# shenwei356/wfa

Measured on AMD Instinct MI355X. Metric: aligned pairs/sec (and Gcells/s) on 1e6 synthetic 1 kbp pairs @5% error, higher is better.
Workload: dtype u32; 1 GPU; 1000000 x 1000 bp pairs/GPU @5% error, global gap-affine 4/6/2, wf-adaptive 10/50/1, seed 3; config=c3, pairs_per_gpu=1000000, length=1000, parallelism=pair-sharded x1, ranks_seen_by_collective=1, backend=none (1 GPU), collective_forced=False, status_ok=1000000, setup_steps=0, gather=none (1 GPU), gather_bytes_per_rank_step=0, packed_pairs=1000000, retried_pairs=831

## Files before the change

### include/wfa_hip.h

```cpp
#ifndef WFA_HIP_H
#define WFA_HIP_H

#include <stddef.h>
#include <stdint.h>

#ifdef __cplusplus
extern "C" {
#endif

#define WFAHIP_VERSION 400

enum {
    WFAHIP_OK              = 0,
    WFAHIP_ERR_NO_DEVICE   = -1,
    WFAHIP_ERR_BAD_ARG     = -2,
    WFAHIP_ERR_OOM         = -3,
    WFAHIP_ERR_HIP         = -4,
    WFAHIP_ERR_UNSUPPORTED = -5,
    WFAHIP_ERR_INTERNAL    = -6
};

enum {
    WFAHIP_PAIR_OK        = 0,
    WFAHIP_PAIR_EMPTY     = 1,
// ... 180 lines not shown

int      wfahip_submit(wfahip_ctx *ctx, const uint8_t *q, uint32_t n, const uint8_t *t, uint32_t m, uint64_t *ticket);

int      wfahip_align_pair(wfahip_ctx *ctx, const wfahip_params *p, const uint8_t *q, uint32_t n, const uint8_t *t, uint32_t m,
                           uint32_t *rec, uint64_t *ops, uint64_t ops_cap, uint64_t *n_ops);
uint64_t wfahip_pending(const wfahip_ctx *ctx);
int      wfahip_collect(wfahip_ctx *ctx, const wfahip_params *p, wfahip_results *out);

typedef struct wfahip_multi wfahip_multi;
int         wfahip_create_multi(const int *device_ids, int n_devices, wfahip_multi **out);
void        wfahip_destroy_multi(wfahip_multi *m);
int         wfahip_multi_size(const wfahip_multi *m);
wfahip_ctx *wfahip_multi_ctx(wfahip_multi *m, int i);
int         wfahip_align_batch_multi(wfahip_multi *m, const wfahip_params *p, const uint8_t *seq_blob,
                                     uint64_t blob_bytes, const uint64_t *q_off, const uint32_t *q_len,
                                     const uint64_t *t_off, const uint32_t *t_len, uint64_t n_pairs,
                                     wfahip_results *out);

int  wfahip_last_timing(const wfahip_ctx *ctx, wfahip_timing *out);

int  wfahip_set_option(wfahip_ctx *ctx, const char *key, int64_t value);

typedef struct { uint32_t score; int32_t lo; uint32_t width; uint64_t word_off; } wfahip_row;
int  wfahip_debug_wavefronts(wfahip_ctx *ctx, const wfahip_params *p, const uint8_t *q, uint32_t n,
                             const uint8_t *t, uint32_t m, wfahip_row **rows, uint64_t *n_rows,
                             uint32_t **words, uint64_t *n_words, wfahip_results *res);
void wfahip_free(void *p);

int  wfahip_debug_team_compact(wfahip_ctx *ctx, const wfahip_params *p, const uint8_t *q, uint32_t n, const uint8_t *t, uint32_t m,
                               wfahip_row **rows, uint64_t *n_rows, uint32_t **words, uint64_t *n_words, wfahip_results *res);
int  wfahip_debug_compact_arena(wfahip_ctx *ctx, uint64_t pair, uint32_t **words, uint64_t *n_words, uint32_t *fmt,
                                uint32_t *meta4);

int  wfahip_debug_score_long_list(const uint8_t *seq_blob, const uint64_t *q_off, const uint32_t *q_len, const uint64_t *t_off,
                                  const uint32_t *t_len, uint64_t n_pairs, uint32_t **words, uint64_t *n_words, uint32_t **table,
                                  uint64_t *n_listed);

int  wfahip_debug_score_device_list(wfahip_ctx *ctx, uint32_t **words, uint64_t *n_words, uint32_t **table, uint64_t *n_listed);

int  wfahip_debug_prepack(wfahip_ctx *ctx, const void *d_seq_blob, const void *d_q_off, const void *d_q_len, const void *d_t_off,
                          const void *d_t_len, const void *d_work, uint64_t n, uint32_t seq_words, uint32_t ppw, uint32_t *slots);

int  wfahip_wide_class_bounds(uint32_t *bounds, int cap);

int  wfahip_debug_wide_plan(wfahip_ctx *ctx, const uint32_t *q_len, const uint32_t *t_len, uint64_t n_pairs, uint32_t **ids,
                            uint64_t *counts, uint32_t *longest, uint64_t *n_ladder);

uint64_t wfahip_gen_stride(uint32_t length, double error_rate);
int      wfahip_generate_pairs(uint64_t seed, uint64_t first_index, uint64_t n_pairs, uint32_t length,
                               double error_rate, int n_threads, uint8_t *blob, uint64_t *q_off,
                               uint32_t *q_len, uint64_t *t_off, uint32_t *t_len);

int      wfahip_debug_clock(wfahip_ctx *ctx, double *mhz, double *mhz_min, double *mhz_max);
int      wfahip_generate_pairs_device(wfahip_ctx *ctx, uint64_t seed, uint64_t first_index, uint64_t n_pairs, uint32_t length,
                                      double error_rate, void *d_blob, void *d_q_off, void *d_q_len, void *d_t_off,
                                      void *d_t_len, void *stream);

#ifdef __cplusplus
}
#endif
#endif
```

### wfa_amd/_lib.py

```python
from __future__ import annotations

import ctypes as C
import os

_HERE = os.path.dirname(os.path.abspath(__file__))
LIB_PATH = os.path.join(_HERE, "lib", "libwfahip.so")

OK, ERR_NO_DEVICE, ERR_BAD_ARG, ERR_OOM, ERR_HIP, ERR_UNSUPPORTED, ERR_INTERNAL = 0, -1, -2, -3, -4, -5, -6
PAIR_OK, PAIR_EMPTY, PAIR_TOO_LONG, PAIR_NO_MEMORY = 0, 1, 2, 4
PAIR_OVER_MAX = 8
MAX_SEQ_LEN = (1 << 29) - 1
REC_WORDS = 16
(REC_STATUS, REC_SCORE, REC_TBEGIN, REC_TEND, REC_QBEGIN, REC_QEND, REC_ALIGN_LEN, REC_MATCHES, REC_GAPS,
 REC_GAP_REGIONS, REC_OPS_LEN, REC_OPS_OFF_LO, REC_OPS_OFF_HI, REC_CELLS_LO, REC_CELLS_HI, REC_N_SCORES) = range(16)

EXPORTS = [
    "wfahip_version", "wfahip_strerror", "wfahip_device_count", "wfahip_create", "wfahip_destroy",
    "wfahip_align_batch", "wfahip_results_free", "wfahip_align_batch_device", "wfahip_last_timing",
    "wfahip_set_option", "wfahip_debug_wavefronts", "wfahip_free", "wfahip_gen_stride",
    "wfahip_generate_pairs", "wfahip_packed_words", "wfahip_pack_pairs", "wfahip_align_batch_packed", "wfahip_align_batch_packed_rc", "wfahip_submit",
    "wfahip_pending", "wfahip_collect", "wfahip_create_multi", "wfahip_destroy_multi", "wfahip_multi_size",
    "wfahip_multi_ctx", "wfahip_align_batch_multi", "wfahip_debug_compact_arena",
    "wfahip_generate_pairs_device", "wfahip_align_pair", "wfahip_last_error", "wfahip_debug_clock",
    "wfahip_debug_team_compact", "wfahip_score_batch", "wfahip_scores_free", "wfahip_score_matrix",
    "wfahip_debug_score_long_list", "wfahip_score_batch_device", "wfahip_debug_score_device_list",
    "wfahip_align_batch_bounded", "wfahip_align_batch_bounded_device", "wfahip_score_batch_packed",
    "wfahip_wide_class_bounds", "wfahip_debug_wide_plan", "wfahip_debug_prepack",
    "wfahip_score_batch_packed_rc", "wfahip_score_matrix_rc", "wfahip_revcomp_packed",
    "wfahip_cigar_text_device", "wfahip_cigar_text", "wfahip_cigars_free", "wfahip_align_batch_text",
    "wfahip_alignment_text_device", "wfahip_alignment_text", "wfahip_align_texts_free",
    "wfahip_pack_pairs_device", "wfahip_align_batch_packed_device",
    "wfahip_score_batch_packed_device", "wfahip_select_pairs_device",
    "wfahip_alignment_text_packed_device", "wfahip_alignment_text_packed",
]


class Params(C.Structure):
    _fields_ = [("mismatch", C.c_uint32), ("gap_open", C.c_uint32), ("gap_ext", C.c_uint32),
                ("global_alignment", C.c_uint8), ("adaptive", C.c_uint8), ("reserved", C.c_uint8 * 2),
                ("min_wf_len", C.c_uint32), ("max_dist_diff", C.c_uint32), ("cutoff_step", C.c_uint32)]


class Results(C.Structure):
    _fields_ = [("n", C.c_uint64), ("status", C.POINTER(C.c_int32)), ("score", C.POINTER(C.c_uint32)),
                ("tbegin", C.POINTER(C.c_int32)), ("tend", C.POINTER(C.c_int32)),
                ("qbegin", C.POINTER(C.c_int32)), ("qend", C.POINTER(C.c_int32)),
                ("align_len", C.POINTER(C.c_uint32)), ("matches", C.POINTER(C.c_uint32)),
                ("gaps", C.POINTER(C.c_uint32)), ("gap_regions", C.POINTER(C.c_uint32)),
                ("ops_off", C.POINTER(C.c_uint64)), ("ops_len", C.POINTER(C.c_uint32)),
                ("ops", C.POINTER(C.c_uint64)), ("n_ops", C.c_uint64)]


class Scores(C.Structure):
    _fields_ = [("n", C.c_uint64), ("status", C.POINTER(C.c_int32)), ("score", C.POINTER(C.c_uint32))]


class Cigars(C.Structure):
    _fields_ = [("n", C.c_uint64), ("n_bytes", C.c_uint64), ("text", C.POINTER(C.c_uint8)), ("off", C.POINTER(C.c_uint64))]


class AlignTexts(C.Structure):
    _fields_ = [("n", C.c_uint64), ("n_bytes", C.c_uint64), ("q_row", C.POINTER(C.c_uint8)), ("a_row", C.POINTER(C.c_uint8)),
                ("t_row", C.POINTER(C.c_uint8)), ("off", C.POINTER(C.c_uint64))]


class Timing(C.Structure):
    _fields_ = [("kernel_ms", C.c_double), ("total_ms", C.c_double), ("n_launches", C.c_uint32),
                ("n_retried_pairs", C.c_uint32), ("cells_stored", C.c_uint64), ("ops_written", C.c_uint64),
                ("arena_bytes", C.c_uint64), ("main_kernel_ms", C.c_double), ("n_main_launches", C.c_uint32),
                ("n_packed_pairs", C.c_uint32), ("main_kernel_kind", C.c_uint32), ("ladder_start_level", C.c_uint32)]


class Row(C.Structure):
    _fields_ = [("score", C.c_uint32), ("lo", C.c_int32), ("width", C.c_uint32), ("word_off", C.c_uint64)]


_lib = None


def lib():
    global _lib
    if _lib is None:
        if not os.path.exists(LIB_PATH):
            raise RuntimeError(f"{LIB_PATH} is missing: build the HIP extension first "
                               "(`make` or `python -c 'import __graft_entry__ as g; g.build()'`). "
                               "There is no CPU fallback.")
# ... 51 lines not shown
        L.wfahip_cigar_text.argtypes = [C.POINTER(Results), C.c_int, C.c_int, C.POINTER(Cigars)]
        L.wfahip_cigars_free.argtypes = [C.POINTER(Cigars)]
        L.wfahip_align_batch_text.restype = C.c_int
        L.wfahip_align_batch_text.argtypes = [vp, C.POINTER(Params), vp, u64, vp, vp, vp, vp, u64, C.c_int, C.POINTER(Results),
                                              C.POINTER(Cigars)]
        L.wfahip_alignment_text_device.restype = C.c_int
        L.wfahip_alignment_text_device.argtypes = [vp, vp, vp, u64, vp, u64, vp, vp, vp, vp, u64, C.c_int, vp, vp, vp, u64, vp,
                                                   C.POINTER(u64), vp]
        L.wfahip_alignment_text.restype = C.c_int
        L.wfahip_alignment_text.argtypes = [C.POINTER(Results), vp, u64, vp, vp, vp, vp, C.c_int, C.c_int, C.POINTER(AlignTexts)]
        L.wfahip_align_texts_free.argtypes = [C.POINTER(AlignTexts)]
        L.wfahip_alignment_text_packed_device.restype = C.c_int
        L.wfahip_alignment_text_packed_device.argtypes = [vp, vp, vp, u64, vp, u64, vp, vp, vp, vp, vp, u64, C.c_int, vp, vp, vp, u64, vp,
                                                          C.POINTER(u64), vp]
        L.wfahip_alignment_text_packed.restype = C.c_int
        L.wfahip_alignment_text_packed.argtypes = [C.POINTER(Results), vp, u64, vp, vp, vp, vp, vp, C.c_int, C.c_int, C.POINTER(AlignTexts)]
        L.wfahip_last_timing.restype = C.c_int
        L.wfahip_last_timing.argtypes = [vp, C.POINTER(Timing)]
        L.wfahip_set_option.restype = C.c_int
        L.wfahip_set_option.argtypes = [vp, C.c_char_p, C.c_int64]
        L.wfahip_debug_wavefronts.restype = C.c_int
        L.wfahip_debug_wavefronts.argtypes = [vp, C.POINTER(Params), C.c_char_p, u32, C.c_char_p, u32,
                                              C.POINTER(C.POINTER(Row)), C.POINTER(u64),
                                              C.POINTER(C.POINTER(u32)), C.POINTER(u64), C.POINTER(Results)]
        L.wfahip_debug_team_compact.restype = C.c_int
        L.wfahip_debug_team_compact.argtypes = [vp, C.POINTER(Params), C.c_char_p, u32, C.c_char_p, u32,
                                              C.POINTER(C.POINTER(Row)), C.POINTER(u64),
                                              C.POINTER(C.POINTER(u32)), C.POINTER(u64), C.POINTER(Results)]
        L.wfahip_free.argtypes = [vp]
        L.wfahip_gen_stride.restype = u64
        L.wfahip_gen_stride.argtypes = [u32, C.c_double]
        L.wfahip_generate_pairs.restype = C.c_int
        L.wfahip_generate_pairs.argtypes = [u64, u64, u64, u32, C.c_double, C.c_int, vp, vp, vp, vp, vp]
        L.wfahip_packed_words.restype = u64
        L.wfahip_packed_words.argtypes = [u32]
        L.wfahip_pack_pairs.restype = C.c_int
        L.wfahip_pack_pairs.argtypes = [vp, vp, vp, vp, vp, u64, C.c_int, vp, vp, vp, C.POINTER(u64)]
        L.wfahip_align_batch_packed.restype = C.c_int
        L.wfahip_align_batch_packed.argtypes = [vp, C.POINTER(Params), vp, u64, vp, vp, vp, vp, u64, C.POINTER(Results)]
        L.wfahip_align_batch_packed_rc.restype = C.c_int
        L.wfahip_align_batch_packed_rc.argtypes = [vp, C.POINTER(Params), vp, u64, vp, vp, vp, vp, vp, u64, C.POINTER(Results)]
        L.wfahip_pack_pairs_device.restype = C.c_int
        L.wfahip_pack_pairs_device.argtypes = [vp, vp, u64, vp, vp, vp, vp, u64, vp, u64, vp, vp, C.POINTER(u64), vp]
        L.wfahip_align_batch_packed_device.restype = C.c_int
        L.wfahip_align_batch_packed_device.argtypes = [vp, C.POINTER(Params), vp, u64, vp, vp, vp, vp, vp, u64, u32, u32, vp, vp,
                                                       u64, C.POINTER(u64), vp]
        L.wfahip_score_batch_packed_device.restype = C.c_int
        L.wfahip_score_batch_packed_device.argtypes = [vp, C.POINTER(Params), vp, u64, vp, vp, vp, vp, vp, u64, u32, u32, vp, vp, vp]
        L.wfahip_select_pairs_device.restype = C.c_int
        L.wfahip_select_pairs_device.argtypes = [vp, vp, u64, vp, vp, vp, vp, vp, vp, vp, vp, vp, vp, vp, C.POINTER(u64), vp]
        L.wfahip_submit.restype = C.c_int
        L.wfahip_submit.argtypes = [vp, C.c_char_p, u32, C.c_char_p, u32, C.POINTER(u64)]
        L.wfahip_pending.restype = u64
        L.wfahip_debug_clock.restype = C.c_int
        L.wfahip_debug_clock.argtypes = [vp, C.POINTER(C.c_double), C.POINTER(C.c_double), C.POINTER(C.c_double)]
        L.wfahip_align_pair.restype = C.c_int
        L.wfahip_align_pair.argtypes = [vp, C.POINTER(Params), C.c_char_p, u32, C.c_char_p, u32, vp, vp, u64, C.POINTER(u64)]
        L.wfahip_last_error.restype = C.c_char_p
        L.wfahip_last_error.argtypes = [vp]
        L.wfahip_pending.argtypes = [vp]
        L.wfahip_collect.restype = C.c_int
        L.wfahip_collect.argtypes = [vp, C.POINTER(Params), C.POINTER(Results)]
        L.wfahip_create_multi.restype = C.c_int
        L.wfahip_create_multi.argtypes = [C.POINTER(C.c_int), C.c_int, C.POINTER(vp)]
        L.wfahip_destroy_multi.argtypes = [vp]
        L.wfahip_multi_size.restype = C.c_int
        L.wfahip_multi_size.argtypes = [vp]
        L.wfahip_multi_ctx.restype = vp
        L.wfahip_multi_ctx.argtypes = [vp, C.c_int]
        L.wfahip_align_batch_multi.restype = C.c_int
        L.wfahip_align_batch_multi.argtypes = [vp, C.POINTER(Params), vp, u64, vp, vp, vp, vp, u64, C.POINTER(Results)]
        L.wfahip_debug_compact_arena.restype = C.c_int
        L.wfahip_debug_compact_arena.argtypes = [vp, u64, C.POINTER(C.POINTER(u32)), C.POINTER(u64), C.POINTER(u32),
                                                 C.POINTER(u32 * 4)]
        L.wfahip_generate_pairs_device.restype = C.c_int
        L.wfahip_generate_pairs_device.argtypes = [vp, u64, u64, u64, u32, C.c_double, vp, vp, vp, vp, vp, vp]
        _lib = L
    return _lib


class WfaHipError(RuntimeError):
    def __init__(self, code: int, what: str = ""):
        self.code = code
        msg = lib().wfahip_strerror(code).decode()
        super().__init__(f"{what}: {msg} ({code})" if what else f"{msg} ({code})")


def check(code: int, what: str = ""):
    if code != OK:
        raise WfaHipError(code, what)
```

### wfa_amd/aligner.py

```python
from __future__ import annotations

import ctypes as C
from dataclasses import dataclass, field
from typing import List, Optional, Sequence, Tuple

import numpy as np

from . import _lib as L

MaxSeqLen = L.MAX_SEQ_LEN
MaskLower32 = 4294967295
OpM, OpD, OpI, OpX, OpH = ord("M"), ord("D"), ord("I"), ord("X"), ord("H")


class WfaError(Exception):
    pass


ErrEmptySeq = WfaError("wfa: invalid empty sequence")
ErrSeqTooLong = WfaError(f"wfa: sequences longer than {MaxSeqLen} are not supported")
ErrOverMaxScore = WfaError("wfa: alignment score exceeds max_score")


@dataclass
# ... 842 lines not shown
        L.check(L.lib().wfahip_debug_team_compact(self._ctx, C.byref(prm), q, len(q), t, len(t), C.byref(rows),
                                                  C.byref(n_rows), C.byref(words), C.byref(n_words), C.byref(res)),
                "wfahip_debug_team_compact")
        try:
            out = {}
            for i in range(n_rows.value):
                r = rows[i]
                out[int(r.score)] = {r.lo + j: int(words[r.word_off + j]) for j in range(r.width)}
            br = BatchResult.from_c(res, 1)
        finally:
            L.lib().wfahip_free(rows)
            L.lib().wfahip_free(words)
            L.lib().wfahip_results_free(C.byref(res))
        return out, br.result(0)

    def debug_wavefronts(self, q: bytes, t: bytes):
        rows, words = C.POINTER(L.Row)(), C.POINTER(C.c_uint32)()
        n_rows, n_words = C.c_uint64(), C.c_uint64()
        res = L.Results()
        prm = self._params()
        L.check(L.lib().wfahip_debug_wavefronts(self._ctx, C.byref(prm), q, len(q), t, len(t), C.byref(rows),
                                                C.byref(n_rows), C.byref(words), C.byref(n_words), C.byref(res)),
                "wfahip_debug_wavefronts")
        try:
            out = {"M": {}, "I": {}, "D": {}}
            for i in range(n_rows.value):
                r = rows[i]
                for ci, name in enumerate("MID"):
                    d = {}
                    for j in range(r.width):
                        w = words[r.word_off + ci * r.width + j]
                        if w:
                            d[r.lo + j] = int(w)
                    if d:
                        out[name][int(r.score)] = d
            br = BatchResult.from_c(res, 1)
        finally:
            L.lib().wfahip_free(rows)
            L.lib().wfahip_free(words)
            L.lib().wfahip_results_free(C.byref(res))
        return out, br.result(0)

    def debug_compact_arena(self, pair: int):
        words = C.POINTER(C.c_uint32)()
        n_words, fmt, meta = C.c_uint64(), C.c_uint32(), (C.c_uint32 * 4)()
        L.check(L.lib().wfahip_debug_compact_arena(self._ctx, pair, C.byref(words), C.byref(n_words), C.byref(fmt),
                                                   C.byref(meta)), "wfahip_debug_compact_arena")
        try:
            arr = np.ctypeslib.as_array(words, shape=(int(n_words.value),)).copy()
        finally:
            L.lib().wfahip_free(words)
        return arr, int(fmt.value), tuple(int(x) for x in meta)

    def debug_wide_plan(self, q_len, t_len):
        q_len = np.ascontiguousarray(q_len, dtype=np.uint32)
        t_len = np.ascontiguousarray(t_len, dtype=np.uint32)
        n, nc = int(len(q_len)), len(wide_class_bounds())
        if len(t_len) != n:
            raise ValueError("q_len and t_len differ in length")
        ids = C.POINTER(C.c_uint32)()
        counts, longest, n_ladder = (C.c_uint64 * nc)(), (C.c_uint32 * nc)(), C.c_uint64()
        vp = lambda a: a.ctypes.data_as(C.c_void_p)
        L.check(L.lib().wfahip_debug_wide_plan(self._ctx, vp(q_len), vp(t_len), n, C.byref(ids), counts, longest, C.byref(n_ladder)),
                "wfahip_debug_wide_plan")
        try:
            flat = np.ctypeslib.as_array(ids, shape=(n,)).copy() if n else np.zeros(0, dtype=np.uint32)
        finally:
            L.lib().wfahip_free(ids)
        counts = [int(c) for c in counts]
        cuts = np.cumsum([0] + counts)
        lists = [flat[cuts[c]:cuts[c + 1]] for c in range(nc)]
        return lists, counts, [int(x) for x in longest], flat[cuts[nc]:cuts[nc] + int(n_ladder.value)]

    def debug_prepack(self, blob, q_off, q_len, t_off, t_len, seq_words: int, ppw: int = 4, work=None):
        import torch
        dev = self._want_tensor("blob", blob, torch.uint8)
        for name, t, dtype in (("q_off", q_off, torch.int64), ("q_len", q_len, torch.int32), ("t_off", t_off, torch.int64),
                               ("t_len", t_len, torch.int32)):
            self._want_tensor(name, t, dtype, dev)
        if work is not None:
            self._want_tensor("work", work, torch.int32, dev)
        n = int(work.numel() if work is not None else q_len.numel())
        slots = np.zeros((n, 4 + 2 * int(seq_words)), dtype=np.uint32)
        torch.cuda.current_stream(dev).synchronize()
        L.check(L.lib().wfahip_debug_prepack(self._ctx, blob.data_ptr(), q_off.data_ptr(), q_len.data_ptr(), t_off.data_ptr(), t_len.data_ptr(),
                                             work.data_ptr() if work is not None else None, n, int(seq_words), int(ppw),
                                             slots.ctypes.data_as(C.c_void_p)), "wfahip_debug_prepack")
        return slots

    def Plot(self, q: bytes, t: bytes, component: str = "M", notChangeToMatch: bool = False, maxScore: int = -1) -> str:
        wf, _ = self.debug_wavefronts(q, t)
        return plot_component(q, t, wf, component, self.p, notChangeToMatch, maxScore)

    def close(self):
        if getattr(self, "_ctx", None):
            L.lib().wfahip_destroy(self._ctx)
            self._ctx = None

    def __del__(self):
        try:
            self.close()
        except Exception:
            pass


def _take_results(res: "L.Results", n: int) -> "BatchResult":
# ... 368 lines not shown
```

### wfa_amd/csrc/wfa_common.hpp

```cpp
#pragma once
#include <hip/hip_runtime.h>
#include <stdint.h>
#include "wfa_ladder.hpp"


#define WFA_RARE(x) __builtin_expect(!!(x), 0)
#define WFA_OFTEN(x) __builtin_expect(!!(x), 1)

namespace wfa {

enum : uint32_t {
    TAG_INS_OPEN = 1, TAG_INS_EXT = 2, TAG_DEL_OPEN = 3, TAG_DEL_EXT = 4, TAG_MISMATCH = 5, TAG_MATCH = 6
};
constexpr uint32_t TAG_BITS = 3, TAG_MASK = 7;

enum : uint32_t {
    ST_OK = 0, ST_EMPTY = 1, ST_TOO_LONG = 2, ST_NO_MEMORY = 4,
    ST_OVER_MAX = 8,
    ST_PENDING = 0xFFFFFFFFu,
    DONE_NOT_OK = 0x80000000u,
    DONE_TAKEN  = 0xFFFFFFFFu,
    ST_REDO_BYTES = 100,
    ST_REDO_ARENA = 101,
    ST_REDO_LDS   = 102,
// ... 26 lines not shown
    uint32_t        n_work;
    uint32_t *queue_head;
    uint32_t *arena;
    uint64_t  arena_words;
    uint32_t x, o, e, oe, g;
    uint32_t global_alignment, adaptive, min_wf_len, max_dist_diff;
    uint32_t           *rec;
    uint64_t           *ops;
    uint64_t            ops_cap;
    unsigned long long *ops_cursor;
    uint32_t           *redo_list;
    uint32_t           *redo_count;
    uint32_t lds_seq_words;
    uint32_t *debug_info;

    uint32_t  chunk_first, chunk_n;
    uint4    *pair_meta;
    uint32_t  dx, doe, de;
    uint32_t  dm, di;
    uint32_t  sub_lds_words;
    uint32_t  min_xe;
    uint4    *done_q;
    uint32_t *done_ctl;
    uint32_t  n_stream_wgs;
    uint32_t  stream_wait;
    uint32_t  blk_batch_n;
    const uint32_t *prepack;
    uint32_t        prepack_words;
    uint32_t  wave_rows;
    uint32_t  wave_bt;
    uint32_t  census;
    uint32_t *page_ctl;
    uint32_t  page_words_log2, n_pages;
    uint64_t  dir_region_words;
    uint32_t  fuse_bt;
    uint32_t  lds_arena_off;
    uint32_t  one_n, one_m;
    uint32_t *wide_ckpt;
    uint32_t  wide_ckpt_on;
    uint32_t  wide_exact;
    uint32_t  compact_fmt;
    uint2    *score_out;
    uint32_t  max_score;
    const uint4    *mx_seq;
    const uint32_t *mx_words;
    uint64_t        mx_r0, mx_c0;
    uint64_t        mx_tbase;
    uint32_t        mx_cols;
    uint32_t        duo_claim;
    const uint8_t  *q_rc;
    uint64_t        mx_rc_shift;
    uint64_t        rc_top;
    const uint32_t *mx_rc_words;
};

}
```

### wfa_amd/csrc/wfa_ctx.hpp

```cpp
#pragma once
#include "../../include/wfa_hip.h"
#include "wfa_common.hpp"
#include "wfa_kinds.hpp"

#include <algorithm>
#include <atomic>
#include <chrono>
#include <cmath>
#include <cstdio>
#include <cstdlib>
#include <cstring>
#include <deque>
#include <functional>
#include <malloc.h>
#include <mutex>
#include <new>
#include <numeric>
#include <string>
#include <thread>
#include <vector>
#include <fcntl.h>
#include <optional>
#include <sys/file.h>
#include <unistd.h>
// ... 96 lines not shown
    int64_t       opt_team_wgs             = 0;
    int64_t       opt_team_solo_max        = 4096;
    bool          opt_team_solo_max_set    = false;
    int64_t       opt_team_wave            = 1;
    int64_t       opt_team_strict          = 1;
    int64_t       opt_unpack_all           = 0;
    int64_t       opt_team_compact         = 1;
    int64_t       opt_team_fast            = 1;
    int64_t       opt_team_pipe            = 1;
    int64_t       opt_team_scout           = 0;
    int64_t       opt_team_order           = 1;
    int64_t       opt_team_slack           = 1024;
    bool          dbg_teamc                = false;
    DevBuf        xbuf;
    int64_t       opt_team_paged           = 1;
    DevBuf        page_ctl;
    int64_t       opt_team_xcd             = 2;
    int64_t       opt_arena_poison         = 0;
    int64_t       opt_pilot                = 1;
    int64_t       opt_tail_overlap         = 1;
    int64_t       opt_overlap              = 0;
    int64_t       opt_fail_pass            = 0;
    int64_t       opt_prepack              = 0;
    int64_t       opt_narrow_long          = 0;
    DevBuf        score_out;
    DevBuf        wide_ckpt;
    DevBuf        mx_seq, mx_words;
    DevBuf        in_rc, rc_jobs;
    DevBuf        sd_ctl, sd_blk, sd_list, sd_redo;
    uint64_t      sd_n_words = 0, sd_n_listed = 0;
    DevBuf        sd_words;
    DevBuf        cig;
    DevBuf        cig_text, cig_off;
    DevBuf        pkd;
    DevBuf        mx_out;
    uint2        *mx_pin       = nullptr;
    size_t        mx_pin_bytes = 0;
    hipEvent_t    mx_ev[4]     = {};
    int64_t       opt_matrix_tile_cells    = 0;
    int64_t       opt_score_long_min       = 64;
    int64_t       opt_score_long_window    = 256;
    int64_t       opt_wide                 = 1;
    int64_t       opt_wide_max_len         = 2047;
    int           opt_wide_waves           = 0;
    bool          opt_wide_exact           = false;
    int64_t       opt_wide_min_pairs       = 64;
    int64_t       opt_wide_bin_min_pairs   = 4096;
    int64_t       opt_wide_classes         = 1;
    DevBuf        wide_ids, wide_blk, wide_ctl;
    int64_t       opt_duo                  = 1;
    int64_t       opt_duo_min_pairs        = 200000;
    bool          opt_duo_pk               = true;
    int64_t       opt_duo_claim            = 0;
    int64_t       opt_duo_short            = 0;
    int64_t       opt_duo_short_min_pairs  = 50000;
    bool          ctrl_clean               = false;
    hipStream_t   ctrl_clean_stream        = nullptr;
    hipEvent_t    ctrl_clean_ev            = nullptr;
    bool          redo_was_empty           = false;
    int64_t       opt_compact_call_bases   = 50000000;
    int64_t       opt_lane                 = 1;
    int64_t       opt_lane_pack            = 1;
    int64_t       opt_lane_min_pairs       = 32768;
    int64_t       opt_long                 = 1;
    int64_t       opt_long_min_len         = 4000;
    int64_t       opt_long_window_words    = 240;
    int64_t       opt_long_first           = 0;
    int64_t       opt_long_wave_bt         = 1;
    int64_t       opt_census               = 0;
    int64_t       opt_learn                = 1;
    uint64_t      learn_key                = 0;
    int           learn_level              = 0;
    uint32_t      learn_calls              = 0;
    uint64_t      rows_key                 = 0;
    uint32_t      rows_scale               = 1;
    uint64_t      band_key                 = 0;
    int           band_kind                = 0;
    uint32_t      band_calls               = 0;
    int64_t       opt_blk_mid              = 1;
    int64_t       opt_mem_limit            = 0;
    int           force_mode               = -1;
    const uint32_t *dbg_arena = nullptr;
    const uint4    *dbg_meta  = nullptr;
    uint64_t        dbg_words = 0, dbg_first = 0, dbg_n = 0;
    uint32_t        dbg_fmt = 0, dbg_g = 1;
    uint32_t        max_score = 0;
    wfahip_timing timing{};
    char          last_error[256] = {0};
};

struct BoundScope {
    wfahip_ctx *c;
    uint32_t    keep;
    BoundScope(wfahip_ctx *ctx, uint32_t max_score) : c(ctx), keep(ctx ? ctx->max_score : 0u) {
        if (c) c->max_score = max_score;
    }
    ~BoundScope() {
        if (c) c->max_score = keep;
    }
    BoundScope(const BoundScope &) = delete;
    BoundScope &operator=(const BoundScope &) = delete;
};


inline int ensure(wfahip_ctx *ctx, DevBuf &b, size_t bytes) {
    if (b.bytes >= bytes && b.p) return WFAHIP_OK;
// ... 91 lines not shown
```

### wfa_amd/csrc/wfa_device.hpp

```cpp
#pragma once
#include "wfa_common.hpp"

namespace wfa {

#define WFA_DEV __device__ __forceinline__

WFA_DEV uint32_t umax2(uint32_t a, uint32_t b) { return a > b ? a : b; }
WFA_DEV uint32_t umin2(uint32_t a, uint32_t b) { return a < b ? a : b; }
WFA_DEV int      imin2(int a, int b) { return a < b ? a : b; }
WFA_DEV int      imax2(int a, int b) { return a > b ? a : b; }

WFA_DEV void push_redo(const KParams &P, uint32_t pair, uint32_t status) {
    const uint32_t i     = atomicAdd(P.redo_count, 1u);
    P.redo_list[2u * i]      = pair;
    P.redo_list[2u * i + 1u] = status;
}

#define WFA_WAVE_REDUCE(OP)                                                                                   \
    asm("s_nop 1\n\t" OP " %0, %0, %0 quad_perm:[1,0,3,2] row_mask:0xf bank_mask:0xf\n\ts_nop 1\n\t" OP          \
        " %0, %0, %0 quad_perm:[2,3,0,1] row_mask:0xf bank_mask:0xf\n\ts_nop 1\n\t" OP                          \
        " %0, %0, %0 row_half_mirror row_mask:0xf bank_mask:0xf\n\ts_nop 1\n\t" OP                              \
        " %0, %0, %0 row_mirror row_mask:0xf bank_mask:0xf\n\ts_nop 1\n\t" OP                                   \
        " %0, %0, %0 row_bcast:15 row_mask:0xa bank_mask:0xf\n\ts_nop 1\n\t" OP                                 \
        " %0, %0, %0 row_bcast:31 row_mask:0xc bank_mask:0xf\n\ts_nop 1"                                         \
// ... 285 lines not shown
    WFA_DEV void prepare(uint32_t s, int k) const {
        uint32_t idx;
        (void)split(s, idx);
        if (n_ent == 0u) return;
        if (idx >= n_ent) idx = n_ent - 1u;
        const uint32_t need_lo = idx >= dmax ? idx - dmax : 0u;
        if (need_lo < win_lo || idx > win_hi) refill(idx, k);
    }
    WFA_DEV uint32_t get_raw(int comp, uint32_t s, int k) const {
        uint32_t idx;
        bool     ok = split(s, idx);
        ok          = ok && idx < n_ent;
        missed = missed || (ok && (idx < win_lo || idx > win_hi));
        const DirEnt e = win[idx & 63u];
        ok = ok && e.w > 0 && k >= e.lo && k < e.lo + e.w;
        const uint64_t off = ok ? e.base + (uint64_t)comp * e.stride + (uint32_t)(k - e.lo) : 0ull;
        const uint32_t v   = A[off];
        return ok ? v : 0u;
    }
};

struct OpsWriter {
    uint64_t *buf;
    uint32_t  cap;
    uint32_t  n;
    uint64_t  cur;
    bool      overflow;
    WFA_DEV void init(uint64_t *b, uint32_t c) {
        buf = b, cap = c, n = 0, cur = 0, overflow = false;
    }
    WFA_DEV void add(uint32_t letter, uint32_t cnt) {
        if (cur != 0 && (uint32_t)(cur >> 32) == letter) {
            cur += cnt;
            return;
        }
        flush();
        cur = ((uint64_t)letter << 32) | cnt;
    }
    WFA_DEV void flush() {
        if (cur != 0) {
            if (n < cap)
                buf[n] = cur;
            else
                overflow = true;
            n++;
            cur = 0;
        }
    }
};

#ifndef WFA_OPS_GROUP
#define WFA_OPS_GROUP 8
#endif
struct OpsWriterRev {
    uint64_t *buf;
    uint32_t  cap;
    uint32_t  n;
    uint64_t  cur;
    bool      overflow;
    bool      seenM;
    uint32_t  alen, matches, gaps, regions;
    uint32_t  p_len, p_gaps, p_regions;
    uint64_t  last;
    static constexpr uint32_t GROUP = WFA_OPS_GROUP;
    uint64_t  hist[GROUP > 1 ? GROUP - 1 : 1];
    bool      grouped;
    bool      active = true;
    bool      combine = true;
    WFA_DEV void init(uint64_t *b, uint32_t c) {
        buf = b, cap = c, n = 0, cur = 0, overflow = false, seenM = false;
        grouped = combine && GROUP > 1 && (reinterpret_cast<uintptr_t>(b + c) & (8u * GROUP - 1u)) == 0u;
#pragma unroll
        for (uint32_t i = 0; i + 1 < GROUP; i++) hist[i] = 0;
        alen = matches = gaps = regions = 0;
        p_len = p_gaps = p_regions = 0;
        last = 0;
    }
    WFA_DEV void add(uint32_t letter, uint32_t cnt) {
        if (cur != 0 && (uint32_t)(cur >> 32) == letter) {
            cur += cnt;
            return;
        }
        flush();
        cur = ((uint64_t)letter << 32) | cnt;
    }
    WFA_DEV void flush() {
        if (cur == 0) return;
        if (n < cap) {
            if (!active) {
            } else if (!grouped) {
                buf[cap - 1 - n] = cur;
            } else if ((n & (GROUP - 1u)) == GROUP - 1u) {
                ulonglong2 *d = reinterpret_cast<ulonglong2 *>(buf + (cap - 1 - n));
                d[0] = make_ulonglong2(cur, hist[0]);
#pragma unroll
                for (uint32_t i = 1; i < GROUP / 2; i++) d[i] = make_ulonglong2(hist[2 * i - 1], hist[2 * i]);
            }
        } else {
            overflow = true;
        }
        n++;
        const uint32_t letter = (uint32_t)(cur >> 32), cnt = (uint32_t)cur;
        const bool     isM = letter == 'M', isG = letter == 'I' || letter == 'D';
        const bool     join = isM && seenM;
        alen += (join ? p_len : 0u) + (isM ? cnt : 0u), matches += isM ? cnt : 0u;
        gaps += join ? p_gaps : 0u, regions += join ? p_regions : 0u;
        p_len     = isM ? 0u : p_len + cnt;
        p_gaps    = isM ? 0u : p_gaps + (isG ? cnt : 0u);
        p_regions = isM ? 0u : p_regions + (isG ? 1u : 0u);
        seenM     = seenM || isM;
        if (grouped) {
#pragma unroll
            for (uint32_t i = GROUP > 1 ? GROUP - 2 : 0; i > 0; i--) hist[i] = hist[i - 1];
            hist[0] = cur;
        }
        last    = cur;
        cur     = 0;
    }
    WFA_DEV void finish() {
        if (grouped && n <= cap && active) {
            const uint32_t r = n & (GROUP - 1u);
#pragma unroll
            for (uint32_t i = 0; i + 1 < GROUP; i++)
                if (i < r) buf[cap - n + i] = hist[i];
        }
        if (!seenM && n > 0) {
            const uint32_t letter = (uint32_t)(last >> 32), cnt = (uint32_t)last;
            alen = cnt, matches = 0;
            gaps    = (letter == 'I' || letter == 'D') ? cnt : 0u;
            regions = (letter == 'I' || letter == 'D') ? 1u : 0u;
        }
    }
};

struct CompactView {
    const uint32_t *A;
    uint64_t        cap;
    uint32_t        g, n_ent, fmt;
    bool            coherent = false;
    WFA_DEV uint32_t ld(uint64_t i) const {
        return coherent ? __hip_atomic_load(A + i, __ATOMIC_RELAXED, __HIP_MEMORY_SCOPE_AGENT) : A[i];
    }
    WFA_DEV uint32_t word(uint32_t idx, int k) const {
        if (idx >= n_ent) return 0u;
        if (fmt == 3u) return ld(512ull * (idx >> 3) + (((uint32_t)k & 60u) << 3) + ((idx & 7u) << 2) + ((uint32_t)k & 3u));
        if (fmt == 1u) return ld(64ull * idx + ((uint32_t)k & 63u));
        if (fmt == 4u) return ld(256ull * idx + ((uint32_t)k & 255u));
        if (fmt == 5u) return ld(32ull * idx + ((uint32_t)k & 31u));
        if (fmt == 6u) return ld(128ull * idx + ((uint32_t)k & 127u));
        if (fmt == 7u)
            return reinterpret_cast<const uint16_t *>(A)[512ull * (idx >> 3) + (((uint32_t)k & 60u) << 3) + ((idx & 7u) << 2) + ((uint32_t)k & 3u)];
        if (fmt == 10u)
            return reinterpret_cast<const uint16_t *>(A)[(uint64_t)(((uint32_t)k & 56u) >> 3) * (uint32_t)(cap >> 5) * 8u + 64ull * (idx >> 3) + (((uint32_t)k & 4u) << 3) +
                                                         ((idx & 7u) << 2) + ((uint32_t)k & 3u)];
        if (fmt == 9u)
            return reinterpret_cast<const uint16_t *>(A)[(uint64_t)(((uint32_t)k & 60u) >> 2) * (uint32_t)(cap >> 5) * 4u + 4ull * idx + ((uint32_t)k & 3u)];
        if (fmt == 8u)
            return reinterpret_cast<const uint16_t *>(A)[32ull * idx + ((uint32_t)k & 31u)];
        const uint4 e = *reinterpret_cast<const uint4 *>(A + cap - 4ull * (idx + 1));
        const int   lo = (int)e.y, w = (int)e.z;
        if (w <= 0 || k < lo || k >= lo + w) return 0u;
        if (fmt == 11u) return reinterpret_cast<const uint16_t *>(A)[e.x + (uint32_t)(k - lo)];
        return A[e.x + (uint32_t)(k - lo)];
    }
    WFA_DEV uint32_t tag(int comp, uint32_t idx, int k, uint32_t &off0) const {
        const uint32_t wd = word(idx, k);
        if (fmt != 0u) return blk_tag(wd, comp, off0);
        off0              = wd >> 7;
        if (comp == 0) return wd & TAG_MASK;
        if (comp == 1) {
            const uint32_t t = (wd >> 3) & 3u;
            return t == 1u ? TAG_INS_OPEN : (t == 2u ? TAG_INS_EXT : 0u);
        }
        const uint32_t t = (wd >> 5) & 3u;
        return t == 1u ? TAG_DEL_OPEN : (t == 2u ? TAG_DEL_EXT : 0u);
    }
};

#ifndef WFA_BTW_ROWS
#define WFA_BTW_ROWS 32
#endif
struct CompactViewWave {
    const uint32_t *A;
    uint64_t        cap;
    uint32_t        g, n_ent, fmt;
    static constexpr int ROWS = WFA_BTW_ROWS;
// ... 375 lines not shown
```

### wfa_amd/csrc/wfa_duo.hip

```cpp
#define WFA_NO_AUX_KERNELS 1
#include "wfa_duo.hpp"
#include "wfa_fwd.hpp"

namespace wfa {

namespace {
template <int DX, int DOE>
hipError_t go_duo(const KParams &P, uint32_t grid, size_t lds_bytes, hipStream_t st, bool census, bool pk) {
    if (pk && census)
        hipLaunchKernelGGL((wfa_duo_kernel<true, DX, DOE>), dim3(grid), dim3(64), lds_bytes, st, P);
    else if (pk)
        hipLaunchKernelGGL((wfa_duo_kernel<false, DX, DOE>), dim3(grid), dim3(64), lds_bytes, st, P);
    else if (census)
        hipLaunchKernelGGL((wfa_duo32_kernel<true, DX, DOE>), dim3(grid), dim3(64), lds_bytes, st, P);
    else
        hipLaunchKernelGGL((wfa_duo32_kernel<false, DX, DOE>), dim3(grid), dim3(64), lds_bytes, st, P);
    return hipGetLastError();
}
}

hipError_t wfa_launch_duo(int shape, const KParams &P, uint32_t grid, size_t lds_bytes, hipStream_t st, bool census, bool pk) {
    switch (shape) {
#define WFA_DUO_SHAPE(I, tag, DX_, DOE_) \
    case I: return go_duo<DX_, DOE_>(P, grid, lds_bytes, st, census, pk);
        WFA_FWD_SHAPES(WFA_DUO_SHAPE)
#undef WFA_DUO_SHAPE
    }
    return hipErrorInvalidValue;
}

}
```

### wfa_amd/csrc/wfa_duo.hpp

```cpp
#pragma once
#include "wfa_blk.hpp"
#include "wfa_duo_cfg.hpp"
#include "wfa_pk16.hpp"

namespace wfa {

struct DuoRed {
#define WFA_DUO_3(opa, opb, opc)                                                                                    \
    unsigned long long sv;                                                                                          \
    asm volatile("s_nop 1\n\t" opa " %0, %0, %0 " WFA_DPP_CTL_XOR1 "\n\t" opb " %1, %1, %1 " WFA_DPP_CTL_XOR1 "\n\t" opc \
        " %2, %2, %2 " WFA_DPP_CTL_XOR1 "\n\t" opa " %0, %0, %0 " WFA_DPP_CTL_XOR2 "\n\t" opb " %1, %1, %1 "        \
        WFA_DPP_CTL_XOR2 "\n\t" opc " %2, %2, %2 " WFA_DPP_CTL_XOR2 "\n\t" opa " %0, %0, %0 " WFA_DPP_CTL_HMIR "\n\t" \
        opb " %1, %1, %1 " WFA_DPP_CTL_HMIR "\n\t" opc " %2, %2, %2 " WFA_DPP_CTL_HMIR "\n\t"                         \
        "s_and_saveexec_b64 %3, %4\n\t" opa " %0, %0, %0 " WFA_DPP_CTL_MIR "\n\t" opb " %1, %1, %1 " WFA_DPP_CTL_MIR    \
        "\n\t" opc " %2, %2, %2 " WFA_DPP_CTL_MIR "\n\ts_mov_b64 exec, %3"                                            \
        : "+v"(a), "+v"(b), "+v"(c), "=&s"(sv)                                                                      \
        : "s"(wm)                                                                                                   \
        : "scc");
#define WFA_DUO_2(opa, opb)                                                                                         \
    unsigned long long sv;                                                                                          \
    asm volatile("s_nop 1\n\t" opa " %0, %0, %0 " WFA_DPP_CTL_XOR1 "\n\t" opb " %1, %1, %1 " WFA_DPP_CTL_XOR1 "\n\ts_nop 0\n\t" \
        opa " %0, %0, %0 " WFA_DPP_CTL_XOR2 "\n\t" opb " %1, %1, %1 " WFA_DPP_CTL_XOR2 "\n\ts_nop 0\n\t" opa        \
        " %0, %0, %0 " WFA_DPP_CTL_HMIR "\n\t" opb " %1, %1, %1 " WFA_DPP_CTL_HMIR "\n\t"                            \
        "s_and_saveexec_b64 %2, %3\n\t" opa " %0, %0, %0 " WFA_DPP_CTL_MIR "\n\t" opb " %1, %1, %1 " WFA_DPP_CTL_MIR    \
        "\n\ts_mov_b64 exec, %2"                                                                                    \
        : "+v"(a), "+v"(b), "=&s"(sv)                                                                               \
        : "s"(wm)                                                                                                   \
        : "scc");
#define WFA_DUO_1(opa)                                                                                              \
    unsigned long long sv;                                                                                          \
    asm volatile("s_nop 1\n\t" opa " %0, %0, %0 " WFA_DPP_CTL_XOR1 "\n\ts_nop 1\n\t" opa " %0, %0, %0 " WFA_DPP_CTL_XOR2 \
        "\n\ts_nop 1\n\t" opa " %0, %0, %0 " WFA_DPP_CTL_HMIR "\n\t"                                                \
        "s_and_saveexec_b64 %1, %2\n\ts_nop 0\n\t" opa " %0, %0, %0 " WFA_DPP_CTL_MIR "\n\ts_mov_b64 exec, %1"       \
        : "+v"(a), "=&s"(sv)                                                                                        \
        : "s"(wm)                                                                                                   \
        : "scc");
    static WFA_DEV void min_max_min(int &a, int &b, int &c, unsigned long long wm) { WFA_DUO_3("v_min_i32_dpp", "v_max_i32_dpp", "v_min_i32_dpp") }
    static WFA_DEV void min_max(int &a, int &b, unsigned long long wm) { WFA_DUO_2("v_min_i32_dpp", "v_max_i32_dpp") }
    static WFA_DEV void max_add(int &a, int &b, unsigned long long wm) { WFA_DUO_2("v_max_i32_dpp", "v_add_u32_dpp") }
    static WFA_DEV int  max1(int a, unsigned long long wm) {
        WFA_DUO_1("v_max_i32_dpp")
        return a;
    }
    static WFA_DEV int or1(int a, unsigned long long wm) {
        WFA_DUO_1("v_or_b32_dpp")
        return a;
    }
#undef WFA_DUO_3
#undef WFA_DUO_2
#undef WFA_DUO_1
};

static WFA_DEV unsigned long long duo_lanes(bool b) {
    unsigned long long mask = __builtin_amdgcn_ballot_w64(b);
    asm("" : "+s"(mask));
    return mask;
}
static WFA_DEV bool duo_lane_of(unsigned long long mask) { return __builtin_amdgcn_inverse_ballot_w64(mask); }

template <bool ON>
static WFA_DEV uint32_t duo_uniform(uint32_t x) {
    if constexpr (ON) return (uint32_t)__builtin_amdgcn_readfirstlane((int)x);
    else return x;
}
using DuoArgs = const __attribute__((address_space(4))) KParams;
static WFA_DEV DuoArgs *duo_cold_args() {
    DuoArgs *p = (DuoArgs *)__builtin_amdgcn_kernarg_segment_ptr();
    asm volatile("" : "+s"(p));
    return p;
}

template <bool CENSUS, int DX, int DOE, bool PK>
__device__ __attribute__((always_inline)) inline void duo_run(const KParams &P) {
    constexpr int PP = 4;
    static_assert(DX >= 1 && DOE >= 1 && DX <= 4 && DOE <= 4, "ring depths of one to four score steps");
    constexpr int R  = DX > DOE ? DX : DOE;
    constexpr int RW = PK ? 2 : PP;
    constexpr bool UNI = WFA_DUO_UNIFORM != 0 && PK;
    constexpr int  SCA = WFA_DUO_SCALAR != 0 && UNI ? WFA_DUO_SCALAR_ITEMS : 0;
    constexpr bool SC_ARGS = (SCA & 1) != 0, SC_UNI = (SCA & 2) != 0, SC_SLOW = (SCA & 4) != 0, SC_NZ = (SCA & 8) != 0, SC_SI = (SCA & 16) != 0;
    extern __shared__ __attribute__((aligned(16))) uint32_t lds[];
    const int  lane = threadIdx.x, l7 = lane & 7, l15 = lane & 15;
    const bool hi_half = (lane & 8) != 0;

    const uint32_t  SW = P.lds_seq_words, PW = P.prepack_words;
    const uint32_t  FP = duo_fetch_pairs(PW), NBUF = duo_bufs(PW);
    uint32_t *const park0 = lds + NBUF * PW;
    const uint64_t  cap      = P.arena_words;
    const int       mdd      = (int)P.max_dist_diff;
    const int       minwf    = (int)P.min_wf_len;
    const bool      adaptive = P.adaptive != 0;
    const uint32_t  seed_si  = P.dx;
    uint32_t        pk_one   = 0x00010001u;
    if constexpr (PK) asm volatile("" : "+s"(pk_one));
    const int       rows_cap = (int)(cap / 32);

    int       st = 0;
    bool      wide = false;
    uint32_t  pidx = 0, si = 0, cells = 0, sbuf = 0;
    int       n = 0, m = 0, kb = 0;
    bool      slow = false, first_eq = false;
    unsigned long long run_m = 0ull, wide_m = 0ull;
    unsigned long long slow_m = 0ull;
    int             j = l7, k0 = 0;
    int             jp[4] = {4 * l7, 4 * l7 + 1, 4 * l7 + 2, 4 * l7 + 3}, kp[4] = {0, 1, 2, 3}, kedge = 31;
    uint32_t        mdn = 0u, mup = 0u;
    const uint32_t *lq = lds + 4, *lt = lds + 4;
    uint32_t       *rowp = nullptr;

    uint32_t M[R][RW], I[RW], D[RW];
    int      rlo[R], rhi[R];
    int      lim[PP], lmx[PP];
#pragma unroll
    for (int d = 0; d < R; d++) {
        rlo[d] = BK_BIG, rhi[d] = -BK_BIG;
#pragma unroll
        for (int p = 0; p < RW; p++) M[d][p] = 0u;
    }
#pragma unroll
    for (int p = 0; p < RW; p++) I[p] = D[p] = 0u;
#pragma unroll
    for (int p = 0; p < PP; p++) lim[p] = 0, lmx[p] = 0;

    uint32_t buf_free  = (1u << NBUF) - 1u;
    uint32_t park_used = 0u;
// ... 13 lines not shown

#ifdef WFA_STAMPS
    unsigned long long stamp_acc[8] = {0, 0, 0, 0, 0, 0, 0, 0}, stamp_prev;
    unsigned long long evt[16] = {0, 0, 0, 0, 0, 0, 0, 0, 0, 0, 0, 0, 0, 0, 0, 0};
    asm volatile("s_memtime %0\n\ts_waitcnt lgkmcnt(0)" : "=s"(stamp_prev)::"memory");
#endif
    const auto args = [&]() {
        if constexpr (SC_ARGS) return duo_cold_args();
        else return &P;
    };
    const auto pair_of = [&](const auto *A, uint32_t idx) { return A->work ? A->work[idx] : A->chunk_first + idx; };
    const auto redo = [&](const auto *A, uint32_t pair, uint32_t status) {
        const uint32_t i = atomicAdd(A->redo_count, 1u);
        A->redo_list[2u * i]      = pair;
        A->redo_list[2u * i + 1u] = status;
    };
    const auto uni = [](uint32_t x) __attribute__((always_inline)) { return duo_uniform<SC_UNI>(x); };
    const auto dn1 = [&](uint32_t x) { return (uint32_t)__builtin_amdgcn_update_dpp(0, (int)x, 0x111, 0xf, 0xf, true) & mdn; };
    const auto up1 = [&](uint32_t x) { return (uint32_t)__builtin_amdgcn_update_dpp(0, (int)x, 0x101, 0xf, 0xf, true) & mup; };
    const auto other_half = [&](int x) { return __builtin_amdgcn_update_dpp(0, x, 0x128, 0xf, 0xf, true); };
    const auto jx = [&](int p) { return UNI ? jp[p] : PP * j + p; };
    const auto kx = [&](int p) { return UNI && p != 0 ? kp[p] : k0 + p; };
    const auto set_derived = [&]() {
        if constexpr (UNI) run_m = duo_lanes(st == 1), wide_m = duo_lanes(wide);
        if constexpr (SC_SLOW) slow_m = duo_lanes(slow);
        const auto *const A = args();
        const uint64_t acap = A->arena_words;
        j   = wide ? l15 : l7;
        mdn = j == 0 ? 0u : ~0u;
        mup = j == (wide ? 15 : 7) ? 0u : ~0u;
        k0  = kb + PP * j;
#pragma unroll
        for (int p = 0; p < PP; p++) lim[p] = imax2(1, imin2(n + k0 + p, m)), lmx[p] = imax2(n + k0 + p, m);
        if constexpr (UNI) {
            static_assert(PP == 4, "four cells a lane");
#pragma unroll
            for (int p = 0; p < PP; p++) {
                jp[p] = PP * j + p, kp[p] = k0 + p;
                asm("" : "+v"(jp[p]));
                if (p != 0) asm("" : "+v"(kp[p]));
            }
            kedge = kb + (wide ? 64 : 32) - 1;
            asm("" : "+v"(kedge));
        }
        lq   = lds + sbuf * PW + 4u;
        lt   = lq + SW;
        if constexpr (DUO_ARENA_FMT == 10u)
            rowp = A->arena + (uint64_t)pidx * acap + (((uint32_t)k0 & 56u) >> 3) * (uint32_t)(rows_cap * 4) + (((uint32_t)k0 >> 2) & 1u) * 16u;
        else if constexpr (DUO_ARENA_FMT == 9u)
            rowp = A->arena + (uint64_t)pidx * acap + (((uint32_t)k0 & 60u) >> 2) * (uint32_t)(rows_cap * 2) + si * 2u;
        else
            rowp = A->arena + (uint64_t)pidx * acap + (uint64_t)(si >> 3) * 256u + (si & 7u) * 2u;
    };
    const auto clear_rings = [&]() {
#pragma unroll
        for (int d = 0; d < R; d++) {
            rlo[d] = BK_BIG, rhi[d] = -BK_BIG;
#pragma unroll
            for (int p = 0; p < RW; p++) M[d][p] = 0u;
        }
#pragma unroll
        for (int p = 0; p < RW; p++) I[p] = D[p] = 0u;
    };
    const auto or_halves = [&](uint32_t v) {
        uint32_t r = 0u;
#pragma unroll
        for (int o = 0; o < 8; o++) r |= (uint32_t)__builtin_amdgcn_readlane((int)v, 8 * o);
        return r;
    };

    const auto fill = [&](auto ph_c, unsigned long long m_free) __attribute__((always_inline)) {
        constexpr int ph = decltype(ph_c)::value;
        while (m_free != 0ull && (park_used != 0u || (pf & PF_STAGED) != 0u)) {
            const uint32_t oct  = (uint32_t)__builtin_ctzll(m_free) >> 3;
            const bool     mine = ((uint32_t)lane >> 3) == oct;
            if (park_used != 0u) {
                const uint32_t rec = (uint32_t)__builtin_ctz(park_used);
                park_used = uni(park_used & (park_used - 1u));
                WFA_EVT(4, 1);
                const uint32_t *const pr = park0 + rec * DUO_PARK_WORDS;
                if (mine) {
                    const uint4 *const w = reinterpret_cast<const uint4 *>(pr + 12 * l7);
                    const uint4 v0 = w[0], v1 = R > 2 ? w[1] : make_uint4(0u, 0u, 0u, 0u), v2 = w[2];
                    const uint32_t pw[8] = {v0.x, v0.y, v0.z, v0.w, v1.x, v1.y, v1.z, v1.w};
                    const uint4 *const s4 = reinterpret_cast<const uint4 *>(pr + 96);
                    const uint4 a0 = s4[0], a1 = s4[1], a2 = s4[2], a3 = s4[3];
                    const uint32_t plo[4] = {a2.x, a2.y, a2.z, a2.w}, phi[4] = {a3.x, a3.y, a3.z, a3.w};
#pragma unroll
                    for (int r = 0; r < R; r++) {
                        if constexpr (PK) {
                            M[(ph + r) % R][0] = pw[2 * r], M[(ph + r) % R][1] = pw[2 * r + 1];
                        } else {
                            M[(ph + r) % R][0] = pw[2 * r] & 0xFFFFu, M[(ph + r) % R][1] = pw[2 * r] >> 16;
                            M[(ph + r) % R][2] = pw[2 * r + 1] & 0xFFFFu, M[(ph + r) % R][3] = pw[2 * r + 1] >> 16;
                        }
                        rlo[(ph + r) % R] = (int)plo[r], rhi[(ph + r) % R] = (int)phi[r];
                    }
                    if constexpr (PK) {
                        I[0] = v2.x, I[1] = v2.y, D[0] = v2.z, D[1] = v2.w;
                    } else {
                        I[0] = v2.x & 0xFFFFu, I[1] = v2.x >> 16, I[2] = v2.y & 0xFFFFu, I[3] = v2.y >> 16;
                        D[0] = v2.z & 0xFFFFu, D[1] = v2.z >> 16, D[2] = v2.w & 0xFFFFu, D[3] = v2.w >> 16;
                    }
                    pidx = a0.x, si = a0.y, cells = a0.z, sbuf = a0.w;
                    n = (int)a1.x, m = (int)a1.y, kb = (int)a1.z, slow = (a1.w & 1u) != 0u, first_eq = (a1.w & 2u) != 0u;
                    st = 1, wide = false;
                }
                m_free &= ~(0xFFull << (8 * oct));
                continue;
            }
            pf_buf   = (uint32_t)__builtin_ctz(st_mask);
            st_mask = uni(st_mask & (st_mask - 1u));
            const uint32_t this_idx = pf_idx;
            pf_idx = uni(pf_idx + 1u);
            const uint32_t *const hb = lds + pf_buf * PW;
            const uint32_t nq = (uint32_t)__builtin_amdgcn_readfirstlane((int)hb[0]), mt = (uint32_t)__builtin_amdgcn_readfirstlane((int)hb[1]);
            const uint32_t status = (uint32_t)__builtin_amdgcn_readfirstlane((int)hb[2]);
            if (st_mask == 0u) pf = uni(pf & ~PF_STAGED);
            if (status != ST_PENDING) {
                if (lane == 0) {
                    const auto *const A = args();
                    A->pair_meta[this_idx] = make_uint4(status, 0u, 0u, 0u);
                    if (status >= ST_REDO_BYTES) redo(A, pair_of(A, this_idx), status);
                }
                buf_free = uni(buf_free | (1u << pf_buf));
                continue;
            }
            WFA_EVT(5, 1);
            if (mine) {
                pidx = this_idx, sbuf = pf_buf;
                n = (int)nq, m = (int)mt;
                const int Ak = m - n;
                si = 0, cells = 0, slow = false;
                kb = -16 + PP * imax2(-3, imin2(3, Ak / (2 * PP)));
                first_eq = ((hb[4] ^ hb[4 + SW]) & 3u) == 0u;
                clear_rings();
                st = 1, wide = false;
            }
            m_free &= ~(0xFFull << (8 * oct));
        }
    };

    const auto refill = [&](auto ph_c) __attribute__((always_inline)) -> bool {
        constexpr int ph  = decltype(ph_c)::value;
        constexpr int NEW = (ph + R - 1) % R;
        if constexpr (!SC_UNI) {
            pf        = (uint32_t)__builtin_amdgcn_readfirstlane((int)pf);
            park_used = (uint32_t)__builtin_amdgcn_readfirstlane((int)park_used);
            buf_free  = (uint32_t)__builtin_amdgcn_readfirstlane((int)buf_free);
            st_mask   = (uint32_t)__builtin_amdgcn_readfirstlane((int)st_mask);
            pf_next   = (uint32_t)__builtin_amdgcn_readfirstlane((int)pf_next);
            pf_end    = (uint32_t)__builtin_amdgcn_readfirstlane((int)pf_end);
        }
        if ((pf & (PF_LD | PF_STAGED)) == PF_LD) {
            const uint32_t cnt = pf_next - pf_ld_idx;
            st_mask = 0u;
            {
                uint32_t f = buf_free;
                for (uint32_t c = 0; c < cnt; c++) st_mask |= f & (0u - f), f &= f - 1u;
            }
            st_mask = uni(st_mask), buf_free = uni(buf_free & ~st_mask);
            const uint32_t w0 = (uint32_t)lane * 4u, slot = w0 / PW;
            if (slot < cnt) {
                uint32_t f = st_mask;
                for (uint32_t c = 0; c < slot; c++) f &= f - 1u;
                const uint32_t b = (uint32_t)__builtin_ctz(f);
                *reinterpret_cast<uint4 *>(lds + b * PW + (w0 - slot * PW)) = pf_w;
            }
            pf_idx = uni(pf_ld_idx), pf = uni((pf | PF_STAGED) & ~PF_LD);
        }
        if ((pf & (PF_TOK | PF_LD)) == PF_TOK) {
            const auto *const A = args();
            if (pf_next >= pf_end) {
                const uint32_t chunk_n = A->chunk_n;
                const uint32_t tok = (uint32_t)__builtin_amdgcn_readfirstlane((int)pf_tok) + claim_base();
                const uint32_t blk = claim_fetches(chunk_n) * FP;
                pf_next = tok, pf_end = uni(tok < chunk_n ? umin2(tok + blk, chunk_n) : tok);
            }
            pf_ld_idx = uni(pf_next);
            const bool have = pf_next < pf_end;
            if (have) {
                const uint32_t *const slot = A->prepack + (uint64_t)pf_ld_idx * PW;
                const uint32_t cnt = umin2(FP, pf_end - pf_next);
                pf_next += cnt;
                if ((uint32_t)lane * 4u < cnt * PW) pf_w = *reinterpret_cast<const uint4 *>(slot + lane * 4);
            }
            pf_next = uni(pf_next);
            pf = uni((pf & ~PF_TOK) | (have ? PF_LD : PF_DRY));
        }
        if ((pf & (PF_TOK | PF_DRY)) == 0u) {
            if (pf_next >= pf_end) {
                const auto *const A = args();
                const uint32_t blk = claim_fetches(A->chunk_n) * FP;
                if (lane == 0) pf_tok = atomicAdd(A->queue_head, blk);
            }
            pf = uni(pf | PF_TOK);
        }
        unsigned long long m_free;
        WFA_STAMP(0);
        for (;;) {
        const int  Wc    = wide ? 64 : 32;
        const bool run   = UNI ? duo_lane_of(run_m) : st == 1;
        bool       touch, narrowable = false;
        unsigned long long m_ev;
        if constexpr (UNI) {
            const unsigned long long touch_m =
                run_m & duo_lanes(rhi[NEW] >= rlo[NEW]) & (duo_lanes(rlo[NEW] <= kb) | duo_lanes(rhi[NEW] >= kedge));
            unsigned long long narrow_m = 0ull;
            if constexpr (ph == 0) {
                int ulo = rlo[0], uhi = rhi[0];
#pragma unroll
                for (int d = 1; d < R; d++) ulo = imin2(ulo, rlo[d]), uhi = imax2(uhi, rhi[d]);
                narrow_m = run_m & wide_m & duo_lanes(uhi - ulo + 1 <= DUO_NARROW_AT);
            }
            touch = duo_lane_of(touch_m), narrowable = duo_lane_of(narrow_m);
            m_ev = touch_m | narrow_m, m_free = ~run_m;
        } else {
            touch = run && rhi[NEW] >= rlo[NEW] && (rlo[NEW] <= kb || rhi[NEW] >= kb + Wc - 1);
            if constexpr (ph == 0) {
                int ulo = rlo[0], uhi = rhi[0];
#pragma unroll
                for (int d = 1; d < R; d++) ulo = imin2(ulo, rlo[d]), uhi = imax2(uhi, rhi[d]);
                narrowable    = run && wide && uhi - ulo + 1 <= DUO_NARROW_AT;
            }
            m_ev = __ballot(touch || narrowable), m_free = __ballot(st == 0);
        }
        if (__builtin_expect(!(m_ev != 0ull || (m_free != 0ull && (park_used != 0u || (pf & PF_STAGED) != 0u))), 1)) break;
        WFA_EVT(1, 1);
        {
            int ulo = rlo[0], uhi = rhi[0];
#pragma unroll
            for (int d = 1; d < R; d++) ulo = imin2(ulo, rlo[d]), uhi = imax2(uhi, rhi[d]);
            const int span = uhi - ulo + 1;
            int act = 0;
            if (touch) act = wide ? (span > DUO_WIDE_MAX ? 4 : 1) : (span > DUO_WIDEN_AT ? 2 : 1);
            else if (narrowable) act = 3;
            const int Wn  = act == 2 ? 64 : (act == 3 ? 32 : Wc);
            const int kbn = (((ulo + uhi + 1 - Wn) >> 1) + 2) & ~3;
            if (act != 0 && act != 4 && !(ulo - kbn >= 1 && uhi - kbn <= Wn - 2)) act = 4;
            const int  o_act = other_half(act), o_kb = other_half(kb), o_kbn = other_half(kbn);
            const bool o_wide = other_half(wide ? 1 : 0) != 0;
// ... 4 lines not shown
            bool               lost    = false;
            while (m_evict != 0ull) {
                const int      l0   = __builtin_ctzll(m_evict);
                const uint32_t oct  = (uint32_t)l0 >> 3;
                m_evict &= ~(0xFFull << (8 * oct));
                const bool mine = evict && ((uint32_t)lane >> 3) == oct;
                if (park_used == (1u << DUO_PARK) - 1u) {
                    if (((uint32_t)lane >> 3) == (oct ^ 1u)) lost = true;
                    if (mine) evict = false, taken = false;
                    continue;
                }
                const uint32_t rec = (uint32_t)__builtin_ctz(~park_used);
                park_used = uni(park_used | (1u << rec));
                WFA_EVT(3, 1);
                uint32_t *const pr = park0 + rec * DUO_PARK_WORDS;
                if (mine) {
                    uint4 *const w = reinterpret_cast<uint4 *>(pr + 12 * l7);
                    const auto pk  = [](uint32_t lo, uint32_t hi) { return lo | (hi << 16); };
                    const auto pk2 = [&](const uint32_t(&v)[RW], int h) -> uint32_t {
                        if constexpr (PK) return v[h];
                        else return pk(v[2 * h], v[2 * h + 1]);
                    };
                    uint32_t pw[8];
                    int      plo[4], phi[4];
#pragma unroll
                    for (int r = 0; r < 4; r++) {
                        pw[2 * r]     = r < R ? pk2(M[(ph + r) % R], 0) : 0u;
                        pw[2 * r + 1] = r < R ? pk2(M[(ph + r) % R], 1) : 0u;
                        plo[r] = r < R ? rlo[(ph + r) % R] : BK_BIG, phi[r] = r < R ? rhi[(ph + r) % R] : -BK_BIG;
                    }
                    w[0] = make_uint4(pw[0], pw[1], pw[2], pw[3]);
                    if constexpr (R > 2) w[1] = make_uint4(pw[4], pw[5], pw[6], pw[7]);
                    w[2] = make_uint4(pk2(I, 0), pk2(I, 1), pk2(D, 0), pk2(D, 1));
                    if (l7 == 0) {
                        uint4 *const s4 = reinterpret_cast<uint4 *>(pr + 96);
                        s4[0] = make_uint4(pidx, si, cells, sbuf);
                        s4[1] = make_uint4((uint32_t)n, (uint32_t)m, (uint32_t)kb, (slow ? 1u : 0u) | (first_eq ? 2u : 0u));
                        s4[2] = make_uint4((uint32_t)plo[0], (uint32_t)plo[1], (uint32_t)plo[2], (uint32_t)plo[3]);
                        s4[3] = make_uint4((uint32_t)phi[0], (uint32_t)phi[1], (uint32_t)phi[2], (uint32_t)phi[3]);
                    }
                }
            }
            if (lost) widen = false, act = 4;
            {
                const bool o_lost = other_half(lost ? 1 : 0) != 0;
                if (o_lost) taken = false;
            }
            if (__ballot(act == 4) != 0ull) {
                WFA_EVT(7, __builtin_popcountll(__ballot(act == 4 && j == 0)));
                if (act == 4 && j == 0) {
                    const auto *const A = args();
                    A->pair_meta[pidx] = make_uint4(ST_REDO_BAND, 0u, 0u, 0u);
                    redo(A, pair_of(A, pidx), ST_REDO_BAND);
                }
                buf_free = uni(or_halves(act == 4 ? (1u << sbuf) : 0u) | buf_free);
                if (act == 4) {
                    st = 0, wide = false;
                    clear_rings();
                }
            }
            const int  rb   = lane & ~15;
            const bool join = taken;
            int src = lane;
            bool moved = false, freed = false;
            {
                if (join) {
                    const int Bo = (lane & ~7) ^ 8, dl = (o_kbn - o_kb) >> 2, jo = (lane - rb) + dl;
                    src = (jo >= 0 && jo < 8) ? Bo + jo : -1, moved = true;
                } else if (act == 1) {
                    const int Bo = wide ? rb : (lane & ~7), Go = wide ? 16 : 8, dl = (kbn - kb) >> 2, jo = (lane - Bo) + dl;
                    src = (jo >= 0 && jo < Go) ? Bo + jo : -1, moved = true;
                } else if (widen) {
                    const int Bo = lane & ~7, dl = (kbn - kb) >> 2, jo = (lane - rb) + dl;
                    src = (jo >= 0 && jo < 8) ? Bo + jo : -1, moved = true;
                } else if (act == 3) {
                    const int dl = (kbn - kb) >> 2, jo = (lane - rb) + dl;
                    if (hi_half) src = -1, freed = true;
                    else src = (jo >= 0 && jo < 16) ? rb + jo : -1;
                    moved = true;
                }
            }
            if (__ballot(moved) != 0ull) {
                WFA_EVT(2, 1);
                const int sl = (src < 0 ? lane : src) << 2;
#pragma unroll
                for (int d = 0; d < R; d++)
#pragma unroll
                    for (int p = 0; p < RW; p++) {
                        const uint32_t v = (uint32_t)__builtin_amdgcn_ds_bpermute(sl, (int)M[d][p]);
                        M[d][p]          = src < 0 ? 0u : v;
                    }
#pragma unroll
                for (int p = 0; p < RW; p++) {
                    const uint32_t v = (uint32_t)__builtin_amdgcn_ds_bpermute(sl, (int)I[p]);
                    const uint32_t u = (uint32_t)__builtin_amdgcn_ds_bpermute(sl, (int)D[p]);
                    I[p] = src < 0 ? 0u : v, D[p] = src < 0 ? 0u : u;
                }
                if (__ballot(join) != 0ull) {
                    const int      o_n = other_half(n), o_m = other_half(m);
                    const uint32_t o_pidx = (uint32_t)other_half((int)pidx), o_si = (uint32_t)other_half((int)si);
                    const uint32_t o_cells = (uint32_t)other_half((int)cells), o_sbuf = (uint32_t)other_half((int)sbuf);
                    const int      o_fl = other_half((slow ? 1 : 0) | (first_eq ? 2 : 0));
                    int o_rlo[R], o_rhi[R];
#pragma unroll
                    for (int d = 0; d < R; d++) o_rlo[d] = other_half(rlo[d]), o_rhi[d] = other_half(rhi[d]);
                    if (join) {
                        n = o_n, m = o_m, pidx = o_pidx, si = o_si, cells = o_cells, sbuf = o_sbuf;
                        slow = (o_fl & 1) != 0, first_eq = (o_fl & 2) != 0;
#pragma unroll
                        for (int d = 0; d < R; d++) rlo[d] = o_rlo[d], rhi[d] = o_rhi[d];
                        st = 1;
                    }
                }
                if (join) kb = o_kbn;
                else if (moved && !freed) kb = kbn;
                if (join || widen) wide = true;
                if (act == 3) wide = false;
                if (freed) {
                    st = 0;
#pragma unroll
                    for (int d = 0; d < R; d++) rlo[d] = BK_BIG, rhi[d] = -BK_BIG;
                }
            }
            fill(ph_c, __ballot(st == 0));
            set_derived();
            __builtin_amdgcn_fence(__ATOMIC_RELEASE, "wavefront");
            __builtin_amdgcn_fence(__ATOMIC_ACQUIRE, "wavefront");
        }
        }
        WFA_STAMP(1);
        return m_free == ~0ull && park_used == 0u && (pf & (PF_DRY | PF_LD | PF_STAGED)) == PF_DRY;
    };

    const auto step = [&](auto ph_c) __attribute__((always_inline)) {
        constexpr int ph = decltype(ph_c)::value;
        const bool run = UNI ? duo_lane_of(run_m) : st == 1;
        const auto any_run = [&](bool b) {
            if constexpr (UNI) return (duo_lanes(b) & run_m) != 0ull;
            else return __ballot(run && b) != 0ull;
        };
        const unsigned long long wm = UNI ? wide_m : __ballot(wide);
        WFA_EVT(0, 1), WFA_EVT(6, __builtin_popcountll(__ballot(run)) / 8);

        uint32_t(&Mo)[RW] = M[(ph + R - DOE) % R];
        uint32_t(&Mx)[RW] = M[(ph + R - DX) % R];
        uint32_t(&Mn)[RW] = M[ph];

        uint32_t nM[PP], nI[RW], nD[RW], wd[RW], cc[PP];
        const uint32_t a_edge = dn1(Mo[RW - 1]), b_edge = dn1(I[RW - 1]);
        const uint32_t c_edge = up1(Mo[0]), d_edge = up1(D[0]);
        const bool     slow_any = SC_SLOW ? (slow_m & run_m) != 0ull : any_run(slow);
        const auto next_slow = [&](const uint32_t(&Mo4)[PP], const uint32_t(&I4)[PP], const uint32_t(&D4)[PP], const uint32_t(&Mx4)[PP],
                                   uint32_t ae, uint32_t be, uint32_t ce, uint32_t de, uint32_t(&nI4)[PP], uint32_t(&nD4)[PP],
                                   uint32_t(&wd4)[PP]) __attribute__((always_inline)) {
#pragma unroll
            for (int p = 0; p < PP; p++) {
                const int      k  = kx(p);
                const uint32_t a0 = p ? Mo4[p - 1] : ae, b0 = p ? I4[p - 1] : be;
                const uint32_t c0 = p < PP - 1 ? Mo4[p + 1] : ce, d0 = p < PP - 1 ? D4[p + 1] : de;
                const uint32_t x0 = Mx4[p];
                const uint32_t a = (int)a0 > m ? 0u : a0, b = (int)b0 > m ? 0u : b0;
                const uint32_t c = (int)c0 - k > n ? 0u : c0, d = (int)d0 - k > n ? 0u : d0;
                const uint32_t x = ((int)x0 > m || (int)x0 - k > n) ? 0u : x0;
                const uint32_t mi = umax2(a, b), tI = umin2(mi, 1u), Isk = mi + tI;
                const uint32_t Dsk = umax2(c, d), tD = umin2(Dsk, 1u);
                const uint32_t x1  = x + umin2(x, 1u);
                const uint32_t Msk = umax3(Isk, Dsk, x1);
                const bool fromX = x != 0u && Msk == x1;
                const bool fromI = !fromX && Msk == Isk;
                const uint32_t mu = umax2(a0, b0), Iu = mu + umin2(mu, 1u), Du = umax2(c0, d0);
                const uint32_t Xu = x0 + umin2(x0, 1u);
                const bool     iext = a < b, dext = c < d;
                const uint32_t o0   = (fromI && iext) ? Iu : ((!fromX && !fromI && dext) ? Du : umax3(Iu, Du, Xu));
                const bool     kin  = k >= -(n - 1) && k <= m - 1;
                nM[p] = kin ? Msk : 0u, nI4[p] = kin ? Isk : 0u, nD4[p] = kin ? Dsk : 0u;
                wd4[p] = blk_word(o0, iext, dext, fromX, fromI);
                cc[p]  = (CENSUS && kin) ? tI + tD + umin2(Msk, 1u) : 0u;
            }
        };
        if constexpr (PK) {
// ... 269 lines not shown
                }
            }
        }

        WFA_STAMP(4);
        const bool keepl = anyM && ihi >= ilo && !no_room;
        if constexpr (CENSUS) {
            int cs = (int)csum, dummy = 0;
            DuoRed::max_add(dummy, cs, wm);
            cells += keepl ? (uint32_t)cs : 0u;
        }
        if constexpr (DUO_ARENA_FMT != 10u) rowp += 2;
        if constexpr (DUO_ARENA_FMT == 7u) rowp += (((uint32_t)(uintptr_t)rowp & 0x38u) == 0u) ? 240 : 0;

        if constexpr (PK) {
#pragma unroll
            for (int h = 0; h < 2; h++) {
                Mn[h] = nM[2 * h] | (nM[2 * h + 1] << 16);
                I[h]  = wide_u32(__builtin_elementwise_min(wide_pk(nI[h]), wide_pk(Mn[h])));
                D[h]  = wide_u32(__builtin_elementwise_min(wide_pk(nD[h]), wide_pk(Mn[h])));
            }
        } else {
#pragma unroll
            for (int p = 0; p < PP; p++) Mn[p] = nM[p], I[p] = nI[p], D[p] = nD[p];
        }
        rlo[ph] = keepl ? kb + ilo : BK_BIG;
        rhi[ph] = keepl ? kb + ihi : -BK_BIG;

        const unsigned long long fin_m = term_m | room_m;
        const bool fin = UNI ? duo_lane_of(fin_m) : run && (term || no_room);
        if constexpr (WFA_DUO_FILL != 0) {
            if constexpr (SC_SI) {
                unsigned long long co;
                asm("v_addc_co_u32_e64 %0, %1, %0, 0, %2" : "+v"(si), "=s"(co) : "s"(run_m & ~fin_m));
            } else if (run && !fin) si += 1u;
        }
        constexpr bool cold    = WFA_DUO_FILL != 0 && PK;
        const bool     any_fin = UNI ? fin_m != 0ull : __ballot(fin) != 0ull;
        if (cold ? __builtin_expect(any_fin, 0) : any_fin) {
            const auto *const A = args();
            const int ctot = (CENSUS && A->census) ? (int)cells : 0;
            int hf   = 0;
#pragma unroll
            for (int p = 0; p < PP; p++)
                if (kx(p) == m - n) hf = (int)nM[p];
            hf = DuoRed::max1(hf, wm);
            if (fin && j == 0) {
                if (no_room) {
                    A->pair_meta[pidx] = make_uint4(ST_REDO_ARENA, 0u, 0u, 0u);
                    redo(A, pair_of(A, pidx), ST_REDO_ARENA);
                } else {
                    A->pair_meta[pidx] = make_uint4(ST_OK, si * A->g, (uint32_t)hf, (uint32_t)ctot);
                }
            }
            buf_free = uni(or_halves(fin ? (1u << sbuf) : 0u) | buf_free);
            if (fin) {
                st = 0, wide = false;
                clear_rings();
            }
            if constexpr (WFA_DUO_FILL != 0) {
                fill(std::integral_constant<int, (ph + 1) % R>{}, __ballot(st == 0));
                set_derived();
                __builtin_amdgcn_fence(__ATOMIC_RELEASE, "wavefront");
                __builtin_amdgcn_fence(__ATOMIC_ACQUIRE, "wavefront");
            }
        }
        if constexpr (WFA_DUO_FILL == 0) {
            if (run && !fin) si += 1u;
            if constexpr (UNI)
                if (any_fin) set_derived();
        }
        WFA_STAMP(5);
    };

    for (;;) {
        if (refill(std::integral_constant<int, 0>{})) break;
        step(std::integral_constant<int, 0>{});
        if constexpr (R > 1) {
            if (refill(std::integral_constant<int, 1 % R>{})) break;
            step(std::integral_constant<int, 1 % R>{});
        }
        if constexpr (R > 2) {
            if (refill(std::integral_constant<int, 2 % R>{})) break;
            step(std::integral_constant<int, 2 % R>{});
        }
        if constexpr (R > 3) {
            if (refill(std::integral_constant<int, 3 % R>{})) break;
            step(std::integral_constant<int, 3 % R>{});
        }
    }
#ifdef WFA_STAMPS
    if (lane == 0 && P.debug_info) {
        unsigned long long *acc = reinterpret_cast<unsigned long long *>(P.debug_info);
        for (int i = 0; i < 8; i++) atomicAdd(acc + i, stamp_acc[i]);
        for (int i = 0; i < 16; i++) atomicAdd(acc + 8 + i, evt[i]);
    }
#endif
}

#ifndef WFA_DUO_VGPRS
#define WFA_DUO_VGPRS 64
#endif
static_assert(16u * (256u - 4u) / 2u < 2048u, "wfa_duo_kernel's packed rings need offsets under 4 096");
template <bool CENSUS, int DX = 2, int DOE = 4>
__global__ __launch_bounds__(64, WFA_DUO_WAVES) __attribute__((amdgpu_num_vgpr(WFA_DUO_VGPRS))) void wfa_duo_kernel(const KParams P) {
    duo_run<CENSUS, DX, DOE, true>(P);
}
template <bool CENSUS, int DX = 2, int DOE = 4>
__global__ __launch_bounds__(64, WFA_DUO_WAVES) __attribute__((amdgpu_num_vgpr(WFA_DUO_VGPRS))) void wfa_duo32_kernel(const KParams P) {
    duo_run<CENSUS, DX, DOE, false>(P);
}

}
```

### wfa_amd/csrc/wfa_duo_cfg.hpp

```cpp
#pragma once
#include "wfa_common.hpp"

namespace wfa {

#ifndef WFA_DUO_WAVES
#define WFA_DUO_WAVES 4
#endif
#ifndef WFA_DUO_PARK
#define WFA_DUO_PARK 4
#endif
#ifndef WFA_DUO_WIDEN_AT
#define WFA_DUO_WIDEN_AT 26
#endif
#ifndef WFA_DUO_NARROW_AT
#define WFA_DUO_NARROW_AT 21
#endif
#ifndef WFA_DUO_GROUP_MAJOR
#define WFA_DUO_GROUP_MAJOR 2
#endif
#ifndef WFA_DUO_EXTEND
#define WFA_DUO_EXTEND 1
#endif
#ifndef WFA_DUO_CLAIM
#define WFA_DUO_CLAIM 4
#endif
#ifndef WFA_DUO_FILL
#define WFA_DUO_FILL 1
#endif
#ifndef WFA_DUO_UNIFORM
#define WFA_DUO_UNIFORM 1
#endif
#ifndef WFA_DUO_SCALAR
#define WFA_DUO_SCALAR 1
#endif
#ifndef WFA_DUO_SCALAR_ITEMS
#define WFA_DUO_SCALAR_ITEMS 31
#endif
constexpr uint32_t DUO_ARENA_FMT = WFA_DUO_GROUP_MAJOR == 2 ? 10u : WFA_DUO_GROUP_MAJOR == 1 ? 9u : 7u;
constexpr int DUO_PARK       = WFA_DUO_PARK;
constexpr int DUO_PARK_WORDS = 8 * 12 + 16;
constexpr int DUO_BUFS       = 8 + 1 + DUO_PARK;
constexpr int DUO_FETCH_MAX  = 8;
constexpr int DUO_WIDEN_AT   = WFA_DUO_WIDEN_AT;
constexpr int DUO_NARROW_AT  = WFA_DUO_NARROW_AT;
constexpr int DUO_WIDE_MAX   = 56;
constexpr int DUO_CLAIM_MAX  = 8;
constexpr int DUO_CLAIM      = WFA_DUO_CLAIM;
static_assert(DUO_CLAIM >= 1 && DUO_CLAIM <= DUO_CLAIM_MAX, "WFA_DUO_CLAIM: 1 .. 8 fetches per claim");

__host__ __device__ inline uint32_t duo_fetch_pairs(uint32_t prepack_words) {
    const uint32_t f = 256u / prepack_words;
    return f < 1u ? 1u : (f > (uint32_t)DUO_FETCH_MAX ? (uint32_t)DUO_FETCH_MAX : f);
}
__host__ __device__ inline uint32_t duo_bufs(uint32_t prepack_words) { return 8u + duo_fetch_pairs(prepack_words) + (uint32_t)DUO_PARK; }
__host__ __device__ inline uint32_t duo_lds_words(uint32_t prepack_words) {
    return duo_bufs(prepack_words) * prepack_words + (uint32_t)DUO_PARK * DUO_PARK_WORDS;
}

hipError_t wfa_launch_duo(int shape, const KParams &P, uint32_t grid, size_t lds_bytes, hipStream_t st, bool census, bool pk);

}
```

### wfa_amd/csrc/wfa_entry.hip

```cpp
#define WFA_NO_AUX_KERNELS 1
#include "wfa_ctx.hpp"
#include "wfa_hostpack.hpp"
#include "wfa_rc.hpp"
#include "wfa_generic.hpp"
#include "wfa_packed.hpp"
#include "wfa_blk.hpp"
#include "wfa_duo_cfg.hpp"
#include "wfa_lane.hpp"
#include "wfa_fwd.hpp"
#include "wfa_long.hpp"
#include "wfa_finalize.hpp"

using namespace wfa;

void results_zero(wfahip_results *r) { std::memset(r, 0, sizeof *r); }

namespace {
struct ResBlock { void *p; size_t bytes; };
std::mutex            g_res_mu;
std::vector<ResBlock> g_res_cache;
size_t                g_res_cached_bytes = 0;
constexpr size_t      RES_CACHE_MIN = 1u << 20, RES_CACHE_MAX_BYTES = 4ull << 30, RES_CACHE_MAX_BLOCKS = 32;

std::vector<ResBlock> g_res_pinned;
// ... 854 lines not shown
    };
    const auto range = [&](uint64_t a, uint64_t b) {
        for (uint64_t i = a; i < b; i++) {
            one(seq_blob + q_off[i], q_len[i], packed + q_woff[i]);
            one(seq_blob + t_off[i], t_len[i], packed + t_woff[i]);
        }
    };
    parallel_ranges(0, n_pairs, (unsigned)std::min<uint64_t>((uint64_t)std::max(1, n_threads), n_pairs / 1024 + 1), range);
    return bad ? WFAHIP_ERR_UNSUPPORTED : WFAHIP_OK;
}

extern "C" int wfahip_pack_pairs(const uint8_t *seq_blob, const uint64_t *q_off, const uint32_t *q_len, const uint64_t *t_off,
                                 const uint32_t *t_len, uint64_t n_pairs, int n_threads, uint32_t *packed, uint64_t *q_woff,
                                 uint64_t *t_woff, uint64_t *n_words) {
    WFAHIP_GUARD(pack_pairs_impl(seq_blob, q_off, q_len, t_off, t_len, n_pairs, n_threads, packed, q_woff, t_woff, n_words))
}

namespace {
constexpr size_t ONE_PIN_BYTES = 1u << 20, ONE_IMG_MAX = 64u << 10, ONE_REC_OFF = ONE_IMG_MAX, ONE_OPS_OFF = ONE_IMG_MAX + 256;
}

static int align_pair_impl(wfahip_ctx *ctx, const wfahip_params *p, const uint8_t *q, uint32_t n, const uint8_t *t, uint32_t m,
                           uint32_t *rec_out, uint64_t *ops_out, uint64_t ops_cap, uint64_t *n_ops) {
    if (!ctx || !p || !rec_out || !n_ops || (!ops_out && ops_cap)) return WFAHIP_ERR_BAD_ARG;
    int rc = check_params(p);
    if (rc != WFAHIP_OK) return rc;
    std::memset(rec_out, 0, REC_WORDS * 4);
    *n_ops = 0;
    if (n == 0 || m == 0) {
        rec_out[REC_STATUS] = ST_EMPTY;
        return WFAHIP_OK;
    }
    if (n > WFAHIP_MAX_SEQ_LEN || m > WFAHIP_MAX_SEQ_LEN) {
        rec_out[REC_STATUS] = ST_TOO_LONG;
        return WFAHIP_OK;
    }
    if (!q || !t) return WFAHIP_ERR_BAD_ARG;
    const uint32_t max_len = std::max(n, m), min_len = std::min(n, m);
    const uint32_t g = gcd_u32(gcd_u32(p->mismatch, p->gap_open + p->gap_ext), p->gap_ext ? p->gap_ext : p->mismatch);
    const uint32_t seq_words = (max_len + 15) / 16 + 1;
    const uint64_t q_cap = ((uint64_t)n + 15) & ~15ull, img = q_cap + (((uint64_t)m + 15) & ~15ull) + 64;
    const uint64_t worst = (uint64_t)p->mismatch * min_len + 2ull * (p->gap_open + p->gap_ext) + (uint64_t)p->gap_ext * (max_len - min_len + 2);
    const uint32_t min_xe = std::min(p->mismatch, p->gap_ext ? p->gap_ext : p->mismatch);
    const uint64_t ops_bound = 2 * (worst / std::max(1u, min_xe)) + 64;
    const int  shape = p->gap_ext != 0 ? fwd_shape(p->mismatch / g, (p->gap_open + p->gap_ext) / g, p->gap_ext / g) : -1;
    const bool fast = ctx->opt_pair_fast != 0 && ctx->opt_packed != 0 && ctx->opt_blk == 16 && ctx->force_mode < 0 && p->global_alignment &&
                      shape >= 0 && (shape == 0 || ctx->opt_pair_fast == 1) &&
                      (size_t)seq_words * 2 * 4 * (ctx->opt_pair_fast == 1 ? 1 : 4) + 16 <= (ctx->opt_pair_fast == 1 ? 64 : 20) * 1024 && img <= ONE_IMG_MAX &&
                      ONE_OPS_OFF + ops_bound * 8 <= ONE_PIN_BYTES;
    if (fast) {
        HIP_TRY(hipSetDevice(ctx->device));
        if (ctx->bt_pending) {
            (void)hipStreamSynchronize(ctx->stream2);
            ctx->bt_pending = false;
        }
        if (!ctx->one_pin) {
            HIP_TRY(hipHostMalloc(reinterpret_cast<void **>(&ctx->one_pin), ONE_PIN_BYTES, hipHostMallocMapped));
            HIP_TRY(hipHostGetDevicePointer(reinterpret_cast<void **>(&ctx->one_dev), ctx->one_pin, 0));
        }
        hipStream_t st = ctx->stream;
        const uint64_t words = std::min<uint64_t>(((worst / g + 16) * 64 + 511) & ~511ull, std::max<uint64_t>(2048, (32ull * max_len + 511) & ~511ull));
        if ((rc = ensure(ctx, ctx->one_ctl, 1024))) return rc;
        if ((rc = ensure(ctx, ctx->redo, 64))) return rc;
        if ((rc = ensure(ctx, ctx->meta, 64))) return rc;
        if (ctx->arena.bytes < words * 4 && (rc = ensure(ctx, ctx->arena, words * 4))) return rc;
        char *const h = ctx->one_pin;
        std::memcpy(h, q, n);
        std::memcpy(h + q_cap, t, m);
        uint64_t *const offs = reinterpret_cast<uint64_t *>(h + img - 64);
        offs[0] = 0, offs[1] = q_cap;
        uint32_t *const lens = reinterpret_cast<uint32_t *>(offs + 2);
        lens[0] = n, lens[1] = m;
        uint32_t *const hrec = reinterpret_cast<uint32_t *>(h + ONE_REC_OFF);
        hrec[REC_STATUS] = ST_PENDING;
        uint32_t *const d_ctrl = static_cast<uint32_t *>(ctx->one_ctl.p);
        KParams P{};
        char *const d = ctx->one_dev;
        P.blob = reinterpret_cast<const uint8_t *>(d), P.blob_bytes = img - 64;
        P.q_off = reinterpret_cast<const uint64_t *>(d + img - 64), P.t_off = P.q_off + 1;
        P.q_len = reinterpret_cast<const uint32_t *>(d + img - 48), P.t_len = P.q_len + 1;
        P.queue_head = d_ctrl + 0, P.redo_count = d_ctrl + 1, P.ops_cursor = reinterpret_cast<unsigned long long *>(d_ctrl + 2);
        P.redo_list = static_cast<uint32_t *>(ctx->redo.p);
        P.x = p->mismatch, P.o = p->gap_open, P.e = p->gap_ext, P.oe = p->gap_open + p->gap_ext, P.g = g;
        P.global_alignment = 1, P.adaptive = p->adaptive ? 1 : 0, P.min_wf_len = p->min_wf_len, P.max_dist_diff = p->max_dist_diff;
        P.rec = reinterpret_cast<uint32_t *>(d + ONE_REC_OFF);
        P.ops = reinterpret_cast<uint64_t *>(d + ONE_OPS_OFF), P.ops_cap = (ONE_PIN_BYTES - ONE_OPS_OFF) / 8;
        P.arena = static_cast<uint32_t *>(ctx->arena.p), P.arena_words = words, P.compact_fmt = WFA_BLK_TILED ? 3u : 1u;
        P.pair_meta = static_cast<uint4 *>(ctx->meta.p);
        P.dx = P.x / g, P.doe = P.oe / g, P.de = 1, P.dm = std::max(P.dx, P.doe) + 1, P.di = 2, P.min_xe = min_xe;
        P.lds_seq_words = seq_words, P.chunk_first = 0, P.chunk_n = 1, P.n_work = 1;
        const uint32_t lds_off   = ((uint32_t)seq_words * 2u + 4u + 31u) & ~31u;
        const uint64_t lds_rows  = std::min<uint64_t>((worst / g + 16 + 7) & ~7ull, ((160u * 1024u - lds_off * 4u) / 256u) & ~7u);
        bool           use_lds   = ctx->opt_pair_fast == 1 && ctx->opt_pair_lds != 0 && ctx->one_lds_skip == 0 && lds_rows >= 64;
        if (ctx->one_lds_skip) ctx->one_lds_skip--;
        uint32_t launches = 0;
        for (;;) {
            hrec[REC_STATUS] = ST_PENDING;
            if (!(ctx->opt_pair_fast == 1 && ctx->one_ctl_clean)) HIP_TRY(hipMemsetAsync(d_ctrl, 0, 1024, st));
            ctx->one_ctl_clean = false;
            if (ctx->opt_pair_fast == 2) {
                HIP_TRY(wfa_launch_fwd(0, K_BLK16, 0u, P, 1u, (size_t)seq_words * 2 * 4 * 4 + 16, st));
                HIP_TRY(wfa_launch_backtrace_one(P, st));
                launches += 2;
            } else if (ctx->opt_pair_fast == 1) {
                P.fuse_bt = 1;
                if (use_lds) {
// ... 98 lines not shown
```

### wfa_amd/csrc/wfa_host.hip

```cpp
#include <map>
#include "wfa_ctx.hpp"
#include "wfa_bound.hpp"
#include "wfa_ladder.hpp"
#include "wfa_generic.hpp"
#include "wfa_packed.hpp"
#include "wfa_reg.hpp"
#include "wfa_blk.hpp"
#include "wfa_duo_cfg.hpp"
#include "wfa_lane.hpp"
#include "wfa_team.hpp"
#include "wfa_teamc.hpp"
#include "wfa_fwd.hpp"
#include "wfa_long.hpp"
#include "wfa_wide.hpp"
#include "wfa_wide_plan.hpp"

using namespace wfa;
static_assert(TEAM_SOLO_MAX == 4096, "wfa_ctx.hpp: default of opt_team_solo_max");

namespace wfa {
hipError_t wfa_launch_fwd(int shape, int kind, uint32_t flags, const KParams &P, uint32_t grid, size_t lds_bytes, hipStream_t st) {
    switch (shape) {
#define WFA_FWD_CASE(I, tag, DX_, DOE_) \
    case I: return wfa_launch_fwd_##tag(kind, flags, P, grid, lds_bytes, st);
// ... 194 lines not shown
    switch (code) {
    case WFAHIP_OK: return "ok";
    case WFAHIP_ERR_NO_DEVICE: return "no HIP device available";
    case WFAHIP_ERR_BAD_ARG: return "bad argument";
    case WFAHIP_ERR_OOM: return "out of memory (device or ops buffer)";
    case WFAHIP_ERR_HIP: return "HIP runtime error";
    case WFAHIP_ERR_UNSUPPORTED: return "unsupported penalties (mismatch and gap_open + gap_ext must be > 0) or input";
    case WFAHIP_ERR_INTERNAL: return "internal error";
    }
    return "unknown error";
}

extern "C" int wfahip_device_count(void) {
    int n = 0;
    if (hipGetDeviceCount(&n) != hipSuccess) return 0;
    return n;
}

static int create_impl(int device_id, wfahip_ctx **out) {
    if (!out) return WFAHIP_ERR_BAD_ARG;
    *out = nullptr;
    int n = wfahip_device_count();
    if (n <= 0) return WFAHIP_ERR_NO_DEVICE;
    int dev = device_id;
    if (dev < 0 && hipGetDevice(&dev) != hipSuccess) return WFAHIP_ERR_NO_DEVICE;
    if (dev >= n) return WFAHIP_ERR_BAD_ARG;
    wfahip_ctx *ctx = new wfahip_ctx();
    ctx->device     = dev;
    if (hipSetDevice(dev) != hipSuccess) {
        delete ctx;
        return WFAHIP_ERR_HIP;
    }
    hipDeviceProp_t prop;
    if (hipGetDeviceProperties(&prop, dev) == hipSuccess) {
        ctx->num_cus   = prop.multiProcessorCount;
        ctx->total_mem = prop.totalGlobalMem;
    }
    if (hipStreamCreateWithFlags(&ctx->stream, hipStreamNonBlocking) != hipSuccess ||
        hipStreamCreateWithFlags(&ctx->stream2, hipStreamNonBlocking) != hipSuccess ||
        hipEventCreate(&ctx->ev0) != hipSuccess || hipEventCreate(&ctx->ev1) != hipSuccess ||
        hipEventCreate(&ctx->evA) != hipSuccess || hipEventCreate(&ctx->evB) != hipSuccess ||
        hipEventCreate(&ctx->evC) != hipSuccess || hipEventCreate(&ctx->evBtA) != hipSuccess ||
        hipEventCreate(&ctx->evBtB) != hipSuccess || hipEventCreateWithFlags(&ctx->ctrl_clean_ev, hipEventDisableTiming) != hipSuccess ||
        hipHostMalloc(reinterpret_cast<void **>(&ctx->hpin), HPIN_WORDS * 4, hipHostMallocDefault) != hipSuccess) {
        wfahip_destroy(ctx);
        return WFAHIP_ERR_HIP;
    }
    *out = ctx;
    return WFAHIP_OK;
}

extern "C" int wfahip_create(int device_id, wfahip_ctx **out) { WFAHIP_GUARD(create_impl(device_id, out)) }

extern "C" void wfahip_destroy(wfahip_ctx *ctx) {
    if (!ctx) return;
    (void)hipSetDevice(ctx->device);
    if (ctx->hpin) (void)hipHostFree(ctx->hpin);
    if (ctx->one_pin) (void)hipHostFree(ctx->one_pin);
    if (ctx->pack_pin) (void)hipHostFree(ctx->pack_pin);
    if (ctx->mx_pin) (void)hipHostFree(ctx->mx_pin);
    for (hipEvent_t e : ctx->mx_ev)
        if (e) (void)hipEventDestroy(e);
    if (ctx->stream_up) (void)hipStreamDestroy(ctx->stream_up);
    if (ctx->stream_dn) (void)hipStreamDestroy(ctx->stream_dn);
    for (hipEvent_t e : ctx->ev_up) (void)hipEventDestroy(e);
    for (int i = 0; i < 2; i++) {
        if (ctx->pin[i]) (void)hipHostFree(ctx->pin[i]);
        if (ctx->pin_ev[i]) (void)hipEventDestroy(ctx->pin_ev[i]);
    }
    for (DevBuf *b : {&ctx->arena, &ctx->fin, &ctx->team_ctl, &ctx->arena2, &ctx->meta2, &ctx->doneq, &ctx->ctrl, &ctx->redo, &ctx->work, &ctx->meta, &ctx->in_blob, &ctx->in_qoff, &ctx->in_qlen,
                      &ctx->in_toff, &ctx->in_tlen, &ctx->out_rec, &ctx->out_ops, &ctx->in_packed, &ctx->in_small, &ctx->prepack, &ctx->one_ctl, &ctx->page_ctl, &ctx->xbuf, &ctx->wide_ckpt, &ctx->score_out,
                      &ctx->mx_seq, &ctx->mx_words, &ctx->mx_out, &ctx->sd_ctl, &ctx->sd_blk, &ctx->sd_list, &ctx->sd_redo, &ctx->sd_words, &ctx->wide_ids, &ctx->wide_blk,
                      &ctx->wide_ctl, &ctx->in_rc, &ctx->rc_jobs, &ctx->cig, &ctx->cig_text, &ctx->cig_off, &ctx->pkd})
        release(*b);
    if (ctx->ev0) (void)hipEventDestroy(ctx->ev0);
    if (ctx->ev1) (void)hipEventDestroy(ctx->ev1);
    if (ctx->evA) (void)hipEventDestroy(ctx->evA);
    if (ctx->evB) (void)hipEventDestroy(ctx->evB);
    if (ctx->evC) (void)hipEventDestroy(ctx->evC);
    if (ctx->evBtA) (void)hipEventDestroy(ctx->evBtA);
    if (ctx->evBtB) (void)hipEventDestroy(ctx->evBtB);
    if (ctx->ctrl_clean_ev) (void)hipEventDestroy(ctx->ctrl_clean_ev);
    for (hipEvent_t e : ctx->evpool) (void)hipEventDestroy(e);
    if (ctx->stream) (void)hipStreamDestroy(ctx->stream);
    if (ctx->stream2) (void)hipStreamDestroy(ctx->stream2);
    delete ctx;
}

static bool public_option(const std::string &k) {
    static const char *const keys[] = {"census", "learn", "mem_limit", "arena_budget_pct", "autopack", "pair_fast", "pair_lds"};
    for (const char *p : keys)
        if (k == p) return true;
    return false;
}

static int set_option_impl(wfahip_ctx *ctx, const char *key, int64_t value) {
    if (!ctx || !key) return WFAHIP_ERR_BAD_ARG;
    std::string k(key);
    if (!public_option(k)) {
        const char *dbg = std::getenv("WFAHIP_DEBUG");
        if (!dbg || !*dbg || std::strcmp(dbg, "0") == 0) {
            std::snprintf(ctx->last_error, sizeof ctx->last_error, "option \"%.60s\" is a debug / experiment knob: set WFAHIP_DEBUG=1 in the environment to use it", key);
            return WFAHIP_ERR_UNSUPPORTED;
        }
    }
    if (k == "arena_bytes_per_slot")
        ctx->opt_arena_bytes_per_slot = value;
    else if (k == "slots")
        ctx->opt_slots = value;
    else if (k == "threads_per_pair")
        ctx->opt_threads_per_pair = value;
    else if (k == "packed")
        ctx->opt_packed = value;
    else if (k == "reg")
        ctx->opt_reg = value;
    else if (k == "blk")
        ctx->opt_blk = (value == 8 || value == 16) ? value : 0;
    else if (k == "blk_batch")
        ctx->opt_blk_batch = value;
    else if (k == "packed_arena_bytes")
        ctx->opt_packed_arena_bytes = value;
    else if (k == "chunk_pairs")
        ctx->opt_chunk_pairs = value;
    else if (k == "packed_waves_per_cu")
        ctx->opt_packed_waves_per_cu = value;
    else if (k == "overlap")
        ctx->opt_overlap = value;
    else if (k == "tail_overlap")
        ctx->opt_tail_overlap = value;
    else if (k == "blk_wide")
        ctx->opt_blk_wide = value;
    else if (k == "blk_narrow")
        ctx->opt_blk_narrow = value;
    else if (k == "bt_stream")
        ctx->opt_bt_stream = value;
    else if (k == "bt_stream_min")
        ctx->opt_bt_stream_min = value;
    else if (k == "bt_stream_single")
// ... 32 lines not shown
        ctx->opt_team_slack = value > 0 ? value : 1;
    else if (k == "arena_poison")
        ctx->opt_arena_poison = value;
    else if (k == "fail_pass")
        ctx->opt_fail_pass = value;
    else if (k == "prepack")
        ctx->opt_prepack = value;
    else if (k == "narrow_long")
        ctx->opt_narrow_long = value;
    else if (k == "census")
        ctx->opt_census = value;
    else if (k == "long")
        ctx->opt_long = value;
    else if (k == "long_first")
        ctx->opt_long_first = value;
    else if (k == "long_wave_bt_pairs")
        ctx->opt_long_wave_bt_pairs = value;
    else if (k == "long_mid_lone")
        ctx->opt_long_mid_lone = value;
    else if (k == "pair_lds")
        ctx->opt_pair_lds = value, ctx->one_lds_skip = 0;
    else if (k == "long_wave_bt")
        ctx->opt_long_wave_bt = value;
    else if (k == "long_min_len")
        ctx->opt_long_min_len = value;
    else if (k == "long_window_words")
        ctx->opt_long_window_words = (value >= 64 && value <= 4096 && value % 4 == 0) ? value : 240;
    else if (k == "wide")
        ctx->opt_wide = value;
    else if (k == "wide_min_pairs")
        ctx->opt_wide_min_pairs = value;
    else if (k == "wide_bin_min_pairs")
        ctx->opt_wide_bin_min_pairs = value;
    else if (k == "wide_classes")
        ctx->opt_wide_classes = value;
    else if (k == "matrix_tile_cells")
        ctx->opt_matrix_tile_cells = value > 0 ? value : 0;
    else if (k == "score_long_min")
        ctx->opt_score_long_min = value > 0 ? value : 1;
    else if (k == "score_long_window_words")
        ctx->opt_score_long_window = value;
    else if (k == "wide_max_len")
        ctx->opt_wide_max_len = value;
    else if (k == "wide_exact")
        ctx->opt_wide_exact = value != 0;
    else if (k == "wide_waves")
        ctx->opt_wide_waves = (value == 1 || value == 4) ? (int)value : 0;
    else if (k == "duo")
        ctx->opt_duo = value;
    else if (k == "duo_pk")
        ctx->opt_duo_pk = value != 0;
    else if (k == "duo_claim")
        ctx->opt_duo_claim = (value >= 1 && value <= DUO_CLAIM_MAX) ? value : 0;
    else if (k == "duo_min_pairs")
        ctx->opt_duo_min_pairs = value;
    else if (k == "compact_call_bases")
        ctx->opt_compact_call_bases = value;
    else if (k == "lane")
        ctx->opt_lane = value;
    else if (k == "lane_pack")
        ctx->opt_lane_pack = value;
    else if (k == "lane_min_pairs")
        ctx->opt_lane_min_pairs = value;
    else if (k == "duo_short")
        ctx->opt_duo_short = value;
    else if (k == "duo_short_min_pairs")
        ctx->opt_duo_short_min_pairs = value;
    else if (k == "blk_mid")
        ctx->opt_blk_mid = value;
    else if (k == "pair_fast")
        ctx->opt_pair_fast = value;
    else if (k == "arena_budget_pct")
        ctx->opt_arena_budget_pct = value;
    else if (k == "autopack")
        ctx->opt_autopack = value;
    else if (k == "learn")
        ctx->opt_learn = value, ctx->learn_key = 0;
    else if (k == "mem_limit") {
        ctx->opt_mem_limit = value;
        hipDeviceProp_t prop;
        if (value > 0)
            ctx->total_mem = (size_t)value;
        else if (hipGetDeviceProperties(&prop, ctx->device) == hipSuccess)
            ctx->total_mem = prop.totalGlobalMem;
    }
    else
        return WFAHIP_ERR_BAD_ARG;
    return WFAHIP_OK;
}

extern "C" int wfahip_set_option(wfahip_ctx *ctx, const char *key, int64_t value) { WFAHIP_GUARD(set_option_impl(ctx, key, value)) }

extern "C" int wfahip_last_timing(const wfahip_ctx *ctx, wfahip_timing *out) {
    if (!ctx || !out) return WFAHIP_ERR_BAD_ARG;
    *out = ctx->timing;
    return WFAHIP_OK;
}

extern "C" void wfahip_free(void *p) { std::free(p); }

extern "C" const char *wfahip_last_error(const wfahip_ctx *ctx) { return ctx ? ctx->last_error : ""; }

extern "C" int wfahip_wide_class_bounds(uint32_t *bounds, int cap) {
    for (int c = 0; bounds && c < WIDE_N_CLASSES && c < cap; c++) bounds[c] = wide_class_bound(c);
    return WIDE_N_CLASSES;
}

static int debug_wide_plan_impl(wfahip_ctx *ctx, const uint32_t *q_len, const uint32_t *t_len, uint64_t n_pairs, uint32_t **ids, uint64_t *counts,
                                uint32_t *longest, uint64_t *n_ladder) {
    *ids = nullptr, *n_ladder = 0;
    for (int c = 0; c < WIDE_N_CLASSES; c++) counts[c] = 0, longest[c] = 0;
    if (n_pairs > 0xFFFFFFF0ull) return WFAHIP_ERR_BAD_ARG;
    if (n_pairs == 0) return WFAHIP_OK;
    HIP_TRY(hipSetDevice(ctx->device));
    hipStream_t    st    = ctx->stream;
    const uint32_t tiles = (uint32_t)((n_pairs + WP_TILE - 1) / WP_TILE);
    int rc;
    if ((rc = ensure(ctx, ctx->in_qlen, n_pairs * 4))) return rc;
    if ((rc = ensure(ctx, ctx->in_tlen, n_pairs * 4))) return rc;
    if ((rc = ensure(ctx, ctx->wide_ctl, WPC_WORDS * 4))) return rc;
    if ((rc = ensure(ctx, ctx->wide_blk, (size_t)WP_CATS * tiles * 4))) return rc;
    if ((rc = ensure(ctx, ctx->wide_ids, n_pairs * 4))) return rc;
    HIP_TRY(hipMemcpyAsync(ctx->in_qlen.p, q_len, n_pairs * 4, hipMemcpyHostToDevice, st));
    HIP_TRY(hipMemcpyAsync(ctx->in_tlen.p, t_len, n_pairs * 4, hipMemcpyHostToDevice, st));
    WPParams S{};
    S.q_len = static_cast<const uint32_t *>(ctx->in_qlen.p), S.t_len = static_cast<const uint32_t *>(ctx->in_tlen.p), S.n = n_pairs, S.tiles = tiles;
    S.blk = static_cast<uint32_t *>(ctx->wide_blk.p), S.ctl = static_cast<uint32_t *>(ctx->wide_ctl.p), S.ids = static_cast<uint32_t *>(ctx->wide_ids.p);
    HIP_TRY(wfa_launch_wide_plan(S, st));
    HIP_TRY(hipStreamSynchronize(st));
    uint32_t pc[WPC_WORDS];
    HIP_TRY(hipMemcpy(pc, S.ctl, sizeof pc, hipMemcpyDeviceToHost));
    uint32_t *h = static_cast<uint32_t *>(std::malloc((size_t)n_pairs * 4));
    if (!h) return WFAHIP_ERR_OOM;
    if (hipMemcpy(h, S.ids, n_pairs * 4, hipMemcpyDeviceToHost) != hipSuccess) {
        std::free(h);
        return WFAHIP_ERR_HIP;
    }
    for (int c = 0; c < WIDE_N_CLASSES; c++) counts[c] = pc[WPC_COUNT + c], longest[c] = pc[WPC_LONGEST + c];
    *n_ladder = pc[WPC_COUNT + WIDE_N_CLASSES], *ids = h;
    return WFAHIP_OK;
}

extern "C" int wfahip_debug_wide_plan(wfahip_ctx *ctx, const uint32_t *q_len, const uint32_t *t_len, uint64_t n_pairs, uint32_t **ids, uint64_t *counts,
                                      uint32_t *longest, uint64_t *n_ladder) {
    if (!ctx || !q_len || !t_len || !ids || !counts || !longest || !n_ladder) return WFAHIP_ERR_BAD_ARG;
    WFAHIP_GUARD(debug_wide_plan_impl(ctx, q_len, t_len, n_pairs, ids, counts, longest, n_ladder))
}

static int align_device_impl(wfahip_ctx *ctx, const wfahip_params *p, const void *d_blob, uint64_t blob_bytes,
                             const void *d_q_off, const void *d_q_len, const void *d_t_off, const void *d_t_len,
                             uint64_t n_pairs, uint32_t max_len, void *d_rec, void *d_ops, uint64_t ops_cap,
                             uint64_t *ops_needed, hipStream_t st, bool debug_single, uint64_t ops_cursor0) {
    int rc = check_params(p);
    if (rc != WFAHIP_OK) return rc;
    if (n_pairs > 0xFFFFFFF0ull) return WFAHIP_ERR_BAD_ARG;
    ctx->timing = wfahip_timing{};
    ctx->dbg_arena = nullptr, ctx->dbg_n = 0;
    if (ctx->bt_pending) {
        (void)hipStreamSynchronize(ctx->stream2);
        ctx->bt_pending = false;
    }
    if (ops_needed) *ops_needed = 0;
    if (n_pairs == 0) return WFAHIP_OK;
    if (!d_q_off || !d_q_len || !d_t_off || !d_t_len || !d_rec || (!d_ops && ops_cap)) return WFAHIP_ERR_BAD_ARG;
    HIP_TRY(hipSetDevice(ctx->device));
    if (!st) st = ctx->stream;

    std::vector<uint32_t> ql, tl;
    const auto host_lens = [&]() -> int {
        if (!ql.empty()) return WFAHIP_OK;
        ql.resize(n_pairs), tl.resize(n_pairs);
        HIP_TRY(hipMemcpyAsync(ql.data(), d_q_len, n_pairs * 4, hipMemcpyDeviceToHost, st));
        HIP_TRY(hipMemcpyAsync(tl.data(), d_t_len, n_pairs * 4, hipMemcpyDeviceToHost, st));
        HIP_TRY(hipStreamSynchronize(st));
        return WFAHIP_OK;
    };
    const auto grow_evpool = [&](uint64_t n) -> int {
        while (ctx->evpool.size() < n) {
            hipEvent_t e;
            HIP_TRY(hipEventCreate(&e));
            ctx->evpool.push_back(e);
        }
        return WFAHIP_OK;
    };
    if (max_len == 0) {
        if ((rc = host_lens())) return rc;
        for (uint64_t i = 0; i < n_pairs; i++) {
            if (ql[i] <= WFAHIP_MAX_SEQ_LEN) max_len = std::max(max_len, ql[i]);
            if (tl[i] <= WFAHIP_MAX_SEQ_LEN) max_len = std::max(max_len, tl[i]);
        }
        if (max_len == 0) max_len = 1;
    }

    rc = ensure(ctx, ctx->ctrl, CTRL_WORDS * 4);
    if (rc) return rc;
    rc = ensure(ctx, ctx->redo, n_pairs * 8);
    if (rc) return rc;
    uint32_t *d_ctrl = static_cast<uint32_t *>(ctx->ctrl.p);
    bool     ctrl_zeroed = true, ctrl_fresh = false;
    uint32_t hc_last[CTRL_WORDS] = {0};
    const auto fetch_ctrl = [&](uint32_t *hc, std::vector<uint64_t> *ent) -> int {
        HIP_TRY(hipMemcpyAsync(ctx->hpin + HPIN_CTRL, d_ctrl, CTRL_WORDS * 4, hipMemcpyDeviceToHost, st));
        const size_t head = std::min<size_t>(HPIN_REDO_ENT * 8, ctx->redo.bytes);
        const bool with_head = ent && !ctx->redo_was_empty;
        if (with_head) HIP_TRY(hipMemcpyAsync(ctx->hpin + HPIN_REDO, ctx->redo.p, head, hipMemcpyDeviceToHost, st));
        HIP_TRY(hipStreamSynchronize(st));
        std::memcpy(hc, ctx->hpin + HPIN_CTRL, CTRL_WORDS * 4);
        if (ent) {
            if (!with_head && hc[1] != 0u) {
                HIP_TRY(hipMemcpyAsync(ctx->hpin + HPIN_REDO, ctx->redo.p, head, hipMemcpyDeviceToHost, st));
                HIP_TRY(hipStreamSynchronize(st));
            }
            ctx->redo_was_empty = hc[1] == 0u;
            const size_t n = hc[1], nh = std::min<size_t>(n, head / 8);
// ... 236 lines not shown
            first = false, packed_done = true;
        }
    }
    if (!packed_done && ctx->opt_packed && !debug_single && ctx->force_mode < 0 && P.global_alignment && P.e != 0u) {
        const uint32_t dx = P.x / P.g, doe = P.oe / P.g, de = P.e / P.g;
        const uint32_t dm = std::max(dx, doe) + 1, di = de + 1;
        constexpr uint32_t SUB_LEN_LIMIT = 10200;
        uint32_t           sub_len       = max_len;
        const int  shape    = fwd_shape(dx, doe, de);
        const bool can_long = ctx->opt_long != 0 && ctx->opt_blk == 16 && shape >= 0 && (int64_t)max_len > ctx->opt_long_min_len;
        if (max_len > SUB_LEN_LIMIT && n_pairs >= 256) {
            if ((rc = host_lens())) return rc;
            uint64_t n_fit = 0;
            uint32_t best  = 0;
            for (uint64_t i = 0; i < n_pairs; i++) {
                const uint32_t l = std::max(ql[i], tl[i]);
                if (l <= SUB_LEN_LIMIT) n_fit++, best = std::max(best, l);
            }
            if (n_fit * 10 >= n_pairs * 9 && best > 0) sub_len = best, sub_len_used = best;
        }
        const bool     long_first = can_long && sub_len_used == 0;
        const uint32_t seq_words = (sub_len + 15) / 16 + 1;
        const uint64_t sub_words = packed_sub_lds_words(seq_words, dm, di);
        const size_t   lds_b     = (size_t)sub_words * 2 * 4;
        const size_t   lds_c     = (size_t)seq_words * 2 * 4 * 4;
        const size_t   lds_d     = (size_t)seq_words * 2 * 4 * (ctx->opt_blk == 8 ? 8 : 4) + 16;
        const bool     can_b     = lds_b <= 20 * 1024;
        const bool     can_c     = ctx->opt_reg && dx == 2 && doe == 4 && de == 1 && lds_c <= 20 * 1024;
        const bool     can_d     = long_first || (ctx->opt_blk && shape >= 0 && (shape == 0 || ctx->opt_blk == 16) && sub_len < 32768 &&
                                                lds_d <= (ctx->opt_blk == 8 ? 40 : 20) * 1024);
        const auto words_dir_of = [&](uint32_t len) {
            uint64_t wd = std::max<uint64_t>(1024, 8ull * len);
            if (ctx->opt_packed_arena_bytes > 0) wd = std::max<uint64_t>(1024, ctx->opt_packed_arena_bytes / 4);
            return (wd + 7) & ~7ull;
        };
        struct PassClass {
            uint32_t seq_words;
            uint64_t words_dir;
        };
        const PassClass batch_class{seq_words, words_dir_of(sub_len)};
        P.arena_words   = batch_class.words_dir;
        P.dx = dx, P.doe = doe, P.de = de, P.dm = dm, P.di = di;
        P.lds_seq_words = seq_words;
        P.sub_lds_words = (uint32_t)sub_words;
        P.min_xe        = std::min(P.x, P.e);
#ifdef WFA_STAMPS
        static DevBuf stampbuf;
        if ((rc = ensure(ctx, stampbuf, 192))) return rc;
        HIP_TRY(hipMemsetAsync(stampbuf.p, 0, 192, st));
        P.debug_info = static_cast<uint32_t *>(stampbuf.p);
#endif
        const uint64_t rkey = class_key;
        const uint64_t arena_mult = (ctx->rows_key == rkey && ctx->opt_packed_arena_bytes <= 0) ? ctx->rows_scale : 1;
        auto forward_pass = [&](Kind kind, const std::vector<uint32_t> *list, uint64_t first_pair, uint64_t count, std::vector<uint64_t> &redo_out,
                                bool detach_bt, const PassClass *cls = nullptr, uint64_t rows_mult = 0) -> int {
            const uint32_t seq_words = (cls ? cls : &batch_class)->seq_words;
            const uint64_t words_dir = (cls ? cls : &batch_class)->words_dir;
            if (rows_mult == 0) rows_mult = arena_mult;
            const KindTraits &T = kind_traits(kind);
            const bool second = ctx->bt_pending || (list && ctx->arena.bytes <= ctx->total_mem / 10);
            DevBuf &arena_buf = second ? ctx->arena2 : ctx->arena;
            DevBuf &meta_buf  = second ? ctx->meta2 : ctx->meta;
            const bool     blk_batch    = (kind == K_BLK16 || kind == K_NARROW) && seq_words <= 16 && ctx->opt_blk_batch != 0;
            if (kind == K_NARROW && !blk_batch && ctx->opt_narrow_long == 0) return WFAHIP_ERR_INTERNAL;
            if (ctx->opt_fail_pass == kind) return WFAHIP_ERR_OOM;
            const uint32_t even_sw      = (seq_words + 1u) & ~1u, duo_pw = 4u + 2u * even_sw;
            if (kind == K_DUO && (duo_pw > 256u || blk_batch)) return WFAHIP_ERR_INTERNAL;
            if (kind == K_LANE && (seq_words > (uint32_t)LN_SEQ_WORDS || list)) return WFAHIP_ERR_INTERNAL;
            const bool     is_long      = T.windows != 0;
            const uint32_t long_sw      = (seq_words + 3u) & ~3u, long_cw = (uint32_t)ctx->opt_long_window_words;
            if (is_long && !can_long) return WFAHIP_ERR_INTERNAL;
            if (is_long && (uint64_t)seq_words * 16u < (uint64_t)max_len && !list) return WFAHIP_ERR_INTERNAL;
            size_t lds_bytes = (size_t)seq_words * 2 * 4 * T.pairs_wave + 16;
            if (is_long) lds_bytes = (size_t)T.windows * 2 * long_cw * 4;
            else if (blk_batch) lds_bytes = (size_t)T.pairs_wave * BLK_BATCH * (2 * seq_words + 8) * 4 + 16;
            else if (kind == K_PACKED) lds_bytes = lds_b;
            else if (kind == K_REG) lds_bytes = lds_c;
            else if (kind == K_BLK16 || kind == K_BLK8) lds_bytes = lds_d;
            else if (kind == K_DUO) lds_bytes = (size_t)duo_lds_words(duo_pw) * 4;
            else if (kind == K_LANE) lds_bytes = (size_t)64 * lane_stride_words(even_sw) * 4;
            const uint64_t words_free   = T.pitch ? std::max<uint64_t>((words_dir * T.rows_mult * rows_mult + 511) & ~511ull, T.words_min) : words_dir;
            const uint64_t words        = bound_cap_words(words_free, T.pitch, T.words_min, P.max_score, P.g);
            const bool     bound_final  = bound_covers(words, T.pitch, P.max_score, P.g);
            P.arena_words = words, P.compact_fmt = compact_fmt_of((Kind)T.base);
            const uint32_t waves_lds    = (uint32_t)std::min<size_t>(32, LDS_MAX_BYTES / lds_bytes);
            const bool     overlap      = ctx->opt_overlap != 0;
            uint32_t       waves_per_cu = std::min<uint32_t>(waves_lds, waves_cap(kind, P.census != 0, overlap));
            if (ctx->opt_packed_waves_per_cu > 0)
                waves_per_cu = std::min<uint32_t>(waves_lds, (uint32_t)ctx->opt_packed_waves_per_cu);
            const uint64_t resident = (uint64_t)T.pairs_wave * ctx->num_cus * waves_per_cu;
            uint64_t budget = (uint64_t)((double)ctx->total_mem * 0.35) / (overlap ? 2 : 1);
            uint64_t chunk  = std::max<uint64_t>(1, std::min<uint64_t>(count, budget / (words * 4ull)));
            if (overlap && count >= 8 * resident) chunk = std::min<uint64_t>(chunk, (count + 7) / 8);
            if (ctx->opt_chunk_pairs > 0) chunk = std::min<uint64_t>(chunk, (uint64_t)ctx->opt_chunk_pairs);
            const uint64_t n_chunks = (count + chunk - 1) / chunk;
            const uint32_t n_buf    = (overlap && n_chunks > 1) ? 2 : 1;
            const uint64_t chunk_alloc = list ? std::max<uint64_t>(chunk, std::min<uint64_t>(chunk + chunk / 4 + 64, budget / (words * 4ull))) : chunk;
            int rc2 = WFAHIP_OK;
            if (arena_buf.bytes < (size_t)(words * 4ull * chunk * n_buf)) {
                rc2 = ensure(ctx, arena_buf, (size_t)(words * 4ull * chunk_alloc * n_buf));
                if (rc2 == WFAHIP_ERR_OOM && chunk_alloc > chunk) rc2 = ensure(ctx, arena_buf, (size_t)(words * 4ull * chunk * n_buf));
            }
            if (rc2) return rc2;
            if (meta_buf.bytes < chunk * 16 * n_buf && (rc2 = ensure(ctx, meta_buf, chunk_alloc * 16 * n_buf))) return rc2;
            detach_bt = detach_bt && n_chunks == 1 && ctx->opt_tail_overlap != 0 &&
                        (count * (uint64_t)max_len > (uint64_t)ctx->opt_compact_call_bases || ctx->opt_compact_call_bases <= 0);
            ctrl_fresh = false;
            const bool stream_bt = kind == K_BLK16 && shape == 0 && !blk_batch && n_buf == 1 && ctx->opt_bt_stream > 0 && (int64_t)chunk >= ctx->opt_bt_stream_min &&
                                   ctx->opt_bt_stream_single != 0;
            P.done_q = nullptr, P.done_ctl = nullptr, P.n_stream_wgs = 0;
            if (stream_bt) {
                if ((rc2 = ensure(ctx, ctx->doneq, 256 + 16 * chunk))) return rc2;
                P.done_ctl = static_cast<uint32_t *>(ctx->doneq.p);
                P.done_q   = reinterpret_cast<uint4 *>(static_cast<char *>(ctx->doneq.p) + 256);
            }
            ctx->timing.arena_bytes = std::max<uint64_t>(ctx->timing.arena_bytes, words * 4ull * chunk * n_buf);
            if (list && (rc2 = upload_work(list->data(), count))) return rc2;
            if ((rc2 = grow_evpool(4 * n_chunks))) return rc2;
            if (!ctrl_zeroed) HIP_TRY(hipMemsetAsync(d_ctrl, 0, 8, st));
            ctrl_zeroed = false;
            hipStream_t st_bt = (n_buf == 2 || detach_bt) ? ctx->stream2 : st;
            for (uint64_t c = 0; c < n_chunks; c++) {
                const uint64_t c0 = c * chunk, cn = std::min<uint64_t>(chunk, count - c0);
                hipEvent_t evFa = ctx->evpool[4 * c], evFb = ctx->evpool[4 * c + 1];
                hipEvent_t evBa = detach_bt ? ctx->evBtA : ctx->evpool[4 * c + 2];
                hipEvent_t evBb = detach_bt ? ctx->evBtB : ctx->evpool[4 * c + 3];
                const uint32_t buf = (uint32_t)(c % n_buf);
                P.arena       = static_cast<uint32_t *>(arena_buf.p) + (uint64_t)buf * chunk * words;
                P.pair_meta   = static_cast<uint4 *>(meta_buf.p) + (uint64_t)buf * chunk;
                P.chunk_first = (uint32_t)(first_pair + c0), P.chunk_n = (uint32_t)cn;
                P.work        = list ? static_cast<const uint32_t *>(ctx->work.p) + c0 : nullptr;
                if (!list && c == 0 && first_pair == 0)
                    ctx->dbg_arena = P.arena, ctx->dbg_meta = P.pair_meta, ctx->dbg_words = words, ctx->dbg_first = first_pair,
                    ctx->dbg_n = cn, ctx->dbg_fmt = P.compact_fmt, ctx->dbg_g = P.g;
                uint32_t grid = (uint32_t)std::min<uint64_t>((uint64_t)ctx->num_cus * waves_per_cu,
                                                            (cn + T.pairs_wave - 1) / T.pairs_wave);
                const uint32_t n_bt = stream_bt ? (uint32_t)std::min<int64_t>(ctx->opt_bt_stream, grid / 4) : 0u;
                if (stream_bt) {
                    if (grid < (uint32_t)ctx->num_cus * waves_per_cu) grid = std::min<uint32_t>(grid + n_bt, (uint32_t)ctx->num_cus * waves_per_cu);
                    P.n_stream_wgs = n_bt;
                    P.stream_wait  = (uint32_t)std::min<int64_t>(std::max<int64_t>(ctx->opt_bt_stream_wait_us, 0) * 100, 0x7FFFFFFF);
                    HIP_TRY(hipMemsetAsync(ctx->doneq.p, 0, 256 + 16 * cn, st));
                    HIP_TRY(hipMemsetAsync(P.pair_meta, 0xFF, 16 * cn, st));
                }
                P.prepack = nullptr, P.prepack_words = 0;
                P.lds_seq_words = is_long ? long_sw : (kind == K_LANE || kind == K_DUO) ? even_sw : seq_words;
                if (kind == K_LANE) P.sub_lds_words = lane_stride_words(even_sw);
                if ((kind == K_BLK16 && !blk_batch && !list && ctx->opt_prepack != 0) || kind == K_DUO || (kind == K_LANE && ctx->opt_lane_pack == 0) || is_long) {
                    const uint32_t pw = 4u + 2u * P.lds_seq_words;
                    if ((rc2 = ensure(ctx, ctx->prepack, (size_t)chunk * pw * 4))) return rc2;
                    if (ctx->pk_words)
                        hipLaunchKernelGGL(wfa_prepack_words_kernel, dim3((uint32_t)((cn + 3) / 4)), dim3(256), 0, st, P, ctx->pk_words,
                                           static_cast<uint32_t *>(ctx->prepack.p), P.lds_seq_words, pw);
                    else {
                        const uint32_t ppw = (cn <= (uint64_t)ctx->num_cus * 64 && 2u * P.lds_seq_words > 32u) ? 1u : (uint32_t)PREPACK_PAIRS;
                        HIP_TRY(wfa_launch_prepack(P, static_cast<uint32_t *>(ctx->prepack.p), P.lds_seq_words, ppw, st));
                    }
                    HIP_TRY(hipGetLastError());
                    P.prepack = static_cast<const uint32_t *>(ctx->prepack.p), P.prepack_words = pw;
                } else if (ctx->pk_words) {
                    hipLaunchKernelGGL(wfa_unpack_pairs_kernel, dim3((uint32_t)((cn + 3) / 4)), dim3(256), 0, st, P, ctx->pk_words,
                                       const_cast<uint8_t *>(P.blob));
                    HIP_TRY(hipGetLastError());
                }
                if (is_long) P.lds_seq_words = long_cw;
                if (n_buf == 2 && c >= 2) HIP_TRY(hipStreamWaitEvent(st, ctx->evpool[4 * (c - 2) + 3], 0));
                if (c > 0) HIP_TRY(hipMemsetAsync(d_ctrl, 0, 4, st));
                if (ctx->opt_arena_poison) HIP_TRY(hipMemsetAsync(P.arena, 0xA5, (size_t)(words * 4ull * cn), st));
                HIP_TRY(hipEventRecord(evFa, st));
                if (kind == K_DUO) {
                    if (grid > 0xFFFFu || T.pairs_wave != 8) return WFAHIP_ERR_INTERNAL;
                    P.duo_claim = ctx->opt_duo_claim > 0 ? (uint32_t)ctx->opt_duo_claim : (uint32_t)DUO_CLAIM;
                    HIP_TRY(wfa_launch_duo(shape, P, grid, lds_bytes, st, P.census != 0, ctx->opt_duo_pk));
                } else if (kind != K_REG && kind != K_PACKED) {
                    uint32_t fl = (P.census ? (uint32_t)FWD_CENSUS : 0u) | (P.adaptive ? (uint32_t)FWD_ADAPTIVE : 0u);
                    if (stream_bt) fl |= FWD_STREAM;
                    if (blk_batch) {
                        const uint64_t groups = (uint64_t)ctx->num_cus * 16 * T.pairs_wave;
                        const uint64_t share  = (cn + groups - 1) / groups;
                        const uint64_t rounds = (share + BLK_BATCH - 1) / BLK_BATCH;
                        P.blk_batch_n = (uint32_t)std::min<uint64_t>(BLK_BATCH, std::max<uint64_t>(1, (share + rounds - 1) / std::max<uint64_t>(1, rounds)));
                        if (ctx->opt_blk_batch > 1) P.blk_batch_n = (uint32_t)std::min<int64_t>(BLK_BATCH, ctx->opt_blk_batch);
                        fl |= FWD_BATCH;
                    }
                    HIP_TRY(wfa_launch_fwd(shape, kind, fl, P, grid, lds_bytes, st));
                } else if (kind == K_REG)
                    hipLaunchKernelGGL((wfa_reg_kernel<2, 4, 1>), dim3(grid), dim3(64), lds_bytes, st, P);
                else
                    hipLaunchKernelGGL(wfa_packed_kernel, dim3(grid), dim3(64), lds_bytes, st, P);
                HIP_TRY(hipGetLastError());
                HIP_TRY(hipEventRecord(evFb, st));
                if (st_bt != st) HIP_TRY(hipStreamWaitEvent(st_bt, evFb, 0));
                if (st_bt != st) HIP_TRY(hipEventRecord(evBa, st_bt));
                if (is_long && (ctx->opt_long_wave_bt >= 2 || (ctx->opt_long_wave_bt == 1 && cn <= (ctx->opt_long_wave_bt_pairs ? (uint64_t)ctx->opt_long_wave_bt_pairs : (uint64_t)ctx->num_cus * 20))))
                    hipLaunchKernelGGL(wfa_backtrace_wave_kernel, dim3((uint32_t)((cn + BTW_WAVES - 1) / BTW_WAVES)), dim3(64 * BTW_WAVES), 0, st_bt, P);
                else
                    hipLaunchKernelGGL(wfa_backtrace_kernel, dim3((uint32_t)((cn + BT_THREADS - 1) / BT_THREADS)), dim3(BT_THREADS), 0, st_bt, P);
                HIP_TRY(hipGetLastError());
                HIP_TRY(hipEventRecord(evBb, st_bt));
            }
            if (st_bt != st && !detach_bt)
                for (uint64_t c = (n_chunks >= 2 ? n_chunks - 2 : 0); c < n_chunks; c++)
                    HIP_TRY(hipStreamWaitEvent(st, ctx->evpool[4 * c + 3], 0));
            uint32_t hc[CTRL_WORDS];
            if (bound_final) {
                hipLaunchKernelGGL(wfa_bound_redo_kernel, dim3((uint32_t)std::min<uint64_t>((count + 255) / 256, 1024)), dim3(256), 0, st, P.redo_list, P.redo_count, P.rec);
                HIP_TRY(hipGetLastError());
            }
            if (!detach_bt) HIP_TRY(hipEventRecord(ctx->ev1, st));
            if ((rc2 = fetch_ctrl(hc, &redo_out))) return rc2;
            if (bound_final) redo_out.erase(std::remove_if(redo_out.begin(), redo_out.end(), [](uint64_t e) { return (uint32_t)(e >> 32) == ST_OVER_MAX; }), redo_out.end());
            if (detach_bt) ctx->bt_pending = true;
            else ctrl_fresh = true, std::memcpy(hc_last, hc, sizeof hc_last);
            for (uint64_t c = 0; c < n_chunks; c++) {
                float msF = 0, msB = 0;
                HIP_TRY(hipEventElapsedTime(&msF, ctx->evpool[4 * c], ctx->evpool[4 * c + 1]));
                if (!detach_bt) HIP_TRY(hipEventElapsedTime(&msB, ctx->evpool[4 * c + (st_bt != st ? 2 : 1)], ctx->evpool[4 * c + 3]));
                ctx->timing.kernel_ms += msF + msB;
                if (!list) ctx->timing.main_kernel_ms += msF, ctx->timing.n_main_launches++;
                ctx->timing.n_launches += 2;
            }
            P.work = nullptr;
            P.lds_seq_words = seq_words;
            P.sub_lds_words = (uint32_t)sub_words;
            return WFAHIP_OK;
        };

        if (can_b || can_c || can_d) {
            std::vector<uint64_t> redo1, redo2;
            const bool narrow1 = can_d && ctx->opt_blk == 16 && ctx->opt_blk_narrow != 0 &&
                                 ((ctx->opt_blk_batch != 0 && max_len < 200 && seq_words <= 16) ||
                                  (ctx->opt_narrow_long != 0 && shape == 0 && (size_t)seq_words * 2 * 4 * 8 + 16 <= 8 * 1024));
            const bool duo_long  = !narrow1 && seq_words > 16 &&
                                   (ctx->opt_duo >= 2 || (ctx->opt_duo == 1 && (int64_t)n_pairs >= ctx->opt_duo_min_pairs));
            const bool duo_short = seq_words <= 16 && ctx->opt_duo != 0 &&
                                   (ctx->opt_duo_short >= 2 || (ctx->opt_duo_short == 1 && (int64_t)n_pairs >= ctx->opt_duo_short_min_pairs));
            const bool duo1    = can_d && ctx->opt_blk == 16 && (duo_long || duo_short) && 4u + 2u * ((seq_words + 1u) & ~1u) <= 256u;
            const bool lane1   = can_d && ctx->opt_blk == 16 && seq_words <= (uint32_t)LN_SEQ_WORDS &&
                                 (ctx->opt_lane >= 2 || (ctx->opt_lane == 1 && (int64_t)n_pairs >= ctx->opt_lane_min_pairs));
            const Kind kind1   = long_first ? K_LONG16 : (duo1 && duo_short) ? K_DUO : lane1 ? K_LANE : duo1 ? K_DUO : narrow1 ? K_NARROW : (can_d ? (ctx->opt_blk == 8 ? K_BLK8 : K_BLK16) : (can_c ? K_REG : K_PACKED));
            const Kind kind_mid = long_first ? K_LONG32 : K_BLK32, kind_wide = long_first ? K_LONG64 : K_BLK64, kind_64 = long_first ? K_LONG16 : K_BLK16;
            uint64_t done_pairs = 0;
            bool     skip_rest  = false;
            Kind     kind_rest  = kind1;
            const bool rows1    = kind_traits(kind1).pitch != 0;
            const bool wide_ok  = rows1 && ctx->opt_blk_wide != 0;
            std::vector<uint64_t> redo_w;
            const auto is_band = [](uint32_t s) { return s == ST_REDO_BAND; };
// ... 329 lines not shown
        ctx->timing.kernel_ms += ms;
        if (first) {
            ctx->timing.main_kernel_ms = ms, ctx->timing.n_main_launches = 1, first = false;
            if (team) ctx->timing.main_kernel_kind = pl.kind;
            after_scout = pl.scout_now;
        } else if (after_scout && teamc) {
            ctx->timing.main_kernel_ms += ms, ctx->timing.n_main_launches++;
        }
        ctx->timing.n_launches++;

        const uint32_t n_redo = hctrl[1];
        if (learn_track) {
            if (team_total == 0) team_total = n_work;
            team_done += n_work - n_redo;
            if (learned_now < 0 && 10 * team_done >= 9 * team_total) learned_now = job.level;
        }
        if (n_redo) {
            Job jb, ja, jw;
            jb.mode = 1, jb.level = job.level, jb.all = false, jb.max_len = job.max_len;
            ja.mode = job.mode, ja.level = job.level + 1, ja.all = false, ja.max_len = job.max_len;
            jw.mode = job.mode, jw.level = job.level, jw.all = false, jw.max_len = job.max_len, jw.hint = job.hint;
            for (uint32_t i = 0; i < n_redo; i++) {
                const uint32_t stw = (uint32_t)(ent[i] >> 32);
                (stw == ST_REDO_WIDE ? jw : (stw == ST_REDO_BYTES || stw == ST_REDO_LDS ? jb : ja)).pairs.push_back((uint32_t)ent[i]);
            }
            if (ctx->timing.main_kernel_kind != K_WIDE) ctx->timing.n_retried_pairs += n_redo - (uint32_t)jw.pairs.size();
            if (!jw.pairs.empty()) jobs.push_front(std::move(jw));
            if (!jb.pairs.empty()) jobs.push_back(std::move(jb));
            if (!ja.pairs.empty()) jobs.push_back(std::move(ja));
        }
        if (debug_single) break;
    }
    if (learned_now >= 0) {
        if (ctx->learn_key != lkey || ctx->learn_level != learned_now) ctx->learn_calls = 0;
        ctx->learn_key = lkey, ctx->learn_level = learned_now;
    }
    if (ctx->bt_pending) HIP_TRY(hipStreamWaitEvent(st, ctx->evBtB, 0));
    if (!no_memory.empty() || ctx->bt_pending || P.max_score != 0u) ctrl_fresh = false;
    if (P.max_score != 0u) {
        hipLaunchKernelGGL(wfa_bound_filter_kernel, dim3((uint32_t)((n_pairs + 255) / 256)), dim3(256), 0, st, P.rec, n_pairs, P.max_score);
        HIP_TRY(hipGetLastError());
    }
    if (!ctrl_fresh) HIP_TRY(hipEventRecord(ctx->ev1, st));

    for (uint32_t pid : no_memory) {
        uint32_t recw[REC_WORDS] = {0};
        recw[REC_STATUS]         = ST_NO_MEMORY;
        HIP_TRY(hipMemcpyAsync(P.rec + (uint64_t)pid * REC_WORDS, recw, sizeof recw, hipMemcpyHostToDevice, st));
    }
    uint32_t hctrl[CTRL_WORDS];
    if (ctrl_fresh) std::memcpy(hctrl, hc_last, sizeof hctrl);
    else if ((rc = fetch_ctrl(hctrl, nullptr))) return rc;
    float ms = 0;
    if (ctx->bt_pending) {
        HIP_TRY(hipEventElapsedTime(&ms, ctx->evBtA, ctx->evBtB));
        ctx->timing.kernel_ms += ms;
        ctx->bt_pending = false;
    }
    HIP_TRY(hipEventElapsedTime(&ms, ctx->ev0, ctx->ev1));
    ctx->timing.total_ms    = ms;
    const uint64_t cursor   = (uint64_t)hctrl[2] | ((uint64_t)hctrl[3] << 32);
    ctx->timing.ops_written = cursor;
    if (ops_needed) *ops_needed = cursor;
    if (!debug_single && hipMemsetAsync(d_ctrl, 0, CTRL_WORDS * 4, st) == hipSuccess && hipEventRecord(ctx->ctrl_clean_ev, st) == hipSuccess)
        ctx->ctrl_clean = true, ctx->ctrl_clean_stream = st;
    else if (!debug_single)
        (void)hipStreamSynchronize(st);
    if (cursor > ops_cap) {
        if (std::getenv("WFAHIP_DEBUG_TIMING")) std::fprintf(stderr, "[wfahip] CIGAR op buffer too small: %llu needed, %llu there\n", (unsigned long long)cursor, (unsigned long long)ops_cap);
        return WFAHIP_ERR_OOM;
    }
    return WFAHIP_OK;
}

int align_device(wfahip_ctx *ctx, const wfahip_params *p, const void *d_blob, uint64_t blob_bytes,
                        const void *d_q_off, const void *d_q_len, const void *d_t_off, const void *d_t_len,
                        uint64_t n_pairs, uint32_t max_len, void *d_rec, void *d_ops, uint64_t ops_cap,
                        uint64_t *ops_needed, hipStream_t st, bool debug_single, uint64_t ops_cursor0) {
    WFAHIP_GUARD(align_device_impl(ctx, p, d_blob, blob_bytes, d_q_off, d_q_len, d_t_off, d_t_len, n_pairs, max_len, d_rec, d_ops,
                                   ops_cap, ops_needed, st, debug_single, ops_cursor0))
}

extern "C" int wfahip_align_batch_device(wfahip_ctx *ctx, const wfahip_params *p, const void *d_seq_blob,
                                         uint64_t blob_bytes, const void *d_q_off, const void *d_q_len,
                                         const void *d_t_off, const void *d_t_len, uint64_t n_pairs,
                                         uint32_t max_len, void *d_rec, void *d_ops, uint64_t ops_cap,
                                         uint64_t *ops_needed, void *stream) {
    if (!ctx) return WFAHIP_ERR_BAD_ARG;
    return align_device(ctx, p, d_seq_blob, blob_bytes, d_q_off, d_q_len, d_t_off, d_t_len, n_pairs, max_len,
                        d_rec, d_ops, ops_cap, ops_needed, static_cast<hipStream_t>(stream), false);
}

extern "C" int wfahip_align_batch_bounded_device(wfahip_ctx *ctx, const wfahip_params *p, const void *d_seq_blob,
                                                 uint64_t blob_bytes, const void *d_q_off, const void *d_q_len,
                                                 const void *d_t_off, const void *d_t_len, uint64_t n_pairs,
                                                 uint32_t max_len, uint32_t max_score, void *d_rec, void *d_ops, uint64_t ops_cap,
                                                 uint64_t *ops_needed, void *stream) {
    if (!ctx || !p) return WFAHIP_ERR_BAD_ARG;
    BoundScope bound(ctx, max_score);
    return align_device(ctx, p, d_seq_blob, blob_bytes, d_q_off, d_q_len, d_t_off, d_t_len, n_pairs, max_len,
                        d_rec, d_ops, ops_cap, ops_needed, static_cast<hipStream_t>(stream), false);
}

hipError_t wfa_launch_prepack(const wfa::KParams &P, uint32_t *out, uint32_t SW, uint32_t ppw, hipStream_t st) {
    if (SW == 0u || ppw == 0u || ppw > 32u || P.chunk_n == 0u) return hipErrorInvalidValue;
    hipLaunchKernelGGL(wfa_prepack_kernel, dim3((uint32_t)(((uint64_t)P.chunk_n + 4u * ppw - 1u) / (4u * ppw))), dim3(256), 0, st, P, out, SW, 4u + 2u * SW, ppw);
    return hipGetLastError();
// ... 8 lines not shown
```

### wfa_amd/csrc/wfa_packed.hpp

```cpp
#pragma once
#include <type_traits>
#include "wfa_device.hpp"

namespace wfa {

#ifdef WFA_STAMPS
#define WFA_STAMP(i)                                                                                  \
    do {                                                                                              \
        unsigned long long _t;                                                                        \
        __builtin_amdgcn_sched_barrier(0);                                                            \
        asm volatile("s_memtime %0\n\ts_waitcnt lgkmcnt(0)" : "=s"(_t)::"memory");                   \
        __builtin_amdgcn_sched_barrier(0);                                                            \
        stamp_acc[i] += _t - stamp_prev;                                                              \
        stamp_prev = _t;                                                                              \
    } while (0)
#else
#define WFA_STAMP(i) \
    do {             \
    } while (0)
#endif

constexpr int PK_G     = 32;
constexpr int PK_TILES = 2;
constexpr int PK_WCAP  = PK_G * PK_TILES;
// ... 194 lines not shown
                    ringM[cm * PK_WCAP + r] = cM[t], ringI[ce * PK_WCAP + r] = cI[t], ringD[ce * PK_WCAP + r] = cD[t];
                    my_cells += (cM[t] != 0u) + (cI[t] != 0u) + (cD[t] != 0u);
                }
            }
            if (j == 0) {
                metaM[2 * cm] = nlo, metaM[2 * cm + 1] = wn;
                metaE[2 * ce] = nlo, metaE[2 * ce + 1] = wn;
                *reinterpret_cast<uint4 *>(A + cap - 4ull * (si + 1)) =
                    wn > 0 ? make_uint4(top, (uint32_t)nlo, (uint32_t)wn, 0u) : make_uint4(0u, 0u, 0u, 0u);
            }
            top += (uint32_t)wn;
        }
        WFA_STAMP(4);
        if (give_up || (run && term)) {
            const uint32_t cells = sub_sum(my_cells);
            int            hf    = 0;
#pragma unroll
            for (int t = 0; t < PK_TILES; t++)
                if (lo + PK_G * t + j == Ak) hf = (int)(cM[t] >> TAG_BITS);
            hf = -sub_min(-hf);
            if (j == 0) {
                if (give_up) {
                    P.pair_meta[pidx] = make_uint4(too_wide ? ST_REDO_BAND : ST_REDO_ARENA, 0u, 0u, 0u);
                    push_redo(P, pair, too_wide ? ST_REDO_BAND : ST_REDO_ARENA);
                } else {
                    P.pair_meta[pidx] = make_uint4(ST_OK, s, (uint32_t)hf, cells);
                }
            }
            st = 0;
        } else if (run) {
            s += g, si += 1u;
            cm = (cm + 1u == DM) ? 0u : cm + 1u;
            ce = (ce + 1u == DI) ? 0u : ce + 1u;
        }
        __builtin_amdgcn_fence(__ATOMIC_RELEASE, "wavefront");
        __builtin_amdgcn_fence(__ATOMIC_ACQUIRE, "wavefront");
        WFA_STAMP(5);
    }
#ifdef WFA_STAMPS
    if (lane == 0 && P.debug_info) {
        unsigned long long *acc = reinterpret_cast<unsigned long long *>(P.debug_info);
        for (int i = 0; i < 8; i++) atomicAdd(acc + i, stamp_acc[i]);
    }
#endif
}

#endif

WFA_DEV uint32_t ops_bound(const KParams &P, uint32_t s_final) {
    return (2u * (s_final / P.min_xe) + (P.global_alignment ? 8u : 12u) + OpsWriterRev::GROUP - 1u) & ~(OpsWriterRev::GROUP - 1u);
}

constexpr uint64_t OPS_OFF_OWN = ~0ull;
WFA_DEV void backtrace_one(const KParams &P, uint32_t idx, uint32_t s_final, uint32_t h_end, uint32_t cells, bool coherent,
                           uint64_t off_given = OPS_OFF_OWN) {
    const uint32_t  pair = P.work ? P.work[idx] : P.chunk_first + idx;
    uint32_t *const rec  = P.rec + (uint64_t)pair * REC_WORDS;
    const int       n = (int)P.q_len[pair], m = (int)P.t_len[pair];
    CompactView cv;
    cv.A = P.arena + (uint64_t)idx * P.arena_words, cv.cap = P.arena_words, cv.g = P.g, cv.n_ent = s_final / P.g + 1u;
    cv.fmt = P.compact_fmt, cv.coherent = coherent;

    const uint32_t bound = ops_bound(P, s_final);
    const uint64_t off   = off_given != OPS_OFF_OWN ? off_given : atomicAdd(P.ops_cursor, (unsigned long long)bound);
    OpsWriterRev   ow;
    const bool     fits = off + bound <= P.ops_cap;
    ow.init(P.ops + off, fits ? bound : 0u);
    TraceOut to;
    if (P.compact_fmt == 11u)
        back_trace_compact(cv, n, m, s_final, (int)(h_end >> 16) - 32768, h_end & 0xFFFFu, P.x, P.o, P.e, ow, to, P.global_alignment == 0u);
    else
        back_trace_compact(cv, n, m, s_final, m - n, h_end, P.x, P.o, P.e, ow, to);
    ow.finish();
    const uint64_t first = off + bound - ow.n;
    uint4 *r4            = reinterpret_cast<uint4 *>(rec);
    r4[0] = make_uint4(ST_OK, to.score, (uint32_t)to.tbegin, (uint32_t)to.tend);
    r4[1] = make_uint4((uint32_t)to.qbegin, (uint32_t)to.qend, ow.alen, ow.matches);
    r4[2] = make_uint4(ow.gaps, ow.regions, ow.n, (uint32_t)first);
    r4[3] = make_uint4((uint32_t)(first >> 32), cells, 0u, s_final);
}

constexpr int BT_THREADS = 512;
template <bool LDSV = false>
WFA_DEV void backtrace_wave_one(const KParams &P, uint32_t idx_, uint32_t *region) {
    const auto     rfl  = [](uint32_t x) { return (uint32_t)__builtin_amdgcn_readfirstlane((int)x); };
    const uint32_t lane = threadIdx.x & 63u;
    const uint32_t idx  = rfl(idx_);
    uint4          meta;
    if constexpr (LDSV) {
        meta = *reinterpret_cast<const uint4 *>(region - 4);
        if (rfl(meta.x) != ST_OK) meta = P.pair_meta[idx];
    } else {
        meta = P.pair_meta[idx];
    }
    meta = make_uint4(rfl(meta.x), rfl(meta.y), rfl(meta.z), rfl(meta.w));
    const uint32_t pair = rfl(P.work ? P.work[idx] : P.chunk_first + idx);
    uint4 *const   r4   = reinterpret_cast<uint4 *>(P.rec + (uint64_t)pair * REC_WORDS);
    if (meta.x != ST_OK) {
        if ((LDSV || meta.x < ST_REDO_BYTES) && lane == 0u) {
            const uint4 z = make_uint4(0u, 0u, 0u, 0u);
            r4[0] = make_uint4(meta.x, 0u, 0u, 0u), r4[1] = z, r4[2] = z, r4[3] = z;
        }
        return;
    }
    const uint32_t s_final = meta.y, h_end = meta.z, cells = meta.w;
    const int      n = LDSV ? (int)P.one_n : (int)rfl(P.q_len[pair]), m = LDSV ? (int)P.one_m : (int)rfl(P.t_len[pair]);
    const uint32_t bound = ops_bound(P, s_final);
    unsigned long long off = 0ull;
    if constexpr (!LDSV) {
        if (lane == 0u) off = atomicAdd(P.ops_cursor, (unsigned long long)bound);
        off = ((unsigned long long)(uint32_t)__builtin_amdgcn_readfirstlane((int)(uint32_t)(off >> 32)) << 32) |
              (uint32_t)__builtin_amdgcn_readfirstlane((int)(uint32_t)off);
    }
    typename std::conditional<LDSV, CompactViewLds, CompactViewWave>::type cv;
    if constexpr (LDSV) {
        cv.A = region, cv.g = P.g, cv.n_ent = s_final / P.g + 1u;
    } else {
        cv.A = P.arena + (uint64_t)idx * P.arena_words, cv.cap = P.arena_words, cv.g = P.g, cv.n_ent = s_final / P.g + 1u;
        cv.fmt = P.compact_fmt, cv.reg = region;
    }
    OpsWriterRev ow;
    const bool   fits = off + bound <= P.ops_cap;
    ow.combine = false;
    ow.init(P.ops + off, fits ? bound : 0u);
    ow.active = lane == 0u;
    TraceOut to;
    back_trace_compact(cv, n, m, s_final, m - n, h_end, P.x, P.o, P.e, ow, to);
    ow.finish();
    if (lane == 0u) {
        const uint64_t first = off + bound - ow.n;
        r4[0] = make_uint4(ST_OK, to.score, (uint32_t)to.tbegin, (uint32_t)to.tend);
        r4[1] = make_uint4((uint32_t)to.qbegin, (uint32_t)to.qend, ow.alen, ow.matches);
        r4[2] = make_uint4(ow.gaps, ow.regions, ow.n, (uint32_t)first);
        r4[3] = make_uint4((uint32_t)(first >> 32), cells, 0u, s_final);
    }
}

#ifndef WFA_NO_AUX_KERNELS
__global__ __launch_bounds__(BT_THREADS) void wfa_backtrace_kernel(const KParams P) {
    __shared__ uint32_t           wsum[BT_THREADS / 64];
    __shared__ unsigned long long wbase;
    const uint32_t idx  = blockIdx.x * blockDim.x + threadIdx.x;
    const bool     have = idx < P.chunk_n;
    uint4          meta = make_uint4(ST_PENDING, 0u, 0u, 0u);
    if (have) meta = P.pair_meta[idx];
    if (have && meta.x != ST_OK && meta.x < ST_REDO_BYTES) {
        const uint32_t pair = P.work ? P.work[idx] : P.chunk_first + idx;
        const uint4    z    = make_uint4(0u, 0u, 0u, 0u);
        uint4 *r4           = reinterpret_cast<uint4 *>(P.rec + (uint64_t)pair * REC_WORDS);
        r4[0] = make_uint4(meta.x, 0u, 0u, 0u), r4[1] = z, r4[2] = z, r4[3] = z;
    }
    bool     walk = have && meta.x == ST_OK;
    uint32_t slot = idx, s_final = meta.y, h_end = meta.z, cells = meta.w;
    if (P.done_q) {
        const uint4 e = have ? P.done_q[idx] : make_uint4(0u, 0u, 0u, 0u);
        walk = e.x != 0u && e.x != DONE_TAKEN && (e.x & DONE_NOT_OK) == 0u;
        slot = e.x - 1u, s_final = e.y, h_end = e.z, cells = e.w;
    }
    const uint32_t bound = walk ? ops_bound(P, s_final) : 0u;
    const uint32_t lane = threadIdx.x & 63u, wv = threadIdx.x >> 6;
    uint32_t       incl = bound;
#pragma unroll
    for (int d = 1; d < 64; d <<= 1) {
        const uint32_t up = __shfl_up(incl, d, 64);
        if ((int)lane >= d) incl += up;
    }
    if (lane == 63u) wsum[wv] = incl;
    __syncthreads();
    if (threadIdx.x == 0) {
        unsigned long long tot = 0;
        for (uint32_t w = 0; w < blockDim.x / 64u; w++) tot += wsum[w];
        wbase = tot ? atomicAdd(P.ops_cursor, tot) : 0ull;
    }
    __syncthreads();
    uint64_t off = wbase + (incl - bound);
    for (uint32_t w = 0; w < wv; w++) off += wsum[w];
    if (walk) backtrace_one(P, slot, s_final, h_end, cells, false, off);
}


constexpr int BTW_WAVES = 4;
__global__ __launch_bounds__(64 * BTW_WAVES) void wfa_backtrace_wave_kernel(const KParams P) {
    __shared__ __attribute__((aligned(16))) uint32_t region[BTW_WAVES][CompactViewWave::WORDS];
    const uint32_t wv  = threadIdx.x >> 6;
    const uint32_t idx = blockIdx.x * (uint32_t)BTW_WAVES + wv;
    if (idx >= P.chunk_n) return;
    backtrace_wave_one(P, idx, region[wv]);
}
#endif

WFA_DEV void stream_backtrace(const KParams &P) {
    const int      lane = threadIdx.x;
    uint32_t *const ctl = P.done_ctl;
    for (;;) {
        uint32_t base = 0u;
        if (lane == 0) base = atomicAdd(ctl + 1, 64u);
        base = (uint32_t)__builtin_amdgcn_readfirstlane((int)base);
        if (base >= P.chunk_n) break;
        const uint32_t idx   = base + (uint32_t)lane;
        const bool     valid = idx < P.chunk_n;
        uint32_t *const ew   = reinterpret_cast<uint32_t *>(P.done_q + idx);
        bool            ok   = !valid;
        const uint64_t  t0   = wall_clock64();
        bool            late = false;
        for (;;) {
            if (!ok) ok = __hip_atomic_load(ew, __ATOMIC_RELAXED, __HIP_MEMORY_SCOPE_AGENT) != 0u;
            if (__ballot(!ok) == 0ull) break;
            __builtin_amdgcn_s_sleep(32);
            if (wall_clock64() - t0 > (uint64_t)P.stream_wait) {
                late = true;
                break;
            }
        }
        if (late) break;
        if (valid) {
            const uint32_t ex = __hip_atomic_load(ew + 0, __ATOMIC_RELAXED, __HIP_MEMORY_SCOPE_AGENT);
            const uint32_t ey = __hip_atomic_load(ew + 1, __ATOMIC_RELAXED, __HIP_MEMORY_SCOPE_AGENT);
            const uint32_t ez = __hip_atomic_load(ew + 2, __ATOMIC_RELAXED, __HIP_MEMORY_SCOPE_AGENT);
            const uint32_t e3 = __hip_atomic_load(ew + 3, __ATOMIC_RELAXED, __HIP_MEMORY_SCOPE_AGENT);
            if ((ex & DONE_NOT_OK) == 0u) backtrace_one(P, ex - 1u, ey, ez, e3, true);
            ew[0] = DONE_TAKEN;
        }
    }
}

}
```

Before: 76.04 million pairs/s.

## Segment duo forward pass so backtraces overlap with unfinished forward work

Splits the duo forward kernel's chunk into up to eight segments. Each wave counts its in-flight pairs per segment and raises a host-visible flag once every wave has moved past a segment, so backtrace kernels can start on a separate stream while the forward pass is still running. Backtrace lanes gain modes that skip pairs still pending and mark finished ones, followed by a cleanup launch. An optional slim backtrace kernel is also added, using fewer VGPRs and a smaller ops grouping. The costs are extra LDS atomics, a VGPR cap on the segmented kernel, and more launches and synchronisation.

New measurement: 75.78 million pairs/s. No clear change (-0.3%).

```diff
diff --git a/include/wfa_hip.h b/include/wfa_hip.h
--- a/include/wfa_hip.h
+++ b/include/wfa_hip.h
@@ -256,6 +256,7 @@
                                uint32_t *q_len, uint64_t *t_off, uint32_t *t_len);
 
 int      wfahip_debug_clock(wfahip_ctx *ctx, double *mhz, double *mhz_min, double *mhz_max);
+int      wfahip_debug_duo_segments(wfahip_ctx *ctx, uint32_t out[4]);
 int      wfahip_generate_pairs_device(wfahip_ctx *ctx, uint64_t seed, uint64_t first_index, uint64_t n_pairs, uint32_t length,
                                       double error_rate, void *d_blob, void *d_q_off, void *d_q_len, void *d_t_off,
                                       void *d_t_len, void *stream);
diff --git a/wfa_amd/_lib.py b/wfa_amd/_lib.py
--- a/wfa_amd/_lib.py
+++ b/wfa_amd/_lib.py
@@ -32,6 +32,7 @@
     "wfahip_pack_pairs_device", "wfahip_align_batch_packed_device",
     "wfahip_score_batch_packed_device", "wfahip_select_pairs_device",
     "wfahip_alignment_text_packed_device", "wfahip_alignment_text_packed",
+    "wfahip_debug_duo_segments",
 ]
 
 
@@ -189,6 +190,8 @@
         L.wfahip_submit.restype = C.c_int
         L.wfahip_submit.argtypes = [vp, C.c_char_p, u32, C.c_char_p, u32, C.POINTER(u64)]
         L.wfahip_pending.restype = u64
+        L.wfahip_debug_duo_segments.restype = C.c_int
+        L.wfahip_debug_duo_segments.argtypes = [vp, C.POINTER(C.c_uint32)]
         L.wfahip_debug_clock.restype = C.c_int
         L.wfahip_debug_clock.argtypes = [vp, C.POINTER(C.c_double), C.POINTER(C.c_double), C.POINTER(C.c_double)]
         L.wfahip_align_pair.restype = C.c_int
diff --git a/wfa_amd/aligner.py b/wfa_amd/aligner.py
--- a/wfa_amd/aligner.py
+++ b/wfa_amd/aligner.py
@@ -918,6 +918,11 @@
             L.lib().wfahip_free(words)
         return arr, int(fmt.value), tuple(int(x) for x in meta)
 
+    def debug_duo_segments(self):
+        out = (C.c_uint32 * 4)()
+        L.check(L.lib().wfahip_debug_duo_segments(self._ctx, out), "wfahip_debug_duo_segments")
+        return tuple(int(x) for x in out)
+
     def debug_wide_plan(self, q_len, t_len):
         q_len = np.ascontiguousarray(q_len, dtype=np.uint32)
         t_len = np.ascontiguousarray(t_len, dtype=np.uint32)
diff --git a/wfa_amd/csrc/wfa_common.hpp b/wfa_amd/csrc/wfa_common.hpp
--- a/wfa_amd/csrc/wfa_common.hpp
+++ b/wfa_amd/csrc/wfa_common.hpp
@@ -102,6 +102,13 @@
     uint64_t        mx_rc_shift;
     uint64_t        rc_top;
     const uint32_t *mx_rc_words;
+    uint32_t        seg_n, seg_len;
+    uint32_t       *seg_count;
+    uint32_t       *seg_flag;
+    uint32_t        bt_first, bt_n;
+    uint32_t        bt_mode;
+    uint32_t       *bt_skipped;
+    uint8_t        *bt_done;
 };
 
 }
diff --git a/wfa_amd/csrc/wfa_ctx.hpp b/wfa_amd/csrc/wfa_ctx.hpp
--- a/wfa_amd/csrc/wfa_ctx.hpp
+++ b/wfa_amd/csrc/wfa_ctx.hpp
@@ -172,6 +172,18 @@
     int64_t       opt_duo_min_pairs        = 200000;
     bool          opt_duo_pk               = true;
     int64_t       opt_duo_claim            = 0;
+    int64_t       opt_duo_seg              = 0;
+    int64_t       opt_duo_seg_len          = 0;
+    int64_t       opt_duo_seg_min_pairs    = 400000;
+    bool          opt_bt_slim              = false;
+    uint32_t     *seg_flags  = nullptr;
+    uint32_t     *seg_flags_dev = nullptr;
+    DevBuf        seg_ctl;
+    DevBuf        bt_done;
+    hipStream_t   stream_bt  = nullptr;
+    std::vector<hipEvent_t> seg_ev;
+    uint32_t      seg_ev_used = 0;
+    uint32_t      seg_S_last = 0, seg_early_last = 0, seg_launch_last = 0;
     int64_t       opt_duo_short            = 0;
     int64_t       opt_duo_short_min_pairs  = 50000;
     bool          ctrl_clean               = false;
diff --git a/wfa_amd/csrc/wfa_device.hpp b/wfa_amd/csrc/wfa_device.hpp
--- a/wfa_amd/csrc/wfa_device.hpp
+++ b/wfa_amd/csrc/wfa_device.hpp
@@ -361,7 +361,8 @@
 #ifndef WFA_OPS_GROUP
 #define WFA_OPS_GROUP 8
 #endif
-struct OpsWriterRev {
+template <uint32_t G>
+struct OpsWriterRevT {
     uint64_t *buf;
     uint32_t  cap;
     uint32_t  n;
@@ -371,7 +372,8 @@
     uint32_t  alen, matches, gaps, regions;
     uint32_t  p_len, p_gaps, p_regions;
     uint64_t  last;
-    static constexpr uint32_t GROUP = WFA_OPS_GROUP;
+    static constexpr uint32_t GROUP = G;
+    static_assert(G >= 1 && (G & (G - 1)) == 0 && WFA_OPS_GROUP % G == 0, "a power of two that divides the regions' alignment");
     uint64_t  hist[GROUP > 1 ? GROUP - 1 : 1];
     bool      grouped;
     bool      active = true;
@@ -441,6 +443,7 @@
         }
     }
 };
+using OpsWriterRev = OpsWriterRevT<WFA_OPS_GROUP>;
 
 struct CompactView {
     const uint32_t *A;
diff --git a/wfa_amd/csrc/wfa_duo.hip b/wfa_amd/csrc/wfa_duo.hip
--- a/wfa_amd/csrc/wfa_duo.hip
+++ b/wfa_amd/csrc/wfa_duo.hip
@@ -6,8 +6,13 @@
 
 namespace {
 template <int DX, int DOE>
-hipError_t go_duo(const KParams &P, uint32_t grid, size_t lds_bytes, hipStream_t st, bool census, bool pk) {
-    if (pk && census)
+hipError_t go_duo(const KParams &P, uint32_t grid, size_t lds_bytes, hipStream_t st, bool census, bool pk, bool seg) {
+    if (seg && !(pk && P.seg_n >= 1u && P.seg_n <= (uint32_t)DUO_SEG_MAX && P.seg_len >= 1u && P.seg_count && P.seg_flag)) return hipErrorInvalidValue;
+    if (seg && census)
+        hipLaunchKernelGGL((wfa_duo_seg_kernel<true, DX, DOE>), dim3(grid), dim3(64), lds_bytes, st, P);
+    else if (seg)
+        hipLaunchKernelGGL((wfa_duo_seg_kernel<false, DX, DOE>), dim3(grid), dim3(64), lds_bytes, st, P);
+    else if (pk && census)
         hipLaunchKernelGGL((wfa_duo_kernel<true, DX, DOE>), dim3(grid), dim3(64), lds_bytes, st, P);
     else if (pk)
         hipLaunchKernelGGL((wfa_duo_kernel<false, DX, DOE>), dim3(grid), dim3(64), lds_bytes, st, P);
@@ -19,10 +24,10 @@
 }
 }
 
-hipError_t wfa_launch_duo(int shape, const KParams &P, uint32_t grid, size_t lds_bytes, hipStream_t st, bool census, bool pk) {
+hipError_t wfa_launch_duo(int shape, const KParams &P, uint32_t grid, size_t lds_bytes, hipStream_t st, bool census, bool pk, bool seg) {
     switch (shape) {
 #define WFA_DUO_SHAPE(I, tag, DX_, DOE_) \
-    case I: return go_duo<DX_, DOE_>(P, grid, lds_bytes, st, census, pk);
+    case I: return go_duo<DX_, DOE_>(P, grid, lds_bytes, st, census, pk, seg);
         WFA_FWD_SHAPES(WFA_DUO_SHAPE)
 #undef WFA_DUO_SHAPE
     }
diff --git a/wfa_amd/csrc/wfa_duo.hpp b/wfa_amd/csrc/wfa_duo.hpp
--- a/wfa_amd/csrc/wfa_duo.hpp
+++ b/wfa_amd/csrc/wfa_duo.hpp
@@ -70,7 +70,7 @@
     return p;
 }
 
-template <bool CENSUS, int DX, int DOE, bool PK>
+template <bool CENSUS, int DX, int DOE, bool PK, bool SEG = false>
 __device__ __attribute__((always_inline)) inline void duo_run(const KParams &P) {
     constexpr int PP = 4;
     static_assert(DX >= 1 && DOE >= 1 && DX <= 4 && DOE <= 4, "ring depths of one to four score steps");
@@ -190,6 +190,43 @@
         else
             rowp = A->arena + (uint64_t)pidx * acap + (uint64_t)(si >> 3) * 256u + (si & 7u) * 2u;
     };
+    uint32_t *const seg_w = park0 + DUO_PARK * DUO_PARK_WORDS;
+    const auto seg_of = [&](const auto *A, uint32_t idx) { return umin2(idx / A->seg_len, A->seg_n - 1u); };
+    const auto seg_hold = [&](const auto *A, uint32_t idx, int d) {
+        if constexpr (SEG) __hip_atomic_fetch_add(seg_w + seg_of(A, idx), (uint32_t)d, __ATOMIC_RELAXED, __HIP_MEMORY_SCOPE_WAVEFRONT);
+    };
+    const auto seg_report = [&](bool dry) {
+        if constexpr (SEG) {
+            const auto *const A = args();
+            const uint32_t S = A->seg_n;
+            uint32_t nrep = 0u;
+            if (lane == 0) {
+                const uint32_t L = A->seg_len, cn = A->chunk_n;
+                const uint32_t cur = __hip_atomic_load(seg_w + DUO_SEG_MAX, __ATOMIC_RELAXED, __HIP_MEMORY_SCOPE_WAVEFRONT);
+                for (uint32_t s = cur; s < S; s++, nrep++) {
+                    const uint32_t end = s + 1u == S ? cn : umin2((s + 1u) * L, cn);
+                    if (!(dry || pf_next >= end) || __hip_atomic_load(seg_w + s, __ATOMIC_RELAXED, __HIP_MEMORY_SCOPE_WAVEFRONT) != 0u) break;
+                }
+            }
+            nrep = (uint32_t)__builtin_amdgcn_readfirstlane((int)nrep);
+            if (nrep != 0u) {
+                __builtin_amdgcn_fence(__ATOMIC_RELEASE, "agent");
+                asm volatile("s_waitcnt vmcnt(0)" ::: "memory");
+                if (lane == 0) {
+                    const uint32_t cur = __hip_atomic_load(seg_w + DUO_SEG_MAX, __ATOMIC_RELAXED, __HIP_MEMORY_SCOPE_WAVEFRONT);
+                    for (uint32_t s = cur; s < cur + nrep; s++)
+                        if (atomicAdd(A->seg_count + s, 1u) + 1u == (pf >> PF_GRID_SHIFT))
+                            __hip_atomic_store(A->seg_flag + s, 1u, __ATOMIC_RELAXED, __HIP_MEMORY_SCOPE_SYSTEM);
+                    __hip_atomic_store(seg_w + DUO_SEG_MAX, cur + nrep, __ATOMIC_RELAXED, __HIP_MEMORY_SCOPE_WAVEFRONT);
+                }
+            }
+        }
+    };
+    if constexpr (SEG) {
+        if (lane <= DUO_SEG_MAX) seg_w[lane] = 0u;
+        __builtin_amdgcn_fence(__ATOMIC_RELEASE, "wavefront");
+        __builtin_amdgcn_fence(__ATOMIC_ACQUIRE, "wavefront");
+    }
     const auto clear_rings = [&]() {
 #pragma unroll
         for (int d = 0; d < R; d++) {
@@ -260,6 +297,7 @@
                     const auto *const A = args();
                     A->pair_meta[this_idx] = make_uint4(status, 0u, 0u, 0u);
                     if (status >= ST_REDO_BYTES) redo(A, pair_of(A, this_idx), status);
+                    seg_hold(A, this_idx, -1);
                 }
                 buf_free = uni(buf_free | (1u << pf_buf));
                 continue;
@@ -322,9 +360,14 @@
                 const uint32_t cnt = umin2(FP, pf_end - pf_next);
                 pf_next += cnt;
                 if ((uint32_t)lane * 4u < cnt * PW) pf_w = *reinterpret_cast<const uint4 *>(slot + lane * 4);
+                if constexpr (SEG) {
+                    if (lane == 0)
+                        for (uint32_t c = 0; c < cnt; c++) seg_hold(A, pf_ld_idx + c, 1);
+                }
             }
             pf_next = uni(pf_next);
             pf = uni((pf & ~PF_TOK) | (have ? PF_LD : PF_DRY));
+            seg_report(!have);
         }
         if ((pf & (PF_TOK | PF_DRY)) == 0u) {
             if (pf_next >= pf_end) {
@@ -435,6 +478,7 @@
                     const auto *const A = args();
                     A->pair_meta[pidx] = make_uint4(ST_REDO_BAND, 0u, 0u, 0u);
                     redo(A, pair_of(A, pidx), ST_REDO_BAND);
+                    seg_hold(A, pidx, -1);
                 }
                 buf_free = uni(or_halves(act == 4 ? (1u << sbuf) : 0u) | buf_free);
                 if (act == 4) {
@@ -509,6 +553,7 @@
             set_derived();
             __builtin_amdgcn_fence(__ATOMIC_RELEASE, "wavefront");
             __builtin_amdgcn_fence(__ATOMIC_ACQUIRE, "wavefront");
+            seg_report((pf & PF_DRY) != 0u);
         }
         }
         WFA_STAMP(1);
@@ -884,6 +929,7 @@
                 } else {
                     A->pair_meta[pidx] = make_uint4(ST_OK, si * A->g, (uint32_t)hf, (uint32_t)ctot);
                 }
+                seg_hold(A, pidx, -1);
             }
             buf_free = uni(or_halves(fin ? (1u << sbuf) : 0u) | buf_free);
             if (fin) {
@@ -896,6 +942,7 @@
                 __builtin_amdgcn_fence(__ATOMIC_RELEASE, "wavefront");
                 __builtin_amdgcn_fence(__ATOMIC_ACQUIRE, "wavefront");
             }
+            seg_report((pf & PF_DRY) != 0u);
         }
         if constexpr (WFA_DUO_FILL == 0) {
             if (run && !fin) si += 1u;
@@ -921,6 +968,7 @@
             step(std::integral_constant<int, 3 % R>{});
         }
     }
+    seg_report(true);
 #ifdef WFA_STAMPS
     if (lane == 0 && P.debug_info) {
         unsigned long long *acc = reinterpret_cast<unsigned long long *>(P.debug_info);
@@ -938,6 +986,13 @@
 __global__ __launch_bounds__(64, WFA_DUO_WAVES) __attribute__((amdgpu_num_vgpr(WFA_DUO_VGPRS))) void wfa_duo_kernel(const KParams P) {
     duo_run<CENSUS, DX, DOE, true>(P);
 }
+#ifndef WFA_DUO_SEG_VGPRS
+#define WFA_DUO_SEG_VGPRS 56
+#endif
+template <bool CENSUS, int DX = 2, int DOE = 4>
+__global__ __launch_bounds__(64, WFA_DUO_WAVES) __attribute__((amdgpu_num_vgpr(WFA_DUO_SEG_VGPRS))) void wfa_duo_seg_kernel(const KParams P) {
+    duo_run<CENSUS, DX, DOE, true, true>(P);
+}
 template <bool CENSUS, int DX = 2, int DOE = 4>
 __global__ __launch_bounds__(64, WFA_DUO_WAVES) __attribute__((amdgpu_num_vgpr(WFA_DUO_VGPRS))) void wfa_duo32_kernel(const KParams P) {
     duo_run<CENSUS, DX, DOE, false>(P);
diff --git a/wfa_amd/csrc/wfa_duo_cfg.hpp b/wfa_amd/csrc/wfa_duo_cfg.hpp
--- a/wfa_amd/csrc/wfa_duo_cfg.hpp
+++ b/wfa_amd/csrc/wfa_duo_cfg.hpp
@@ -57,6 +57,14 @@
     return duo_bufs(prepack_words) * prepack_words + (uint32_t)DUO_PARK * DUO_PARK_WORDS;
 }
 
-hipError_t wfa_launch_duo(int shape, const KParams &P, uint32_t grid, size_t lds_bytes, hipStream_t st, bool census, bool pk);
+#ifndef WFA_DUO_SEG
+#define WFA_DUO_SEG 1
+#endif
+constexpr int DUO_SEG_DEFAULT   = WFA_DUO_SEG;
+constexpr int DUO_SEG_MAX       = 8;
+constexpr int DUO_SEG_LDS_WORDS = 16;
+static_assert(DUO_SEG_MAX + 1 <= DUO_SEG_LDS_WORDS, "a count per segment and the report cursor");
+
+hipError_t wfa_launch_duo(int shape, const KParams &P, uint32_t grid, size_t lds_bytes, hipStream_t st, bool census, bool pk, bool seg = false);
 
 }
diff --git a/wfa_amd/csrc/wfa_entry.hip b/wfa_amd/csrc/wfa_entry.hip
--- a/wfa_amd/csrc/wfa_entry.hip
+++ b/wfa_amd/csrc/wfa_entry.hip
@@ -930,6 +930,7 @@
         HIP_TRY(hipSetDevice(ctx->device));
         if (ctx->bt_pending) {
             (void)hipStreamSynchronize(ctx->stream2);
+            if (ctx->stream_bt) (void)hipStreamSynchronize(ctx->stream_bt);
             ctx->bt_pending = false;
         }
         if (!ctx->one_pin) {
diff --git a/wfa_amd/csrc/wfa_host.hip b/wfa_amd/csrc/wfa_host.hip
--- a/wfa_amd/csrc/wfa_host.hip
+++ b/wfa_amd/csrc/wfa_host.hip
@@ -270,6 +270,20 @@
 
 extern "C" int wfahip_create(int device_id, wfahip_ctx **out) { WFAHIP_GUARD(create_impl(device_id, out)) }
 
+static int debug_duo_segments_impl(wfahip_ctx *ctx, uint32_t *out) {
+    HIP_TRY(hipSetDevice(ctx->device));
+    HIP_TRY(hipStreamSynchronize(ctx->stream));
+    if (ctx->stream_bt) HIP_TRY(hipStreamSynchronize(ctx->stream_bt));
+    out[0] = ctx->seg_S_last, out[1] = ctx->seg_early_last, out[2] = 0u, out[3] = ctx->seg_launch_last;
+    if (ctx->seg_S_last && ctx->seg_ctl.p)
+        HIP_TRY(hipMemcpy(out + 2, static_cast<const uint32_t *>(ctx->seg_ctl.p) + DUO_SEG_MAX, 4, hipMemcpyDeviceToHost));
+    return WFAHIP_OK;
+}
+extern "C" int wfahip_debug_duo_segments(wfahip_ctx *ctx, uint32_t out[4]) {
+    if (!ctx || !out) return WFAHIP_ERR_BAD_ARG;
+    WFAHIP_GUARD(debug_duo_segments_impl(ctx, out))
+}
+
 extern "C" void wfahip_destroy(wfahip_ctx *ctx) {
     if (!ctx) return;
     (void)hipSetDevice(ctx->device);
@@ -289,7 +303,7 @@
     for (DevBuf *b : {&ctx->arena, &ctx->fin, &ctx->team_ctl, &ctx->arena2, &ctx->meta2, &ctx->doneq, &ctx->ctrl, &ctx->redo, &ctx->work, &ctx->meta, &ctx->in_blob, &ctx->in_qoff, &ctx->in_qlen,
                       &ctx->in_toff, &ctx->in_tlen, &ctx->out_rec, &ctx->out_ops, &ctx->in_packed, &ctx->in_small, &ctx->prepack, &ctx->one_ctl, &ctx->page_ctl, &ctx->xbuf, &ctx->wide_ckpt, &ctx->score_out,
                       &ctx->mx_seq, &ctx->mx_words, &ctx->mx_out, &ctx->sd_ctl, &ctx->sd_blk, &ctx->sd_list, &ctx->sd_redo, &ctx->sd_words, &ctx->wide_ids, &ctx->wide_blk,
-                      &ctx->wide_ctl, &ctx->in_rc, &ctx->rc_jobs, &ctx->cig, &ctx->cig_text, &ctx->cig_off, &ctx->pkd})
+                      &ctx->wide_ctl, &ctx->in_rc, &ctx->rc_jobs, &ctx->cig, &ctx->cig_text, &ctx->cig_off, &ctx->pkd, &ctx->seg_ctl, &ctx->bt_done})
         release(*b);
     if (ctx->ev0) (void)hipEventDestroy(ctx->ev0);
     if (ctx->ev1) (void)hipEventDestroy(ctx->ev1);
@@ -302,6 +316,9 @@
     for (hipEvent_t e : ctx->evpool) (void)hipEventDestroy(e);
     if (ctx->stream) (void)hipStreamDestroy(ctx->stream);
     if (ctx->stream2) (void)hipStreamDestroy(ctx->stream2);
+    if (ctx->stream_bt) (void)hipStreamDestroy(ctx->stream_bt);
+    for (hipEvent_t e : ctx->seg_ev) (void)hipEventDestroy(e);
+    if (ctx->seg_flags) (void)hipHostFree(ctx->seg_flags);
     delete ctx;
 }
 
@@ -440,6 +457,14 @@
         ctx->opt_duo_pk = value != 0;
     else if (k == "duo_claim")
         ctx->opt_duo_claim = (value >= 1 && value <= DUO_CLAIM_MAX) ? value : 0;
+    else if (k == "bt_slim")
+        ctx->opt_bt_slim = value != 0;
+    else if (k == "duo_seg")
+        ctx->opt_duo_seg = (value >= 0 && value <= DUO_SEG_MAX) ? value : 0;
+    else if (k == "duo_seg_len")
+        ctx->opt_duo_seg_len = value > 0 ? value : 0;
+    else if (k == "duo_seg_min_pairs")
+        ctx->opt_duo_seg_min_pairs = value;
     else if (k == "duo_min_pairs")
         ctx->opt_duo_min_pairs = value;
     else if (k == "compact_call_bases")
@@ -546,8 +571,10 @@
     ctx->dbg_arena = nullptr, ctx->dbg_n = 0;
     if (ctx->bt_pending) {
         (void)hipStreamSynchronize(ctx->stream2);
+        if (ctx->stream_bt) (void)hipStreamSynchronize(ctx->stream_bt);
         ctx->bt_pending = false;
     }
+    ctx->seg_S_last = 0, ctx->seg_early_last = 0, ctx->seg_launch_last = 0, ctx->seg_ev_used = 0;
     if (ops_needed) *ops_needed = 0;
     if (n_pairs == 0) return WFAHIP_OK;
     if (!d_q_off || !d_q_len || !d_t_off || !d_t_len || !d_rec || (!d_ops && ops_cap)) return WFAHIP_ERR_BAD_ARG;
@@ -890,6 +917,96 @@
 #endif
         const uint64_t rkey = class_key;
         const uint64_t arena_mult = (ctx->rows_key == rkey && ctx->opt_packed_arena_bytes <= 0) ? ctx->rows_scale : 1;
+        const auto seg_range = [&](const KParams &Q, uint32_t s, uint32_t &first, uint32_t &n) {
+            const uint64_t cn = Q.chunk_n, a = std::min<uint64_t>((uint64_t)s * Q.seg_len, cn);
+            const uint64_t b  = s + 1u == Q.seg_n ? cn : std::min<uint64_t>((uint64_t)(s + 1u) * Q.seg_len, cn);
+            first = (uint32_t)a, n = (uint32_t)(b - a);
+        };
+        const auto seg_prepare = [&](KParams &Q, uint32_t S, uint64_t cn, hipStream_t s0) -> int {
+            int r;
+            if (!ctx->seg_flags) {
+                HIP_TRY(hipHostMalloc(reinterpret_cast<void **>(&ctx->seg_flags), DUO_SEG_MAX * 4, hipHostMallocMapped));
+                HIP_TRY(hipHostGetDevicePointer(reinterpret_cast<void **>(&ctx->seg_flags_dev), ctx->seg_flags, 0));
+            }
+            if (!ctx->stream_bt) {
+                int lo = 0, hi = 0;
+                HIP_TRY(hipDeviceGetStreamPriorityRange(&lo, &hi));
+                HIP_TRY(hipStreamCreateWithPriority(&ctx->stream_bt, hipStreamNonBlocking, hi));
+            }
+            while (ctx->seg_ev.size() < 2u * (DUO_SEG_MAX + 2u)) {
+                hipEvent_t e;
+                HIP_TRY(hipEventCreate(&e));
+                ctx->seg_ev.push_back(e);
+            }
+            if ((r = ensure(ctx, ctx->seg_ctl, (DUO_SEG_MAX + 8) * 4))) return r;
+            if ((r = ensure(ctx, ctx->bt_done, (size_t)cn))) return r;
+            for (int i = 0; i < DUO_SEG_MAX; i++) reinterpret_cast<volatile uint32_t *>(ctx->seg_flags)[i] = 0u;
+            HIP_TRY(hipMemsetAsync(ctx->seg_ctl.p, 0, (DUO_SEG_MAX + 8) * 4, s0));
+            HIP_TRY(hipMemsetAsync(ctx->bt_done.p, 0, (size_t)cn, s0));
+            HIP_TRY(hipMemsetAsync(Q.pair_meta, 0xFF, 16 * cn, s0));
+            Q.seg_n = S;
+            Q.seg_len = ctx->opt_duo_seg_len > 0 ? (uint32_t)std::min<int64_t>(ctx->opt_duo_seg_len, 0x7FFFFFFF) : (uint32_t)std::max<uint64_t>(1, (cn + S - 1) / S);
+            Q.seg_count = static_cast<uint32_t *>(ctx->seg_ctl.p), Q.seg_flag = ctx->seg_flags_dev;
+            Q.bt_skipped = static_cast<uint32_t *>(ctx->seg_ctl.p) + DUO_SEG_MAX, Q.bt_done = static_cast<uint8_t *>(ctx->bt_done.p);
+            return WFAHIP_OK;
+        };
+        const auto seg_backtraces = [&](KParams &Q, uint32_t S, uint64_t cn, hipEvent_t evF, hipEvent_t ev_end) -> int {
+            hipStream_t sb = ctx->stream_bt;
+            const volatile uint32_t *const fl = ctx->seg_flags;
+            uint32_t launched = 0u, early = 0u, n_launch = 0u;
+            const auto launch = [&](uint32_t first, uint32_t n, uint32_t mode, bool slim) -> int {
+                if (n == 0u && mode != 2u) return WFAHIP_OK;
+                Q.bt_first = first, Q.bt_n = n, Q.bt_mode = mode;
+                hipEvent_t ea = ctx->seg_ev[2u * ctx->seg_ev_used], eb = ctx->seg_ev[2u * ctx->seg_ev_used + 1u];
+                ctx->seg_ev_used++;
+                HIP_TRY(hipEventRecord(ea, sb));
+                const uint32_t cnt = n ? n : (uint32_t)cn;
+                if (slim)
+                    hipLaunchKernelGGL(wfa_backtrace_slim_kernel, dim3((cnt + BT_SLIM_THREADS - 1) / BT_SLIM_THREADS), dim3(BT_SLIM_THREADS), 0, sb, Q);
+                else
+                    hipLaunchKernelGGL(wfa_backtrace_kernel, dim3((cnt + BT_THREADS - 1) / BT_THREADS), dim3(BT_THREADS), 0, sb, Q);
+                HIP_TRY(hipGetLastError());
+                HIP_TRY(hipEventRecord(eb, sb));
+                n_launch++;
+                return WFAHIP_OK;
+            };
+            int r = WFAHIP_OK;
+            for (;;) {
+                const hipError_t q = hipEventQuery(evF);
+                if (q != hipSuccess && q != hipErrorNotReady) HIP_TRY(q);
+                const bool done = q == hipSuccess;
+                if (done) break;
+                for (uint32_t s = 0; s < S; s++)
+                    if (!((launched >> s) & 1u) && fl[s] != 0u) {
+                        uint32_t first, n;
+                        seg_range(Q, s, first, n);
+                        if ((r = launch(first, n, 1u, true))) return r;
+                        launched |= 1u << s, early++;
+                    }
+            }
+            HIP_TRY(hipStreamWaitEvent(sb, evF, 0));
+            for (uint32_t s = 0; s < S;) {
+                if ((launched >> s) & 1u) {
+                    s++;
+                    continue;
+                }
+                uint32_t first, n, e = s;
+                seg_range(Q, s, first, n);
+                while (e + 1u < S && !((launched >> (e + 1u)) & 1u)) {
+                    uint32_t f2, n2;
+                    seg_range(Q, ++e, f2, n2);
+                    n += n2;
+                }
+                if ((r = launch(first, n, early ? 1u : 0u, false))) return r;
+                s = e + 1u;
+            }
+            if (early && (r = launch(0u, 0u, 2u, false))) return r;
+            HIP_TRY(hipEventRecord(ev_end, sb));
+            ctx->seg_S_last = S, ctx->seg_early_last = early, ctx->seg_launch_last = n_launch;
+            Q.seg_n = 0, Q.seg_len = 0, Q.seg_count = nullptr, Q.seg_flag = nullptr;
+            Q.bt_first = 0, Q.bt_n = 0, Q.bt_mode = 0, Q.bt_skipped = nullptr, Q.bt_done = nullptr;
+            return WFAHIP_OK;
+        };
         auto forward_pass = [&](Kind kind, const std::vector<uint32_t> *list, uint64_t first_pair, uint64_t count, std::vector<uint64_t> &redo_out,
                                 bool detach_bt, const PassClass *cls = nullptr, uint64_t rows_mult = 0) -> int {
             const uint32_t seq_words = (cls ? cls : &batch_class)->seq_words;
@@ -941,8 +1058,13 @@
             }
             if (rc2) return rc2;
             if (meta_buf.bytes < chunk * 16 * n_buf && (rc2 = ensure(ctx, meta_buf, chunk_alloc * 16 * n_buf))) return rc2;
-            detach_bt = detach_bt && n_chunks == 1 && ctx->opt_tail_overlap != 0 &&
-                        (count * (uint64_t)max_len > (uint64_t)ctx->opt_compact_call_bases || ctx->opt_compact_call_bases <= 0);
+            const bool detach_ok = detach_bt && n_chunks == 1 && ctx->opt_tail_overlap != 0;
+            detach_bt = detach_ok && (count * (uint64_t)max_len > (uint64_t)ctx->opt_compact_call_bases || ctx->opt_compact_call_bases <= 0);
+            uint32_t seg_S = 1;
+            if (kind == K_DUO && detach_ok && !list && ctx->opt_duo_pk) {
+                if (ctx->opt_duo_seg > 1) seg_S = (uint32_t)std::min<int64_t>(ctx->opt_duo_seg, DUO_SEG_MAX), detach_bt = true;
+                else if (ctx->opt_duo_seg == 0 && detach_bt && DUO_SEG_DEFAULT > 1 && (int64_t)count >= ctx->opt_duo_seg_min_pairs) seg_S = (uint32_t)DUO_SEG_DEFAULT;
+            }
             ctrl_fresh = false;
             const bool stream_bt = kind == K_BLK16 && shape == 0 && !blk_batch && n_buf == 1 && ctx->opt_bt_stream > 0 && (int64_t)chunk >= ctx->opt_bt_stream_min &&
                                    ctx->opt_bt_stream_single != 0;
@@ -1009,7 +1131,12 @@
                 if (kind == K_DUO) {
                     if (grid > 0xFFFFu || T.pairs_wave != 8) return WFAHIP_ERR_INTERNAL;
                     P.duo_claim = ctx->opt_duo_claim > 0 ? (uint32_t)ctx->opt_duo_claim : (uint32_t)DUO_CLAIM;
-                    HIP_TRY(wfa_launch_duo(shape, P, grid, lds_bytes, st, P.census != 0, ctx->opt_duo_pk));
+                    if (seg_S > 1) {
+                        if ((rc2 = seg_prepare(P, seg_S, cn, st))) return rc2;
+                        HIP_TRY(wfa_launch_duo(shape, P, grid, lds_bytes + (size_t)DUO_SEG_LDS_WORDS * 4, st, P.census != 0, true, true));
+                    } else {
+                        HIP_TRY(wfa_launch_duo(shape, P, grid, lds_bytes, st, P.census != 0, ctx->opt_duo_pk));
+                    }
                 } else if (kind != K_REG && kind != K_PACKED) {
                     uint32_t fl = (P.census ? (uint32_t)FWD_CENSUS : 0u) | (P.adaptive ? (uint32_t)FWD_ADAPTIVE : 0u);
                     if (stream_bt) fl |= FWD_STREAM;
@@ -1028,10 +1155,16 @@
                     hipLaunchKernelGGL(wfa_packed_kernel, dim3(grid), dim3(64), lds_bytes, st, P);
                 HIP_TRY(hipGetLastError());
                 HIP_TRY(hipEventRecord(evFb, st));
+                if (seg_S > 1) {
+                    if ((rc2 = seg_backtraces(P, seg_S, cn, evFb, evBb))) return rc2;
+                    continue;
+                }
                 if (st_bt != st) HIP_TRY(hipStreamWaitEvent(st_bt, evFb, 0));
                 if (st_bt != st) HIP_TRY(hipEventRecord(evBa, st_bt));
                 if (is_long && (ctx->opt_long_wave_bt >= 2 || (ctx->opt_long_wave_bt == 1 && cn <= (ctx->opt_long_wave_bt_pairs ? (uint64_t)ctx->opt_long_wave_bt_pairs : (uint64_t)ctx->num_cus * 20))))
                     hipLaunchKernelGGL(wfa_backtrace_wave_kernel, dim3((uint32_t)((cn + BTW_WAVES - 1) / BTW_WAVES)), dim3(64 * BTW_WAVES), 0, st_bt, P);
+                else if (ctx->opt_bt_slim != 0)
+                    hipLaunchKernelGGL(wfa_backtrace_slim_kernel, dim3((uint32_t)((cn + BT_SLIM_THREADS - 1) / BT_SLIM_THREADS)), dim3(BT_SLIM_THREADS), 0, st_bt, P);
                 else
                     hipLaunchKernelGGL(wfa_backtrace_kernel, dim3((uint32_t)((cn + BT_THREADS - 1) / BT_THREADS)), dim3(BT_THREADS), 0, st_bt, P);
                 HIP_TRY(hipGetLastError());
@@ -1467,7 +1600,14 @@
     if (ctrl_fresh) std::memcpy(hctrl, hc_last, sizeof hctrl);
     else if ((rc = fetch_ctrl(hctrl, nullptr))) return rc;
     float ms = 0;
-    if (ctx->bt_pending) {
+    if (ctx->bt_pending && ctx->seg_ev_used) {
+        for (uint32_t i = 0; i < ctx->seg_ev_used; i++) {
+            HIP_TRY(hipEventElapsedTime(&ms, ctx->seg_ev[2u * i], ctx->seg_ev[2u * i + 1u]));
+            ctx->timing.kernel_ms += ms;
+        }
+        ctx->timing.n_launches += ctx->seg_ev_used - 1u;
+        ctx->seg_ev_used = 0, ctx->bt_pending = false;
+    } else if (ctx->bt_pending) {
         HIP_TRY(hipEventElapsedTime(&ms, ctx->evBtA, ctx->evBtB));
         ctx->timing.kernel_ms += ms;
         ctx->bt_pending = false;
diff --git a/wfa_amd/csrc/wfa_packed.hpp b/wfa_amd/csrc/wfa_packed.hpp
--- a/wfa_amd/csrc/wfa_packed.hpp
+++ b/wfa_amd/csrc/wfa_packed.hpp
@@ -270,6 +270,7 @@
 }
 
 constexpr uint64_t OPS_OFF_OWN = ~0ull;
+template <class Writer = OpsWriterRev>
 WFA_DEV void backtrace_one(const KParams &P, uint32_t idx, uint32_t s_final, uint32_t h_end, uint32_t cells, bool coherent,
                            uint64_t off_given = OPS_OFF_OWN) {
     const uint32_t  pair = P.work ? P.work[idx] : P.chunk_first + idx;
@@ -281,7 +282,7 @@
 
     const uint32_t bound = ops_bound(P, s_final);
     const uint64_t off   = off_given != OPS_OFF_OWN ? off_given : atomicAdd(P.ops_cursor, (unsigned long long)bound);
-    OpsWriterRev   ow;
+    Writer         ow;
     const bool     fits = off + bound <= P.ops_cap;
     ow.init(P.ops + off, fits ? bound : 0u);
     TraceOut to;
@@ -355,13 +356,24 @@
 }
 
 #ifndef WFA_NO_AUX_KERNELS
-__global__ __launch_bounds__(BT_THREADS) void wfa_backtrace_kernel(const KParams P) {
-    __shared__ uint32_t           wsum[BT_THREADS / 64];
+template <int THREADS, class Writer>
+WFA_DEV void backtrace_lanes(const KParams &P) {
+    __shared__ uint32_t           wsum[THREADS / 64];
     __shared__ unsigned long long wbase;
-    const uint32_t idx  = blockIdx.x * blockDim.x + threadIdx.x;
-    const bool     have = idx < P.chunk_n;
+    if (P.bt_mode == 2u && __hip_atomic_load(P.bt_skipped, __ATOMIC_RELAXED, __HIP_MEMORY_SCOPE_AGENT) == 0u) return;
+    const uint32_t rel  = blockIdx.x * blockDim.x + threadIdx.x;
+    const uint32_t idx  = P.bt_first + rel;
+    bool           have = rel < (P.bt_n ? P.bt_n : P.chunk_n) && idx < P.chunk_n;
+    if (P.bt_mode == 2u && have) have = P.bt_done[idx] == 0;
     uint4          meta = make_uint4(ST_PENDING, 0u, 0u, 0u);
     if (have) meta = P.pair_meta[idx];
+    if (P.bt_mode == 1u) {
+        const bool               pending = have && meta.x == ST_PENDING;
+        const unsigned long long pm      = __ballot(pending);
+        if (pm != 0ull && (threadIdx.x & 63u) == 0u) atomicAdd(P.bt_skipped, (uint32_t)__builtin_popcountll(pm));
+        have = have && !pending;
+        if (have) P.bt_done[idx] = 1;
+    }
     if (have && meta.x != ST_OK && meta.x < ST_REDO_BYTES) {
         const uint32_t pair = P.work ? P.work[idx] : P.chunk_first + idx;
         const uint4    z    = make_uint4(0u, 0u, 0u, 0u);
@@ -393,7 +405,14 @@
     __syncthreads();
     uint64_t off = wbase + (incl - bound);
     for (uint32_t w = 0; w < wv; w++) off += wsum[w];
-    if (walk) backtrace_one(P, slot, s_final, h_end, cells, false, off);
+    if (walk) backtrace_one<Writer>(P, slot, s_final, h_end, cells, false, off);
+}
+
+__global__ __launch_bounds__(BT_THREADS) void wfa_backtrace_kernel(const KParams P) { backtrace_lanes<BT_THREADS, OpsWriterRev>(P); }
+
+constexpr int BT_SLIM_THREADS = 256;
+__global__ __launch_bounds__(BT_SLIM_THREADS) __attribute__((amdgpu_num_vgpr(32))) void wfa_backtrace_slim_kernel(const KParams P) {
+    backtrace_lanes<BT_SLIM_THREADS, OpsWriterRevT<4>>(P);
 }
 
 
```
